# tsinghua-fib-lab/PIML

Hardware: AMD Instinct MI355X
Metric: agent-pair force evals/sec + simulated steps/sec, 4096-agent GC scene (higher is better)
Workload: dtype f32

## Files before the change

include/piml_hip.h:

```cpp
#ifndef PIML_HIP_H
#define PIML_HIP_H

#include <stddef.h>
#include <stdint.h>

#ifdef __cplusplus
extern "C" {
#endif

#define PIML_HIP_ABI_VERSION 35
#define PIML_MAX_TOPK 32

int piml_abi_version(void);

const char* piml_error_string(int err);

int piml_heading_fwd(const float* velocity, int C, int T, int N, float* heading, void* stream);

int piml_relfeat_fwd(const float* position, const float* heading, const float* velocity,
                     const float* acceleration, int state_ld, const float* destination,
                     const float* obstacles, int C, int N, int M, int focal_begin,
                     int focal_count, int topk_ped, int topk_obs, float cos_thr_ped,
                     float cos_thr_obs, float dist_thr_ped, float dist_thr_obs,
                     float* ped_feat, float* obs_feat, float* dest_feat, int dest_feat_ld,
// ... 564 lines not shown
    float* partials;
    float* grads;
    float* packed;
    float* pred;
    const float* g_pred_rows;
    const float* g_d2;
    const float *fold_w3, *fold_b3;
    float fold_scale;
    float* dw1_out;
} piml_decoder_branch;

int piml_decoder_pack_floats(void);
int piml_decoder_partial_floats(void);
int piml_decoder_workgroups(long long agents);
int piml_decoder_fwd(const piml_decoder_branch* branches, int nbranches, const float* self_features, float tau,
                     float* acc, void* stream);
int piml_decoder_bwd(const piml_decoder_branch* branches, int nbranches, const float* g_pred,
                     const float* self_features, float tau, float* g_self, void* stream);

int piml_rowdecoder_slots(long long rows);
int piml_rowdecoder_fwd(const piml_decoder_branch* branches, int nbranches, void* stream);
int piml_rowdecoder_fwd_packed(const piml_decoder_branch* branches, int nbranches, void* stream);
int piml_rowdecoder_bwd(const piml_decoder_branch* branches, int nbranches, void* stream);
int piml_rowdecoder_bwd_acc(const piml_decoder_branch* branches, int nbranches, int accumulate, void* stream);

typedef struct piml_collision_head {
    const float* msgs;
    long long rows;
    const float *w1, *b1, *w2, *b2;
    float* packed;
    float* out;
    const float *fold_w3, *fold_b3;
    float fold_scale;
} piml_collision_head;

int piml_collision_head_pack_floats(void);
int piml_collision_head_fwd(const float* msgs, long long rows, const float* w1, const float* b1, const float* w2,
                            const float* b2, float* packed, float* out, void* stream);

typedef struct piml_head64 {
    const float* x;
    long long rows;
    const float *w1, *b1, *w2, *b2;
    float* hidden;
    float* out;
    const float* g_out;
    float* g_x;
    float* partials;
    float* grads;
} piml_head64;
int piml_head64_partial_floats(void);
int piml_head64_slots(long long rows);
int piml_head64_fwd(const piml_head64* head, void* stream);
int piml_head64_bwd(const piml_head64* head, void* stream);
int piml_head64_bwd_acc(const piml_head64* head, int accumulate, void* stream);

typedef struct piml_corrector {
    long long agents;
    int k;
    float scale;
    const float* enc;
    const unsigned* keep_bits;
    const float *wa, *ba, *wb, *bb, *wc, *bc, *wd, *bd;
    float *hid, *score, *attn, *pooled, *chid, *out;
    const float* g_out;
    float *g_pooled, *g_score, *g_chid, *g_enc;
    float *partials_a, *partials_b, *grads;
} piml_corrector;
int piml_corrector_partial_floats(int which);
int piml_corrector_slots(int which, long long agents, int k);
int piml_corrector_fwd(const piml_corrector* c, void* stream);
int piml_corrector_bwd(const piml_corrector* c, int accumulate, void* stream);

int piml_pinnsf_unfold_defer(int on, void* stream);
#define PIML_PACKED_VALID 1
#define PIML_FORK 2
#define PIML_ACCUMULATE 4
#define PIML_DEFER_SLOT_SUMS 8
#define PIML_DEFER_PACK 16
#define PIML_POOL_H2 32
#define PIML_POOL_TRAIN 64
#define PIML_POOL_MSGS 128
#define PIML_DEFER_UNFOLD 256
int piml_pinnsf_pool_train_ok(const piml_encoder_branch* enc, int nbranches);
int piml_pinnsf_pool_msgs_ok(const piml_encoder_branch* enc, int nbranches);
int piml_pinnsf_pool_h2_ok(const piml_encoder_branch* enc, int nbranches);
int piml_pinnsf_pack_flush(void);
int piml_pinnsf_slot_sums_flush(void);
int piml_pinnsf_pack(const piml_encoder_branch* enc, const piml_decoder_branch* dec, int nbranches,
                     const piml_collision_head* head, int flags, void* stream);
int piml_pinnsf_fwd(const piml_encoder_branch* enc, const piml_decoder_branch* dec, int nbranches,
                    const piml_collision_head* head, const float* self_features, float tau, float* acc, int flags,
                    void* stream);
int piml_pinnsf_bwd(const piml_encoder_branch* enc, const piml_decoder_branch* dec, int nbranches, const float* g_pred,
                    const float* self_features, float tau, float* g_self, int flags, void* stream);

typedef struct piml_comm_id { char internal[128]; } piml_comm_id;
int piml_comm_available(void);
int piml_comm_unique_id(piml_comm_id* id);
int piml_comm_init(void** comm, int world, int rank, const piml_comm_id* id);
int piml_comm_destroy(void* comm);
int piml_allgather_state(void* comm, const float* own, size_t floats_per_rank, float* full, void* stream);
int piml_reducescatter_grad(void* comm, const float* full, float* own, size_t floats_per_rank, void* stream);
int piml_allreduce_sum(void* comm, float* buf, size_t count, void* stream);

typedef struct piml_ipc_handle { char internal[64]; } piml_ipc_handle;
int piml_p2p_alloc(size_t bytes, void** devptr);
int piml_p2p_free(void* devptr);
int piml_p2p_export(void* devptr, piml_ipc_handle* out);
int piml_p2p_open(const piml_ipc_handle* in, void** devptr);
int piml_p2p_close(void* devptr);
int piml_p2p_copy(void* dst, const void* src, size_t bytes, void* stream);
#define PIML_P2P_MAX_PARTS 8
typedef struct piml_p2p_msg {
    const float* scatter_src;
    size_t scatter_floats;
    float* out_scatter;
    int n_bcast;
    const float* bcast_src[PIML_P2P_MAX_PARTS];
    size_t bcast_floats[PIML_P2P_MAX_PARTS];
    float* out_bcast[PIML_P2P_MAX_PARTS];
    int sum;
} piml_p2p_msg;
int piml_p2p_exchange(const piml_p2p_msg* msg, int rank, int world, float* const* peer_recv, unsigned* const* peer_flags,
                      size_t slot_floats, unsigned* ctr, unsigned spin_limit, int* status, void* stream);
int piml_allgather_state_p2p(const float* own, size_t floats_per_rank, int rank, int world, float* const* peer_recv,
                             unsigned* const* peer_flags, unsigned seq, unsigned spin_limit, int* status, void* stream);

#ifdef __cplusplus
}
#endif
#endif
```

include/piml_hip_tuning.h:

```cpp
#ifndef PIML_HIP_TUNING_H
#define PIML_HIP_TUNING_H

#include "piml_hip.h"

#ifdef __cplusplus
extern "C" {
#endif

int piml_timer_create(void** event);
int piml_timer_record(void* event, void* stream);
int piml_timer_elapsed_ms(void* start, void* stop, float* ms);
int piml_timer_destroy(void* event);

int piml_trace_begin(void);
int piml_trace_mark(const char* name, void* stream);
int piml_trace_end(char* names, int names_cap, float* us, int us_cap);

int piml_probe_arith(const float* rx, const float* ry, const float* hx, const float* hy,
                     float* dist, float* cosv, int n, void* stream);

long long piml_encoder_split_tiles(long long tiles);
long long piml_encoder_split_tiles_train(long long tiles);
int piml_encoder_products(int split_bf16);
int piml_rowdecoder_products(int split_bf16);
int piml_encoder_dw2(int layer_split);
int piml_encoder_fused_bwd(int on);
int piml_encoder_sums_bwd(int form);
int piml_encoder_sums_dec_slots(int on);
int piml_encoder_compact_rows(int on);
int piml_relfeat_pack_form(int form);
int piml_relfeat_pack_plan(int form, int waves, int obstacle_workgroups, int nbr, int has_head, int has_fold, int skip_f32,
                           int* pack_blocks, int* share);
int piml_relfeat_pack_tail_blocks(int b, int nb, int total, int* out, int cap);
int piml_pinnsf_streams_init(void);

#ifdef __cplusplus
}
#endif
#endif
```

piml_amd/_lib.py:

```python
import ctypes
import os

import torch

_HERE = os.path.dirname(os.path.abspath(__file__))
LIB_PATH = os.environ.get('PIML_LIB') or os.path.join(_HERE, 'libpiml_hip.so')
ABI_VERSION = 35
COMPACT_MAX_AGENTS = 16384
COMPACT_SLOTS = 256

_lib = None

_i, _f, _p, _z = ctypes.c_int, ctypes.c_float, ctypes.c_void_p, ctypes.c_size_t
_ll = ctypes.c_longlong
_d = ctypes.c_double


class EncoderBranch(ctypes.Structure):
    _fields_ = [('x', _p), ('rows', _ll), ('in_dim', _i), ('k', _i),
                ('w1', _p), ('b1', _p), ('w2', _p), ('b2', _p), ('w3', _p), ('b3', _p),
                ('scale', _f), ('h1', _p), ('h2', _p), ('msgs', _p), ('g_pooled', _p), ('g_msgs', _p),
                ('g2', _p), ('g1', _p), ('g_x', _p), ('partials', _p), ('grads', _p), ('packed', _p), ('relu_mask', _p),
                ('keep_bits', _p), ('drop_state', _p), ('drop_p', _f), ('sum_a', _p), ('sum_b', _p),
                ('nbr_idx', _p), ('plan', _p)]
# ... 10 lines not shown
class CollisionHead(ctypes.Structure):
    _fields_ = [('msgs', _p), ('rows', _ll), ('w1', _p), ('b1', _p), ('w2', _p), ('b2', _p), ('packed', _p), ('out', _p),
                ('fold_w3', _p), ('fold_b3', _p), ('fold_scale', _f)]


class Head64(ctypes.Structure):
    _fields_ = [('x', _p), ('rows', _ll), ('w1', _p), ('b1', _p), ('w2', _p), ('b2', _p), ('hidden', _p), ('out', _p),
                ('g_out', _p), ('g_x', _p), ('partials', _p), ('grads', _p)]


class Corrector(ctypes.Structure):
    _fields_ = [('agents', _ll), ('k', _i), ('scale', _f), ('enc', _p), ('keep_bits', _p),
                ('wa', _p), ('ba', _p), ('wb', _p), ('bb', _p), ('wc', _p), ('bc', _p), ('wd', _p), ('bd', _p),
                ('hid', _p), ('score', _p), ('attn', _p), ('pooled', _p), ('chid', _p), ('out', _p),
                ('g_out', _p), ('g_pooled', _p), ('g_score', _p), ('g_chid', _p), ('g_enc', _p),
                ('partials_a', _p), ('partials_b', _p), ('grads', _p)]


class Scenario(ctypes.Structure):
    _fields_ = [('position', _p), ('velocity', _p), ('acceleration', _p), ('destination', _p), ('hist_velocity', _p),
                ('self_features', _p), ('desired_speed', _p), ('mask', _p), ('flag', _p), ('waypoints', _p), ('exit_idx', _p),
                ('spawn_iters', _p), ('position_out', _p), ('velocity_out', _p), ('acceleration_out', _p),
                ('destination_out', _p), ('mask_out', _p), ('spawn_out', _p), ('frame_counter', _p), ('spawned', _p),
                ('dropped', _p), ('entries', _p), ('route_polyline', _p),
                ('hist_width', _i), ('F', _i), ('D', _i), ('E', _i), ('P', _i), ('R', _i), ('capacity', _i), ('T', _i),
                ('n_initial', _i), ('route_max_iters', _i), ('spawn_cap', _i), ('uniform_speed', _i),
                ('dt', _f), ('spawn_offset', _f), ('route_clearance', _f), ('arrival_radius', _f), ('speed_mean', _f),
                ('speed_std', _f), ('speed_min', _f), ('seed', ctypes.c_uint64), ('poisson_thresholds', ctypes.c_uint32 * 8)]


class ScenarioRules(ctypes.Structure):
    _fields_ = [('spawn_law', _i), ('arrival_rule', _i), ('initial_velocity', _i), ('speed_clamp', _i), ('spawn_cap2', _i),
                ('grid', _i), ('length', _f), ('width', _f), ('side_ratio', _f), ('direction_ratio', _f),
                ('poisson_thresholds2', ctypes.c_uint32 * 8), ('square_grid', _f * 32)]


class MlapmLaw(ctypes.Structure):
    _fields_ = [('variant', _i), ('tau', _f), ('A', _f), ('B', _f), ('C', _f), ('D', _f), ('theta_deg', _f), ('radius', _f)]


class WallGrid(ctypes.Structure):
    _fields_ = [('points', _p), ('cell_start', _p), ('n_points', _i), ('gx', _i), ('gy', _i),
                ('x0', _f), ('y0', _f), ('cell', _f), ('cutoff', _f)]


class WallLaw(ctypes.Structure):
    _fields_ = [('A', _f), ('B', _f)]


class GroupLaw(ctypes.Structure):
    _fields_ = [('A', _f), ('dist', _f)]


class SceneGroups(ctypes.Structure):
    _fields_ = [('row_unit', _p), ('unit_rows', _p), ('n_units', _i), ('group_first', _p), ('group_size', _p)]


class NoiseLaw(ctypes.Structure):
    _fields_ = [('rho', _f), ('amp', _f)]


class NoiseArgs(ctypes.Structure):
    _fields_ = [('state', _p), ('law', NoiseLaw), ('law_table', _p)]


class NavGrid(ctypes.Structure):
    _fields_ = [('u', _p), ('G', _i), ('gx', _i), ('gy', _i), ('x0', _f), ('y0', _f), ('cell', _f), ('near', _f)]


class NavSight(ctypes.Structure):
    _fields_ = [('parent', _p), ('G', _i), ('gx', _i), ('gy', _i)]


class ExitChoice(ctypes.Structure):
    _fields_ = [('margin', _f), ('commit', _f), ('every', _i)]


SPAWN_LAWS = {'gc': 0, 'crosswalk': 1, 'square': 2, 'unit1': 3, 'unit2': 4, 'unit3': 5, 'clip': 6}
SPAWN_CLIP_GROUPS = 7
ARRIVAL_RULES = {'gc': 0, 'radius': 1, 'x_band': 2, 'x_exit': 3}


PACKED_VALID, FORK, ACCUMULATE, DEFER_SLOT_SUMS, DEFER_PACK, POOL_H2, POOL_TRAIN, POOL_MSGS, DEFER_UNFOLD = 1, 2, 4, 8, 16, 32, 64, 128, 256

SIGNATURES = {
    'piml_abi_version': [],
    'piml_heading_fwd': [_p, _i, _i, _i, _p, _p],
    'piml_relfeat_fwd': [_p, _p, _p, _p, _i, _p, _p, _i, _i, _i, _i, _i, _i, _i, _f, _f, _f, _f,
                         _p, _p, _p, _i, _p, _p, _p],
    'piml_mlapm_step_fwd': [_p, _p, _p, _p, _i, _i, _f, _f, _f, _f, _f, _f, _f, _f, _i, _p, _p, _p],
    'piml_mlapm_step_bwd': [_p, _p, _p, _p, _p, _i, _i, _f, _f, _f, _f, _f, _f, _f, _f, _p, _p, _p, _p, _p],
    'piml_mlapm_rollout_step': [_p, _p, _p, _p, _ll, _i, _i, _f, _f, _f, _f, _f, _f, _f, _f, _p, _p, _p],
    'piml_mlapm_bwd_workspace_floats': [_i, _i],
    'piml_mlapm_step_bwd_ws': [_p, _p, _p, _p, _p, _i, _i, _f, _f, _f, _f, _f, _f, _f, _f, _p, _p, _p, _p, _p, _ll, _p],
    'piml_mlapm_fit_workspace_doubles': [_i, _i],
    'piml_mlapm_fit_loss_grad': [_p, _p, _p, _p, _p, _p, _i, _i, _p, _i, _p, _i, _p, _i, _f, _f, _p, _ll, _p, _p, _p],
    'piml_mlapm_rollout_fit_workspace_doubles': [_i, _i, _ll],
    'piml_mlapm_rollout_fit_loss_grad': [_p, _p, _p, _p, _p, _i, _ll, _i, _p, _i, _p, _p, _i, _ll, _p, _i, _f, _f, _d,
                                         _p, _ll, _p, _p, _p, _p],
    'piml_collision_matrix': [_p, _i, _i, _f, _i, _p, _p],
    'piml_collision_friends': [_p, _p, _i, _i, _i, _i, _p],
    'piml_collision_counts': [_p, _i, _i, _p, _i, _p, _p],
    'piml_collision_counts_frames': [_p, _i, _i, _i, _p, _i, _p, _p],
    'piml_collision_counts_scratch': [_p, _i, _i, _p, _i, _p, _p, _p],
    'piml_collision_counts_grid': [_p, _i, _i, _p, _i, _p, _p, _p],
    'piml_collision_label': [_p, _z, _i, _p, _p],
    'piml_sinkhorn_frames': [_p, _p, _p, _p, _i, _i, _i, _f, _i, _f, _p, _p, _p, _p, _p],
    'piml_mmd_frames': [_p, _p, _p, _p, _i, _i, _i, _d, _i, _d, _p, _p],
    'piml_crowd_stats_workspace_bytes': [_i, _i, _i],
    'piml_crowd_stats': [_p, _p, _p, _p, _i, _i, _i, _i, _i, _f, _i, _f, _f, _f, _f, _f, _i, _i, _f, _i,
                         _p, _p, _p, _p, _p, _p, _p, _p, _p, _p, _ll, _p],
    'piml_crowd_stats_voronoi_workspace_bytes': [_i, _i, _i, _i],
    'piml_crowd_stats_voronoi': [_p, _p, _p, _p, _i, _i, _i, _i, _i, _f, _p, _i, _i, _f, _f, _f, _f, _i, _f, _f, _f, _f, _f,
                                 _i, _i, _f, _i, _p, _p, _p, _p, _p, _p, _p, _p, _p, _p, _p, _ll, _p],
    'piml_pair_stats_workspace_bytes': [_i, _i, _i, _i],
    'piml_pair_stats': [_p, _p, _p, _p, _i, _i, _i, _i, _i, _p, _i, _f, _f, _i, _f, _f, _f, _f, _f, _i, _f, _i,
                        _p, _p, _p, _p, _p, _p, _p, _p, _ll, _p],
    'piml_flow_stats_workspace_bytes': [_i, _i, _i, _i],
    'piml_flow_stats': [_p, _p, _p, _p, _i, _i, _i, _i, _i, _f, _f, _i, _f, _f, _f, _f, _f, _i, _f, _f, _f, _f, _f, _i, _i,
                        _p, _p, _p, _p, _p, _p, _p, _p, _p, _p, _p, _p, _ll, _p],
    'piml_view_stats_workspace_bytes': [_i, _i, _i, _i],
    'piml_view_stats': [_p, _p, _p, _p, _i, _i, _i, _i, _i, _p, _i, _f, _f, _i, _f, _f, _f, _f, _i, _i, _f, _f, _f, _f,
                        _p, _p, _p, _p, _p, _p, _p, _ll, _p],
    'piml_track_stats_workspace_bytes': [_i, _i, _i],
    'piml_track_stats': [_p, _p, _p, _i, _i, _i, _i, _i, _f, _f, _i, _f, _f, _i, _p, _p, _p, _p, _p, _p, _p, _p, _p, _p, _p, _p,
                         _p, _p, _ll, _p],
    'piml_obstacle_stats_workspace_bytes': [_i, _i, _i, _i],
    'piml_obstacle_stats': [_p, _p, _p, _p, _i, _i, _i, _i, _i, _p, _i, _f, _f, _f, _i, _f, _f, _f, _f, _f, _i, _f, _i,
                            _p, _p, _p, _p, _p, _p, _p, _p, _p, _p, _p, _p, _p, _p, _ll, _p],
    'piml_line_stats_workspace_bytes': [_i, _i, _i, _i, _i, _i],
    'piml_line_stats': [_p, _p, _p, _i, _i, _i, _i, _i, _p, _i, _f, _f, _i, _i, _p, _p, _p, _p, _p, _p, _p, _p, _p, _p, _p, _ll,
                        _p],
    'piml_group_pairs': [_p, _p, _p, _i, _i, _i, _i, _i, _f, _f, _f, _i, _i, _p, _p, _p, _p, _p, _p, _p],
    'piml_group_members': [_p, _p, _i, _i, _i, _i, _i, _p, _i, _f, _f, _f, _f, _i, _i, _p, _p, _p, _p, _p, _p],
    'piml_group_components': [_p, _p, _p, _p, _i, _i, _i, _i, _i, _i, _p, _p, _p, _p, _p, _p, _p, _p, _p],
    'piml_calc_acceleration': [_p, _z, _i, _i, _f, _f, _f, _f, _f, _f, _p, _p],
    'piml_rollout_step': [_p, _p, _p, _p, _p, _p, _i, _p, _p, _i, _i, _p, _p, _p, _p, _p, _p, _p, _i, _p, _p, _p,
                          _p, _p, _p, _p, _p, _i, _i, _i, _f, _i, _p],
    'piml_rollout_step_ksum': [_p, _i, _p, _i, _f, _p, _p, _p, _p, _p, _p, _i, _p, _p, _i, _i, _p, _p, _p, _p, _p, _p, _p, _i, _p, _p, _p,
                               _p, _p, _p, _p, _p, _i, _i, _i, _f, _i, _p],
    'piml_scenario_step': [_p, _p, _i, _p],
    'piml_scenario_step_rules': [_p, _p, _p, _i, _p],
    'piml_scenario_step_members': [_p, _p, _i, _p, _p, _i, _p],
    'piml_scenario_step_mlapm': [_p, _p, _i, _p, _p, _i, _p],
    'piml_mlapm_law_table_bytes': [_i],
    'piml_mlapm_law_table_fill': [_p, _i, _p],
    'piml_scenario_step_mlapm_laws': [_p, _p, _i, _p, _p, _i, _p],
    'piml_wall_force': [_p, _ll, _p, _f, _f, _p, _p, _p, _p],
    'piml_scenario_step_mlapm_walls': [_p, _p, _i, _p, _p, _p, _p, _p, _p, _i, _p],
    'piml_group_force': [_p, _p, _p, _ll, _f, _f, _p, _p],
    'piml_scenario_step_mlapm_groups': [_p, _p, _i, _p, _p, _p, _p, _p, _p, _p, _p, _p, _i, _i, _p],
    'piml_noise_force': [_p, _p, _p, _p, _p, _i, _i, _ll, _f, _f, _p],
    'piml_scenario_step_mlapm_noise': [_p, _p, _i, _p, _p, _p, _p, _p, _p, _p, _p, _p, _p, _i, _i, _p],
    'piml_nav_relax': [_p, _p, _p, _p, _i, _i, _i, _i, _p, _p],
    'piml_nav_direction': [_p, _p, _p, _ll, _p, _p, _p, _p, _p],
    'piml_scenario_step_mlapm_nav': [_p, _p, _i, _p, _p, _p, _p, _p, _p, _p, _p, _i, _p],
    'piml_nav_density': [_p, _p, _i, _i, _f, _f, _f, _i, _i, _p, _p],
    'piml_nav_cost': [_p, _i, _i, _i, _f, _i, _f, _f, _f, _p, _p],
    'piml_nav_relax_cost': [_p, _p, _p, _p, _p, _i, _i, _i, _i, _i, _p, _p],
    'piml_scenario_step_mlapm_navdyn': [_p, _p, _i, _p, _p, _p, _p, _p, _p, _p, _ll, _p, _i, _p],
    'piml_nav_descent': [_p, _i, _i, _i, _p, _p],
    'piml_nav_flow': [_p, _p, _p, _i, _i, _f, _f, _f, _i, _i, _p, _p, _p],
    'piml_nav_cost_flow': [_p, _p, _p, _i, _i, _i, _i, _f, _i, _f, _f, _f, _f, _f, _p, _p],
    'piml_nav_relax_cost_gates': [_p, _p, _p, _p, _p, _i, _i, _i, _i, _i, _p, _p],
    'piml_nav_relax_active': [_p, _p, _p, _i, _p, _p, _i, _i, _i, _i, _i, _p, _p, _p, _p],
    'piml_nav_choose_exit': [_p, _i, _p, _p, _ll, _p, _p, _p, _i, _p],
    'piml_nav_sight_relax': [_p, _p, _p, _p, _p, _p, _p, _i, _i, _i, _i, _p, _p],
    'piml_nav_direction_sight': [_p, _p, _p, _ll, _p, _p, _p, _p, _p, _p],
    'piml_scenario_step_mlapm_sight': [_p, _p, _i, _p, _p, _p, _p, _p, _p, _p, _p, _p, _i, _p],
    'piml_scenario_step_nav': [_p, _p, _i, _p, _p, _i, _p, _p, _p, _p],
    'piml_scenario_route': [_p, _p, _i, _p, _i, _i, _f, _p, _p, _p],
    'piml_collision_correction_fwd': [_p, _p, _p, _z, _i, _i, _f, _f, _p, _p],
    'piml_collision_correction_bwd': [_p, _p, _p, _p, _z, _i, _i, _f, _f, _p, _p, _p, _p],
    'piml_train_step_fwd': [_p] * 7 + [_i, _i, _p, _p, _p, _p, _p, _p, _p, _i, _i, _i, _i, _f, _p, _p, _p, _p, _p, _p, _p, _p],
    'piml_train_step_fwd_copy': [_p] * 7 + [_i, _i, _p, _p, _p, _p, _p, _p, _p, _i, _i, _i, _i, _f, _p, _p, _p, _p, _p, _p, _p, _p, _ll, _p],
    'piml_train_step_bwd': [_p, _p, _p, _p, _p, _i, _i, _i, _i, _f, _p, _p, _p, _p, _p],
    'piml_train_step_bwd6': [_p, _p, _p, _p, _p, _p, _i, _i, _i, _i, _f, _p, _p, _p, _p, _p],
    'piml_pinnsf_unfold_defer': [_i, _p],
    'piml_train_step_bwd7': [_p, _ll, _p, _p, _p, _p, _ll, _p, _p, _i, _i, _i, _i, _f, _p, _p, _p, _p, _p],
    'piml_train_step_tail_fwd': [_p, _p, _p, _p, _i, _p, _i, _p, _f, _p, _p, _p, _i, _i, _p, _p, _p, _p, _p, _p, _p, _i, _i, _i, _i, _f,
                                 _p, _p, _p, _p, _p, _p, _p, _p, _ll, _p],
    'piml_train_step_tail_bwd': [_p, _ll, _p, _p, _p, _p, _ll, _p, _p, _i, _i, _i, _i, _f, _p, _p, _p, _p, _p, _f, _i, _i, _p, _p, _p, _p],
    'piml_pinnsf_epilogue_fwd': [_p, _p, _p, _z, _f, _p, _p],
    'piml_pinnsf_epilogue_bwd': [_p, _p, _z, _f, _p, _p],
    'piml_pinnsf_epilogue_ksum_fwd': [_p, _i, _p, _i, _p, _z, _f, _p, _p],
    'piml_pinnsf_epilogue_ksum_bwd': [_p, _p, _z, _f, _i, _i, _p, _p, _p, _p],
    'piml_pinnsf_epilogue_agentnorm_fwd': [_p, _p, _p, _i, _i, _f, _p, _p],
    'piml_pinnsf_epilogue_ksum_agentnorm_fwd': [_p, _i, _p, _i, _p, _i, _i, _f, _p, _p],
    'piml_pinnsf_epilogue_agentnorm_bwd': [_p, _p, _i, _i, _f, _p, _p],
    'piml_self_features_fwd': [_p, _i, _p, _p, _z, _p, _p],
    'piml_self_features_bwd': [_p, _z, _p, _p, _p, _p],
    'piml_colsum_blocks': [_z, _i],
    'piml_act_bwd_colsum': [_p, _p, _z, _i, _p, _p, _p, _p],
    'piml_sum_leading': [_p, _i, _z, _p, _p],
    'piml_act_bwd_colsum_stage1': [_p, _p, _z, _i, _p, _p, _p, _p],
    'piml_layer_reduce': [_p, _i, _z, _p, _p, _i, _i, _p, _p],
    'piml_scale_ksum_fwd': [_p, _p, _z, _i, _i, _f, _p, _p, _p, _p],
    'piml_ksum_blocks': [_z, _i],
    'piml_scale_ksum_bwd': [_p, _p, _z, _i, _i, _f, _p, _p, _p, _p],
    'piml_dropout_keep_bits': [_p, _ll, _i, _f, _i, _p, _p],
    'piml_timer_create': [ctypes.POINTER(_p)],
    'piml_timer_record': [_p, _p],
    'piml_timer_elapsed_ms': [_p, _p, ctypes.POINTER(_f)],
    'piml_timer_destroy': [_p],
    'piml_trace_begin': [],
    'piml_trace_mark': [ctypes.c_char_p, _p],
    'piml_trace_end': [ctypes.c_char_p, _i, ctypes.POINTER(_f), _i],
    'piml_probe_arith': [_p, _p, _p, _p, _p, _p, _i, _p],
    'piml_encoder_partial_floats': [],
    'piml_encoder_pack_floats': [],
    'piml_encoder_split_tiles': [_ll],
    'piml_encoder_split_tiles_train': [_ll],
    'piml_multi_copy': [ctypes.POINTER(_p), ctypes.POINTER(_p), ctypes.POINTER(_z), _i, _p],
    'piml_rollout_prologue': [_p] * 8 + [_i] * 4 + [_p] * 11 + [_p],
    'piml_rollout_losses_blocks': [_i, _i],
    'piml_rollout_losses': [_p, _p, _ll, _p, _p, _p, _p, _p, _i, _i, _i, _f, _p, _p, _p, _p, _p, _p, _p],
    'piml_rollout_losses_bwd': [_p, _p, _p, _p, _p, _p, _ll, _p, _p],
    'piml_rollout_losses_frames': [_p, _p, _ll, _p, _p, ctypes.POINTER(_p), _i, _p, _i, _i, _i, _f, _f, _f, _p, _p, _p, _p, _p, _p, _p],
    'piml_rollout_losses_frames_bwd': [_p, _p, _p, _p, _f, _f, _p, _p, _p, _ll, _p, _p],
    'piml_collision_pred_loss_blocks': [_ll, _i],
    'piml_collision_pred_loss': [ctypes.POINTER(_p), ctypes.POINTER(_p), _i, _ll, _i, _i, _p, _i, _i, _f, _p, _p, _p, _p, _p],
    'piml_collision_pred_loss_bwd': [_p, _p, _ll, _p, _p],
    'piml_adam_tickets': [],
    'piml_adam_step': [ctypes.POINTER(_p)] * 5 + [ctypes.POINTER(_ll), _i, ctypes.c_double, ctypes.c_double, ctypes.c_double, ctypes.c_double, ctypes.c_double, _p, _p],
    'piml_pointwise_losses_blocks': [_ll, _ll, _i],
    'piml_pointwise_losses': [_p, _p, _ll, _ll, _p, _ll, _f, _p, _i, _p, _p, _p, _p, _p],
    'piml_p2p_alloc': [_z, ctypes.POINTER(_p)],
    'piml_p2p_free': [_p],
    'piml_p2p_export': [_p, _p],
    'piml_p2p_open': [_p, ctypes.POINTER(_p)],
    'piml_p2p_close': [_p],
    'piml_p2p_copy': [_p, _p, _z, _p],
    'piml_allgather_state_p2p': [_p, _z, _i, _i, ctypes.POINTER(_p), ctypes.POINTER(_p), ctypes.c_uint, ctypes.c_uint, _p, _p],
    'piml_encoder_products': [_i],
    'piml_relfeat_pack_form': [_i],
    'piml_relfeat_pack_plan': [_i, _i, _i, _i, _i, _i, _i, ctypes.POINTER(_i), ctypes.POINTER(_i)],
    'piml_relfeat_pack_tail_blocks': [_i, _i, _i, ctypes.POINTER(_i), _i],
    'piml_rowdecoder_products': [_i],
    'piml_encoder_dw2': [_i],
    'piml_encoder_fused_bwd': [_i],
    'piml_encoder_sums_bwd': [_i],
    'piml_encoder_sums_dec_slots': [_i],
    'piml_encoder_compact_rows': [_i],
    'piml_encoder_pack': [ctypes.POINTER(EncoderBranch), _i, _p],
    'piml_encoder_workgroups': [ctypes.POINTER(EncoderBranch), _i, ctypes.POINTER(_i)],
    'piml_encoder_fwd': [ctypes.POINTER(EncoderBranch), _i, _p],
    'piml_encoder_fwd_packed': [ctypes.POINTER(EncoderBranch), _i, _p],
    'piml_encoder_bwd': [ctypes.POINTER(EncoderBranch), _i, _p],
    'piml_encoder_bwd_acc': [ctypes.POINTER(EncoderBranch), _i, _i, _p],
    'piml_encoder_ksum': [_p, _ll, _i, _p, _p],
    'piml_decoder_pack_floats': [],
    'piml_decoder_partial_floats': [],
    'piml_decoder_workgroups': [_ll],
    'piml_decoder_fwd': [ctypes.POINTER(DecoderBranch), _i, _p, _f, _p, _p],
    'piml_decoder_bwd': [ctypes.POINTER(DecoderBranch), _i, _p, _p, _f, _p, _p],
    'piml_rowdecoder_slots': [_ll],
    'piml_rowdecoder_fwd': [ctypes.POINTER(DecoderBranch), _i, _p],
    'piml_rowdecoder_fwd_packed': [ctypes.POINTER(DecoderBranch), _i, _p],
    'piml_rowdecoder_bwd': [ctypes.POINTER(DecoderBranch), _i, _p],
    'piml_rowdecoder_bwd_acc': [ctypes.POINTER(DecoderBranch), _i, _i, _p],
    'piml_collision_head_pack_floats': [],
    'piml_collision_head_fwd': [_p, _ll, _p, _p, _p, _p, _p, _p, _p],
    'piml_head64_partial_floats': [],
    'piml_head64_slots': [_ll],
    'piml_head64_fwd': [ctypes.POINTER(Head64), _p],
    'piml_head64_bwd': [ctypes.POINTER(Head64), _p],
    'piml_head64_bwd_acc': [ctypes.POINTER(Head64), _i, _p],
    'piml_corrector_partial_floats': [_i],
    'piml_corrector_slots': [_i, _ll, _i],
    'piml_corrector_fwd': [ctypes.POINTER(Corrector), _p],
    'piml_corrector_bwd': [ctypes.POINTER(Corrector), _i, _p],
    'piml_pinnsf_pool_h2_ok': [ctypes.POINTER(EncoderBranch), _i],
    'piml_pinnsf_pool_train_ok': [ctypes.POINTER(EncoderBranch), _i],
    'piml_pinnsf_pool_msgs_ok': [ctypes.POINTER(EncoderBranch), _i],
    'piml_pinnsf_streams_init': [],
    'piml_pinnsf_pack_flush': [],
    'piml_pinnsf_slot_sums_flush': [],
    'piml_pinnsf_pack': [ctypes.POINTER(EncoderBranch), ctypes.POINTER(DecoderBranch), _i, ctypes.POINTER(CollisionHead),
                         _i, _p],
    'piml_pinnsf_fwd': [ctypes.POINTER(EncoderBranch), ctypes.POINTER(DecoderBranch), _i, ctypes.POINTER(CollisionHead),
                        _p, _f, _p, _i, _p],
    'piml_pinnsf_bwd': [ctypes.POINTER(EncoderBranch), ctypes.POINTER(DecoderBranch), _i, _p, _p, _f, _p, _i, _p],
    'piml_comm_available': [],
    'piml_comm_unique_id': [_p],
    'piml_comm_init': [ctypes.POINTER(_p), _i, _i, _p],
    'piml_comm_destroy': [_p],
    'piml_allgather_state': [_p, _p, _z, _p, _p],
    'piml_reducescatter_grad': [_p, _p, _p, _z, _p],
    'piml_allreduce_sum': [_p, _p, _z, _p],
    'piml_relfeat_fwd_self': [_p, _p, _p, _p, _i, _p, _p, _p, _i, _i, _i, _i, _i, _i, _i, _f, _f, _f, _f, _p, _p, _p, _p, _p, _p, _p],
    'piml_relfeat_bwd_self': [_p, _p, _p, _p, _p, _p, _i, _p, _i, _i, _i, _i, _i, _i, _p, _p, _p, _p],
    'piml_relfeat_fwd_tick': [_p, _p, _p, _p, _i, _p, _p, _i, _i, _i, _i, _i, _i, _i, _f, _f, _f, _f,
                              _p, _p, _p, _i, _p, _p, _p, _p],
    'piml_relfeat_self_fwd': [_p, _p, _p, _p, _i, _i, _i, _i, _i, _i, _f, _f, _f, _f, _p, _p, _p, _p, _p, _p, _p],
    'piml_relfeat_self_fwd_part': [_i, _p, _p, _p, _p, _i, _i, _i, _i, _i, _i, _f, _f, _f, _f, _p, _p, _p, _p, _p, _p, _p],
    'piml_relfeat_self_bwd': [_p, _p, _p, _p, _p, _p, _p, _i, _i, _i, _i, _i, _p, _p, _p, _p],
    'piml_relfeat_bwd_det': [_p, _p, _p, _p, _p, _p, _p, _p, _i, _p, _i, _i, _i, _i, _i, _i, _i, _p, _p, _p],
    'piml_relfeat_bwd': [_p, _p, _p, _p, _p, _p, _i, _p, _i, _i, _i, _i, _i, _i, _p, _p, _p],
}


class P2PMsg(ctypes.Structure):
    _fields_ = [('scatter_src', _p), ('scatter_floats', _z), ('out_scatter', _p), ('n_bcast', _i),
                ('bcast_src', _p * 8), ('bcast_floats', _z * 8), ('out_bcast', _p * 8), ('sum', _i)]


SIGNATURES['piml_p2p_exchange'] = [ctypes.POINTER(P2PMsg), _i, _i, ctypes.POINTER(_p), ctypes.POINTER(_p), _z, _p, ctypes.c_uint, _p, _p]


class PimlHipError(RuntimeError):
    pass


def lib():
    global _lib
    if _lib is None:
        if not os.path.exists(LIB_PATH):
            raise PimlHipError(
                f'{LIB_PATH} is missing: build it with `python -m piml_amd.build` '
                '(hipcc --offload-arch=gfx950). piml_amd has no CPU fallback.')
        L = ctypes.CDLL(LIB_PATH)
        for name, args in SIGNATURES.items():
            fn = getattr(L, name)
            fn.argtypes = args
            fn.restype = _i
        L.piml_encoder_split_tiles.restype = _ll
# ... 137 lines not shown
```

piml_amd/csrc/decoder.hip:

```cpp
#include <cstdlib>
#include <type_traits>

#include "common.hpp"
#include "pack.hpp"
#include "reduce.hpp"
#include "stages.hpp"
#include "x3.hpp"
#include "store.hpp"
#include "../../include/piml_hip.h"

namespace piml {

typedef float f32x16 __attribute__((ext_vector_type(16)));

constexpr int DEC_SLAB = 32;

struct DecArgs {
    piml_decoder_branch br[2];
    int nbr;
    const float* self_features;
    float tau;
    float* acc;
    const float* g_pred;
    float* g_self;
    int wg_split;
    int pool_h2;
};

#ifdef PIML_DEC_STAMPS
__device__ unsigned long long g_dec_stamps[1024 * 16];
#define DEC_STAMP(i, wait)                                                                         \
    do {                                                                                           \
        __builtin_amdgcn_sched_barrier(0);                                                         \
        if (wait) asm volatile("s_waitcnt vmcnt(0) lgkmcnt(0)" ::: "memory");                      \
        if (threadIdx.x == 0 && blockIdx.x < 1024) g_dec_stamps[blockIdx.x * 16 + (i)] = __builtin_amdgcn_s_memtime(); \
        __builtin_amdgcn_sched_barrier(0);                                                         \
    } while (0)
#else
#define DEC_STAMP(i, wait)
#endif

__device__ __forceinline__ f32x16 dmfma(float a, float b, f32x16 c) {
    return __builtin_amdgcn_mfma_f32_32x32x2f32(a, b, c, 0, 0, 0);
}
__device__ __forceinline__ int dfeat0(int blk, int q, int h) { return 32 * blk + 8 * q + 4 * h; }

__global__ __launch_bounds__(256) void dec_pack_kernel(DecArgs A) {
    const int b = blockIdx.y;
    const piml_decoder_branch J = b ? A.br[1] : A.br[0];
    const int e = blockIdx.x * 256 + threadIdx.x;
    if (e < DEC_PACK) J.packed[e] = dec_pack_value(J, e);
}

__device__ __forceinline__ void dec_pool_body(const piml_decoder_branch& J, long long bx) {
    const long long t = bx * 256 + threadIdx.x;
    if (t >= J.agents * (DH / 4)) return;
    const long long a = t / (DH / 4);
    const int c = (int)(t % (DH / 4));
    const float4* p = reinterpret_cast<const float4*>(J.msgs) + a * J.k * (DH / 4) + c;
    float4 s = make_float4(0.f, 0.f, 0.f, 0.f);
    for (int i = 0; i < J.k; ++i) {
        const float4 v = p[(size_t)i * (DH / 4)];
        s.x += v.x; s.y += v.y; s.z += v.z; s.w += v.w;
    }
    reinterpret_cast<float4*>(J.pooled)[t] = s;
}

__global__ __launch_bounds__(256) void dec_pool_kernel(DecArgs A) {
    dec_pool_body(blockIdx.y ? A.br[1] : A.br[0], blockIdx.x);
}

constexpr int POOL_ROWS = 10;

template <bool POOL, bool SPLIT = false, bool ROWS = false>
__device__ __forceinline__ void dec_fwd_body(const DecArgs& A, long long tile, int split_branch = 0) {
    constexpr int NB = SPLIT ? 1 : 2;
    __shared__ float part1[NB][2][2][16][64];
    __shared__ float part2[NB][2][2][16][64];
    __shared__ float part3[NB][2][2][32];
    __shared__ float poolx[POOL ? NB : 1][POOL ? 4 : 1][POOL ? 16 : 1][64];
    const int lane = threadIdx.x & 63, wave = uniform((int)(threadIdx.x >> 6));
    const int j = lane & 31, h = lane >> 5;
    const int b = SPLIT ? split_branch : wave >> 2, ob = (wave >> 1) & 1, kh = wave & 1;
    const int bi = SPLIT ? 0 : b;
    const bool active = b < A.nbr;
    const piml_decoder_branch J = b ? A.br[1] : A.br[0];
    const long long agent = tile * 32 + j;
    const bool valid = active && agent < J.agents;
    const float4* PK = reinterpret_cast<const float4*>(J.packed);
    const float* bias = J.packed + DP_B;
    float4 w2f[4], w3f[4], w1f[2][4], b2v[4];
    float b3x = 0.f, b3y = 0.f;
    if (active) {
#pragma unroll
        for (int bl = 0; bl < 2; ++bl)
#pragma unroll
            for (int q = 0; q < 4; ++q) w1f[bl][q] = PK[(A.pool_h2 == 2 ? DP_A1F : DP_A1) / 4 + ((ob * 4 + 2 * kh + bl) * 4 + q) * 64 + lane];
    }
    float4 b1v[4];
    float sfv[5] = {0.f, 0.f, 0.f, 0.f, 0.f};
    auto late_loads = [&]() {
#pragma unroll
        for (int q = 0; q < 4; ++q) {
            b1v[q] = *reinterpret_cast<const float4*>(bias + dfeat0(ob, q, h));
            if (!POOL && !ROWS && A.pool_h2 == 2) {
                const float4 cv = *reinterpret_cast<const float4*>(J.packed + DP_CF + dfeat0(ob, q, h));
                const float kf = (float)J.k;
                b1v[q].x += kf * cv.x; b1v[q].y += kf * cv.y; b1v[q].z += kf * cv.z; b1v[q].w += kf * cv.w;
            }
            w2f[q] = PK[DP_A2 / 4 + ((ob * 2 + kh) * 4 + q) * 64 + lane];
            w3f[q] = PK[DP_A3 / 4 + (kh * 4 + q) * 64 + lane];
            b2v[q] = *reinterpret_cast<const float4*>(bias + 64 + dfeat0(ob, q, h));
        }
        b3x = bias[128];
        b3y = bias[129];
        if (A.self_features && b == 0 && wave == 0) {
            const float* sp = A.self_features + (agent < A.br[0].agents ? agent : 0) * 7;
            sfv[0] = sp[0]; sfv[1] = sp[1]; sfv[2] = sp[2]; sfv[3] = sp[3]; sfv[4] = sp[6];
        }
    };
    if (POOL) {
        if (active) {
            const int blk = wave & 3, k = J.k;
            const float* mp = J.msgs + (valid ? agent : 0) * (long long)k * DH;
            float4 sum[4];
#pragma unroll
            for (int q = 0; q < 4; ++q) sum[q] = make_float4(0.f, 0.f, 0.f, 0.f);
            for (int r0 = 0; r0 < k; r0 += POOL_ROWS) {
                float4 v[POOL_ROWS][4];
#pragma unroll
                for (int u = 0; u < POOL_ROWS; ++u) {
                    const int r = r0 + u < k ? r0 + u : 0;
#pragma unroll
                    for (int q = 0; q < 4; ++q) v[u][q] = *reinterpret_cast<const float4*>(mp + (long long)r * DH + dfeat0(blk, q, h));
                }
#pragma unroll
                for (int u = 0; u < POOL_ROWS; ++u) {
                    const bool ok = r0 + u < k;
#pragma unroll
                    for (int q = 0; q < 4; ++q) {
                        sum[q].x += ok ? v[u][q].x : 0.f; sum[q].y += ok ? v[u][q].y : 0.f;
                        sum[q].z += ok ? v[u][q].z : 0.f; sum[q].w += ok ? v[u][q].w : 0.f;
                    }
                }
            }
            late_loads();
            __builtin_amdgcn_sched_barrier(0);
#pragma unroll
            for (int q = 0; q < 4; ++q) {
                if (valid) *reinterpret_cast<float4*>(J.pooled + agent * DH + dfeat0(blk, q, h)) = sum[q];
                poolx[bi][blk][4 * q + 0][lane] = valid ? sum[q].x : 0.f; poolx[bi][blk][4 * q + 1][lane] = valid ? sum[q].y : 0.f;
                poolx[bi][blk][4 * q + 2][lane] = valid ? sum[q].z : 0.f; poolx[bi][blk][4 * q + 3][lane] = valid ? sum[q].w : 0.f;
            }
        }
        __syncthreads();
    }
    float4 pv[2][4];
    if (SPLIT && !POOL && !ROWS) DEC_STAMP(0, false);
    if (active) {
        if (POOL) {
#pragma unroll
            for (int bl = 0; bl < 2; ++bl)
#pragma unroll
                for (int q = 0; q < 4; ++q)
                    pv[bl][q] = make_float4(poolx[bi][2 * kh + bl][4 * q][lane], poolx[bi][2 * kh + bl][4 * q + 1][lane],
                                            poolx[bi][2 * kh + bl][4 * q + 2][lane], poolx[bi][2 * kh + bl][4 * q + 3][lane]);
        } else {
            const float* base = (ROWS ? J.msgs : J.pooled) + (valid ? agent : 0) * DH;
#pragma unroll
            for (int bl = 0; bl < 2; ++bl)
#pragma unroll
                for (int q = 0; q < 4; ++q) pv[bl][q] = *reinterpret_cast<const float4*>(base + dfeat0(2 * kh + bl, q, h));
            if (!ROWS && A.pool_h2) {
                const long long g0 = (valid ? agent : 0) * J.k;
                if (valid && (g0 >> 5) != ((g0 + J.k - 1) >> 5)) {
                    const float* more = J.msgs + agent * DH;
#pragma unroll
                    for (int bl = 0; bl < 2; ++bl)
#pragma unroll
                        for (int q = 0; q < 4; ++q) {
                            const float4 c = *reinterpret_cast<const float4*>(more + dfeat0(2 * kh + bl, q, h));
                            pv[bl][q].x += c.x; pv[bl][q].y += c.y; pv[bl][q].z += c.z; pv[bl][q].w += c.w;
                        }
                }
            }
        }
        if (!POOL) late_loads();
        f32x16 a1;
#pragma unroll
        for (int q = 0; q < 4; ++q) {
            const float4 bq = b1v[q];
            a1[4 * q] = kh ? 0.f : bq.x; a1[4 * q + 1] = kh ? 0.f : bq.y;
            a1[4 * q + 2] = kh ? 0.f : bq.z; a1[4 * q + 3] = kh ? 0.f : bq.w;
        }
        __builtin_amdgcn_sched_barrier(0);
        if (SPLIT && !POOL && !ROWS) { DEC_STAMP(1, false); DEC_STAMP(2, true); }
#pragma unroll
        for (int bl = 0; bl < 2; ++bl)
#pragma unroll
            for (int q = 0; q < 4; ++q) {
                const float4 w = w1f[bl][q], x = pv[bl][q];
                a1 = dmfma(w.x, valid ? x.x : 0.f, a1);
                a1 = dmfma(w.y, valid ? x.y : 0.f, a1);
                a1 = dmfma(w.z, valid ? x.z : 0.f, a1);
                a1 = dmfma(w.w, valid ? x.w : 0.f, a1);
            }
#pragma unroll
        for (int r = 0; r < 16; ++r) part1[bi][ob][kh][r][lane] = a1[r];
        if (SPLIT && !POOL && !ROWS) DEC_STAMP(3, true);
    }
    __syncthreads();
    if (SPLIT && !POOL && !ROWS) DEC_STAMP(4, false);
    if (active) {
        if (!POOL && !ROWS && A.pool_h2 >= 2 && ob == 0) {
            const long long g0 = (valid ? agent : 0) * J.k;
            if (valid && (g0 >> 5) != ((g0 + J.k - 1) >> 5)) {
#pragma unroll
                for (int bl = 0; bl < 2; ++bl)
#pragma unroll
                    for (int q = 0; q < 4; ++q) *reinterpret_cast<float4*>(J.pooled + agent * DH + dfeat0(2 * kh + bl, q, h)) = pv[bl][q];
            }
        }
        float x[16];
#pragma unroll
        for (int r = 0; r < 16; ++r) x[r] = fmaxf(part1[bi][kh][0][r][lane] + part1[bi][kh][1][r][lane], 0.f);
        x[0] = __builtin_fmaf(part1[bi][kh][0][0][lane] + part1[bi][kh][1][0][lane], 0.f, x[0]);
        if (ob == 0 && J.h1 && valid) {
            float* o = J.h1 + agent * DD;
#pragma unroll
            for (int q = 0; q < 4; ++q)
                *reinterpret_cast<float4*>(o + dfeat0(kh, q, h)) = make_float4(x[4 * q], x[4 * q + 1], x[4 * q + 2], x[4 * q + 3]);
        }
        f32x16 a2;
#pragma unroll
        for (int q = 0; q < 4; ++q) {
            const float4 bq = b2v[q];
            a2[4 * q] = kh ? 0.f : bq.x; a2[4 * q + 1] = kh ? 0.f : bq.y;
            a2[4 * q + 2] = kh ? 0.f : bq.z; a2[4 * q + 3] = kh ? 0.f : bq.w;
        }
#pragma unroll
        for (int q = 0; q < 4; ++q) {
            const float4 w = w2f[q];
            a2 = dmfma(w.x, x[4 * q + 0], a2);
            a2 = dmfma(w.y, x[4 * q + 1], a2);
            a2 = dmfma(w.z, x[4 * q + 2], a2);
            a2 = dmfma(w.w, x[4 * q + 3], a2);
        }
#pragma unroll
        for (int r = 0; r < 16; ++r) part2[bi][ob][kh][r][lane] = a2[r];
        if (SPLIT && !POOL && !ROWS) DEC_STAMP(5, true);
    }
    __syncthreads();
    if (SPLIT && !POOL && !ROWS) DEC_STAMP(6, false);
    if (active && ob == 0) {
        float y[16];
#pragma unroll
        for (int r = 0; r < 16; ++r) y[r] = part2[bi][kh][0][r][lane] + part2[bi][kh][1][r][lane];
        if (J.d2 && valid) {
            float* o = J.d2 + agent * DD;
#pragma unroll
            for (int q = 0; q < 4; ++q)
                *reinterpret_cast<float4*>(o + dfeat0(kh, q, h)) = make_float4(y[4 * q], y[4 * q + 1], y[4 * q + 2], y[4 * q + 3]);
        }
        f32x16 a3;
#pragma unroll
        for (int r = 0; r < 16; ++r) a3[r] = 0.f;
        if (h == 0 && kh == 0) { a3[0] = b3x; a3[1] = b3y; }
#pragma unroll
        for (int q = 0; q < 4; ++q) {
            const float4 w = w3f[q];
            a3 = dmfma(w.x, y[4 * q + 0], a3);
            a3 = dmfma(w.y, y[4 * q + 1], a3);
            a3 = dmfma(w.z, y[4 * q + 2], a3);
            a3 = dmfma(w.w, y[4 * q + 3], a3);
        }
        if (h == 0) { part3[bi][kh][0][j] = a3[0]; part3[bi][kh][1][j] = a3[1]; }
        if (SPLIT && !POOL && !ROWS) DEC_STAMP(7, true);
    }
    __syncthreads();
    if (SPLIT && !POOL && !ROWS) DEC_STAMP(8, false);
    if (ROWS) {
        if ((wave & 3) == 0 && h == 0 && agent < J.agents)
            reinterpret_cast<float2*>(J.pred)[agent] = make_float2(part3[0][0][0][j] + part3[0][1][0][j],
                                                                   part3[0][0][1][j] + part3[0][1][1][j]);
        return;
    }
    if (wave == 0 && h == 0 && agent < A.br[0].agents) {
        float ax = part3[0][0][0][j] + part3[0][1][0][j], ay = part3[0][0][1][j] + part3[0][1][1][j];
        if (A.self_features && b == 0) {
            const float dx = sfv[0], dy = sfv[1], vx = sfv[2], vy = sfv[3], v0 = sfv[4];
            float t = norm2(dx, dy);
            t = (t == 0.f) ? t + 0.1f : t;
            ax += (v0 * (dx / t) - vx) / A.tau;
            ay += (v0 * (dy / t) - vy) / A.tau;
        }
        if (SPLIT) {
            if (A.nbr > 1) {
                atomicAdd(A.acc + 2 * agent, ax);
                atomicAdd(A.acc + 2 * agent + 1, ay);
            } else {
                reinterpret_cast<float2*>(A.acc)[agent] = make_float2(ax, ay);
            }
        } else {
            if (A.nbr > 1) { ax += part3[1][0][0][j] + part3[1][1][0][j]; ay += part3[1][0][1][j] + part3[1][1][1][j]; }
            reinterpret_cast<float2*>(A.acc)[agent] = make_float2(ax, ay);
        }
    }
    if (SPLIT && !POOL && !ROWS) DEC_STAMP(9, true);
}

__global__ __launch_bounds__(512) void dec_fwd_kernel(DecArgs A) { dec_fwd_body<false>(A, blockIdx.x); }

template <bool ROWS = false, bool SPLIT = false>
__device__ __forceinline__ void dec_bwd_dx_body(const DecArgs& A, long long tile, int rows_branch = 0, float* keep_g2 = nullptr,
                                                float* keep_g1 = nullptr) {
    constexpr int NB = (ROWS || SPLIT) ? 1 : 2;
    __shared__ float part[NB][2][2][16][64];
    const int lane = threadIdx.x & 63, wave = uniform((int)(threadIdx.x >> 6));
    const int j = lane & 31, h = lane >> 5;
    const int b = (ROWS || SPLIT) ? rows_branch : wave >> 2, ob = (wave >> 1) & 1, kh = wave & 1, blk = wave & 3;
    const int bi = (ROWS || SPLIT) ? 0 : b;
    const bool active = b < A.nbr;
    const piml_decoder_branch J = b ? A.br[1] : A.br[0];
    const long long agent = tile * 32 + j;
    const bool valid = active && agent < J.agents;
    const float4* PK = reinterpret_cast<const float4*>(J.packed);
    float2 gp = make_float2(0.f, 0.f);
    float4 hv[2][4], t1f[8];
    float sfv[5] = {0.f, 0.f, 0.f, 0.f, 0.f};
    if (active) {
        gp = reinterpret_cast<const float2*>(ROWS ? J.g_pred_rows : A.g_pred)[valid ? agent : 0];
        if (!valid) gp = make_float2(0.f, 0.f);
        float4 gd2[4];
        if (ROWS && J.g_d2) {
#pragma unroll
            for (int q = 0; q < 4; ++q) gd2[q] = *reinterpret_cast<const float4*>(J.g_d2 + (valid ? agent : 0) * DD + dfeat0(kh, q, h));
        }
        if (!ROWS && wave == 0 && b == 0 && A.g_self && A.self_features) {
            const float* sp = A.self_features + (valid ? agent : 0) * 7;
            sfv[0] = sp[0]; sfv[1] = sp[1]; sfv[4] = sp[6];
        }
        const float bg = h ? gp.y : gp.x;
        const float* hp = J.h1 + (valid ? agent : 0) * DD;
#pragma unroll
        for (int o2 = 0; o2 < 2; ++o2)
#pragma unroll
            for (int q = 0; q < 4; ++q) hv[o2][q] = *reinterpret_cast<const float4*>(hp + dfeat0(o2, q, h));
        const float t3f = J.packed[DP_T3 + 64 * kh + lane];
        float4 t2f[4];
#pragma unroll
        for (int q = 0; q < 4; ++q) t2f[q] = PK[DP_T2 / 4 + (ob * 8 + kh * 4 + q) * 64 + lane];
#pragma unroll
        for (int t = 0; t < 8; ++t) t1f[t] = PK[((!ROWS && A.pool_h2 == 2) ? DP_T1F : DP_T1) / 4 + (blk * 8 + t) * 64 + lane];
        __builtin_amdgcn_sched_barrier(0);
        if (SPLIT) { DEC_STAMP(1, false); DEC_STAMP(2, true); }
        f32x16 g2, g1;
#pragma unroll
        for (int r = 0; r < 16; ++r) { g2[r] = 0.f; g1[r] = 0.f; }
        g2 = dmfma(t3f, bg, g2);
        if (ROWS && J.g_d2) {
#pragma unroll
            for (int q = 0; q < 4; ++q) {
                g2[4 * q] += valid ? gd2[q].x : 0.f; g2[4 * q + 1] += valid ? gd2[q].y : 0.f;
                g2[4 * q + 2] += valid ? gd2[q].z : 0.f; g2[4 * q + 3] += valid ? gd2[q].w : 0.f;
            }
        }
        if (SPLIT && keep_g2) {
            if (ob == 0) {
#pragma unroll
                for (int q = 0; q < 4; ++q)
                    *reinterpret_cast<float4*>(keep_g2 + j * DD + dfeat0(kh, q, h)) =
                        valid ? make_float4(g2[4 * q], g2[4 * q + 1], g2[4 * q + 2], g2[4 * q + 3]) : make_float4(0.f, 0.f, 0.f, 0.f);
            }
        } else if (ob == 0 && valid) {
            float* o = J.g_pre2 + agent * DD;
#pragma unroll
            for (int q = 0; q < 4; ++q)
                *reinterpret_cast<float4*>(o + dfeat0(kh, q, h)) = make_float4(g2[4 * q], g2[4 * q + 1], g2[4 * q + 2], g2[4 * q + 3]);
        }
#pragma unroll
        for (int q = 0; q < 4; ++q) {
            const float4 w = t2f[q];
            g1 = dmfma(w.x, g2[4 * q + 0], g1);
            g1 = dmfma(w.y, g2[4 * q + 1], g1);
            g1 = dmfma(w.z, g2[4 * q + 2], g1);
            g1 = dmfma(w.w, g2[4 * q + 3], g1);
        }
#pragma unroll
        for (int r = 0; r < 16; ++r) part[bi][ob][kh][r][lane] = g1[r];
        if (SPLIT) DEC_STAMP(3, true);
    }
    __syncthreads();
    if (SPLIT) DEC_STAMP(4, false);
    if (active) {
    float g1c[2][16];
#pragma unroll
    for (int o2 = 0; o2 < 2; ++o2)
#pragma unroll
        for (int q = 0; q < 4; ++q) {
            const float4 a = hv[o2][q];
            const float m[4] = {a.x, a.y, a.z, a.w};
#pragma unroll
            for (int u = 0; u < 4; ++u) {
                const float v = part[bi][o2][0][4 * q + u][lane] + part[bi][o2][1][4 * q + u][lane];
                g1c[o2][4 * q + u] = (valid && m[u] > 0.f) ? v : 0.f;
            }
        }
    if (SPLIT && keep_g1) {
        if (blk < 2) {
#pragma unroll
            for (int q = 0; q < 4; ++q) {
                const float4 v0 = make_float4(g1c[0][4 * q], g1c[0][4 * q + 1], g1c[0][4 * q + 2], g1c[0][4 * q + 3]);
                const float4 v1 = make_float4(g1c[1][4 * q], g1c[1][4 * q + 1], g1c[1][4 * q + 2], g1c[1][4 * q + 3]);
                if (blk == 0) *reinterpret_cast<float4*>(keep_g1 + j * DD + dfeat0(0, q, h)) = v0;
                else *reinterpret_cast<float4*>(keep_g1 + j * DD + dfeat0(1, q, h)) = v1;
            }
        }
    } else if (blk < 2 && valid) {
        float* o = J.g_pre1 + agent * DD;
#pragma unroll
        for (int q = 0; q < 4; ++q) {
            const float4 v0 = make_float4(g1c[0][4 * q], g1c[0][4 * q + 1], g1c[0][4 * q + 2], g1c[0][4 * q + 3]);
            const float4 v1 = make_float4(g1c[1][4 * q], g1c[1][4 * q + 1], g1c[1][4 * q + 2], g1c[1][4 * q + 3]);
            if (blk == 0) *reinterpret_cast<float4*>(o + dfeat0(0, q, h)) = v0;
            else *reinterpret_cast<float4*>(o + dfeat0(1, q, h)) = v1;
        }
    }
    {
        f32x16 gpool;
#pragma unroll
        for (int r = 0; r < 16; ++r) gpool[r] = 0.f;
#pragma unroll
        for (int bp = 0; bp < 2; ++bp)
#pragma unroll
            for (int q = 0; q < 4; ++q) {
                const float4 w = t1f[bp * 4 + q];
                gpool = dmfma(w.x, g1c[bp][4 * q + 0], gpool);
                gpool = dmfma(w.y, g1c[bp][4 * q + 1], gpool);
                gpool = dmfma(w.z, g1c[bp][4 * q + 2], gpool);
                gpool = dmfma(w.w, g1c[bp][4 * q + 3], gpool);
            }
        if (valid) {
            float* o = J.g_pooled + agent * DH;
#pragma unroll
            for (int q = 0; q < 4; ++q)
                *reinterpret_cast<float4*>(o + dfeat0(blk, q, h)) =
                    make_float4(gpool[4 * q], gpool[4 * q + 1], gpool[4 * q + 2], gpool[4 * q + 3]);
        }
    }
    }
    if (SPLIT) DEC_STAMP(5, true);
    if (!ROWS && wave == 0 && b == 0 && h == 0 && valid && A.g_self && A.self_features) {
        const float dx = sfv[0], dy = sfv[1], v0 = sfv[4], tau = A.tau;
        const float n = norm2(dx, dy);
        const float t = (n == 0.f) ? n + 0.1f : n;
        const float ex = dx / t, ey = dy / t;
        const float gex = gp.x * v0 / tau, gey = gp.y * v0 / tau;
        const float gt = -(gex * dx + gey * dy) / (t * t);
        float gdx = gex / t, gdy = gey / t;
        if (n != 0.f) { gdx += gt * (dx / n); gdy += gt * (dy / n); }
        float* o = A.g_self + agent * 7;
        o[0] = gdx; o[1] = gdy; o[2] = -gp.x / tau; o[3] = -gp.y / tau; o[4] = 0.f; o[5] = 0.f;
        o[6] = (gp.x * ex + gp.y * ey) / tau;
    }
}

__global__ __launch_bounds__(512) void dec_bwd_dx_kernel(DecArgs A) { dec_bwd_dx_body<false>(A, blockIdx.x); }

template <bool ROWS = false>
__device__ __forceinline__ void dec_bwd_dw_body(const DecArgs& A, int b, int p, int w, int lane, long long slab = DEC_SLAB) {
    const piml_decoder_branch J = b ? A.br[1] : A.br[0];
    const long long R = J.agents;
    const long long s0 = (long long)p * slab < R ? (long long)p * slab : R;
    const long long s1e = s0 + slab < R ? s0 + slab : R;
    const float* __restrict__ in1 = ROWS ? J.msgs : J.pooled;
    const float* __restrict__ gpr = ROWS ? J.g_pred_rows : A.g_pred;
    const int i = lane & 31, h = lane >> 5;
    const int mb1 = w >> 2, nb1 = w & 3, mb2 = (w >> 1) & 1, nb2 = w & 1;
    const bool do2 = w < 4, do3 = w == 4 || w == 5;
    f32x16 c1, c2, c3;
#pragma unroll
    for (int r = 0; r < 16; ++r) { c1[r] = 0.f; c2[r] = 0.f; c3[r] = 0.f; }
    float s1 = 0.f, s2 = 0.f, s3 = 0.f;
    constexpr int U = DEC_SLAB / 2;
    for (long long r0 = s0; r0 < s1e || r0 == s0; r0 += DEC_SLAB) {
        const long long r1 = r0 + DEC_SLAB < s1e ? r0 + DEC_SLAB : s1e;
        float a1[U], b1[U], a2[U], b2[U], a3[U], b3[U];
#pragma unroll
        for (int u = 0; u < U; ++u) {
            const long long row = r0 + 2 * u + h;
            const bool ok = row < r1;
            const long long ro = ok ? row : (r0 < R ? r0 : 0);
            a1[u] = J.g_pre1[ro * DD + 32 * mb1 + i];
            b1[u] = in1[ro * DH + 32 * nb1 + i];
            a2[u] = do2 ? J.g_pre2[ro * DD + 32 * mb2 + i] : 0.f;
            b2[u] = do2 ? J.h1[ro * DD + 32 * nb2 + i] : 0.f;
            a3[u] = (do3 && i < 2) ? gpr[ro * 2 + i] : 0.f;
            b3[u] = do3 ? J.d2[ro * DD + 32 * nb2 + i] : 0.f;
        }
#pragma unroll
        for (int u = 0; u < U; ++u) {
            const bool ok = r0 + 2 * u + h < r1;
            const float x1 = ok ? a1[u] : 0.f, x2 = ok ? a2[u] : 0.f, x3 = ok ? a3[u] : 0.f;
            c1 = dmfma(x1, b1[u], c1);
            if (do2) c2 = dmfma(x2, b2[u], c2);
            if (do3) c3 = dmfma(x3, b3[u], c3);
            s1 += x1; s2 += x2; s3 += x3;
        }
    }
    float* P = J.partials + (size_t)p * DEC_PART;
#pragma unroll
    for (int r = 0; r < 16; ++r) {
        const int ri = (r & 3) + 8 * (r >> 2) + 4 * h;
        P[(size_t)(32 * mb1 + ri) * DH + 32 * nb1 + i] = c1[r];
        if (do2) P[DD * DH + (32 * mb2 + ri) * DD + 32 * nb2 + i] = c2[r];
        if (do3 && ri < 2) P[DD * DH + DD * DD + ri * DD + 32 * nb2 + i] = c3[r];
    }
    s1 += __shfl_xor(s1, 32, 64);
    s2 += __shfl_xor(s2, 32, 64);
    s3 += __shfl_xor(s3, 32, 64);
    float* Pb = P + DD * DH + DD * DD + 2 * DD;
    if (h == 0) {
        if (nb1 == 0) Pb[32 * mb1 + i] = s1;
        if (do2 && nb2 == 0) Pb[DD + 32 * mb2 + i] = s2;
        if (w == 4 && i < 8) Pb[2 * DD + i] = i < 2 ? s3 : 0.f;
    }
}

__device__ __forceinline__ void dec_bwd_dw_body4(const DecArgs& A, int b, int p, int w, int lane, const float* keep_g2, const float* keep_g1) {
    const piml_decoder_branch J = b ? A.br[1] : A.br[0];
    const long long R = J.agents;
    const long long s0 = (long long)p * DEC_SLAB < R ? (long long)p * DEC_SLAB : R;
    const int n = (int)(R - s0 < DEC_SLAB ? R - s0 : DEC_SLAB);
    const long long sb = n > 0 ? s0 : 0;
    const int i = lane & 31, h = lane >> 5;
    const int mb2 = w >> 1, nb2 = w & 1;
    const bool do3 = w < 2;
    constexpr int U = DEC_SLAB / 2;
    const float* __restrict__ pooled0 = J.pooled + sb * DH + 32 * w + i;
    const float* __restrict__ h10 = J.h1 + sb * DD + 32 * nb2 + i;
    const float* __restrict__ d20 = J.d2 + sb * DD + 32 * nb2 + i;
    const float* __restrict__ gp0 = A.g_pred + sb * 2 + (i & 1);
    const float* kg1 = keep_g1 + h * DD + i;
    const float* kg2 = keep_g2 + h * DD + 32 * mb2 + i;
    float a1a[U], a1b[U], b1[U], a2[U], b2[U], a3[U], b3[U];
#pragma unroll
    for (int u = 0; u < U; ++u) {
        a1a[u] = kg1[2 * u * DD];
        a1b[u] = kg1[2 * u * DD + 32];
        a2[u] = kg2[2 * u * DD];
        a3[u] = 0.f; b3[u] = 0.f;
    }
    if (n == DEC_SLAB) {
        const float* pb = pooled0 + h * DH;
        const float* hb = h10 + h * DD;
#pragma unroll
        for (int u = 0; u < U; ++u) { b1[u] = pb[2 * u * DH]; b2[u] = hb[2 * u * DD]; }
        if (do3) {
            const float* db = d20 + h * DD;
            const float* gb = gp0 + h * 2;
#pragma unroll
            for (int u = 0; u < U; ++u) { b3[u] = db[2 * u * DD]; a3[u] = gb[4 * u]; }
        }
    } else {
#pragma unroll
        for (int u = 0; u < U; ++u) {
            const int rc = 2 * u + h < n ? 2 * u + h : 0;
            b1[u] = pooled0[rc * DH]; b2[u] = h10[rc * DD];
        }
        if (do3) {
#pragma unroll
            for (int u = 0; u < U; ++u) {
                const int rc = 2 * u + h < n ? 2 * u + h : 0;
                b3[u] = d20[rc * DD]; a3[u] = gp0[rc * 2];
            }
        }
    }
    DEC_STAMP(8, false);
    DEC_STAMP(9, true);
    f32x16 c1a, c1b, c2, c3;
#pragma unroll
    for (int r = 0; r < 16; ++r) { c1a[r] = 0.f; c1b[r] = 0.f; c2[r] = 0.f; c3[r] = 0.f; }
    float s1a = 0.f, s1b = 0.f, s2 = 0.f, s3 = 0.f;
#pragma unroll
    for (int u = 0; u < U; ++u) {
        c1a = dmfma(a1a[u], b1[u], c1a);
        c1b = dmfma(a1b[u], b1[u], c1b);
        c2 = dmfma(a2[u], b2[u], c2);
        s1a += a1a[u]; s1b += a1b[u]; s2 += a2[u];
    }
    if (do3) {
#pragma unroll
        for (int u = 0; u < U; ++u) {
            const float x3 = (i < 2 && 2 * u + h < n) ? a3[u] : 0.f;
            c3 = dmfma(x3, b3[u], c3);
            s3 += x3;
        }
    }
    float* P = J.partials + (size_t)p * DEC_PART;
    DEC_STAMP(10, false);
    {
#ifdef PIML_DEC_STAMPS
        asm volatile("v_mov_b32 %0, %0" : "+v"(c1a[0]));
        DEC_STAMP(11, false);
#endif
    }
    {
        store_acc32<PIML_WT_DEC_BWD_SLOTS>(P + 32 * w, DH, lane, [&](int r) { return c1a[r]; });
        store_acc32<PIML_WT_DEC_BWD_SLOTS>(P + 32 * DH + 32 * w, DH, lane, [&](int r) { return c1b[r]; });
        store_acc32<PIML_WT_DEC_BWD_SLOTS>(P + DD * DH + 32 * mb2 * DD + 32 * nb2, DD, lane, [&](int r) { return c2[r]; });
        if (do3 && h == 0) {
            float* P3 = P + DD * DH + DD * DD + 32 * nb2 + i;
            P3[0] = c3[0]; P3[DD] = c3[1];
        }
    }
    s1a += __shfl_xor(s1a, 32, 64);
    s1b += __shfl_xor(s1b, 32, 64);
    s2 += __shfl_xor(s2, 32, 64);
    s3 += __shfl_xor(s3, 32, 64);
    float* Pb = P + DD * DH + DD * DD + 2 * DD;
    if (h == 0) {
        if (w == 0) { Pb[i] = s1a; Pb[32 + i] = s1b; }
        if (nb2 == 0) Pb[DD + 32 * mb2 + i] = s2;
        if (w == 0 && i < 8) Pb[2 * DD + i] = i < 2 ? s3 : 0.f;
    }
    DEC_STAMP(12, false);
    DEC_STAMP(13, true);
}

__global__ __launch_bounds__(256) void dec_bwd_split_kernel(DecArgs A) {
    const int bx = blockIdx.x;
    const int b = A.nbr > 1 ? (bx & 1) : 0;
    const long long tile = A.nbr > 1 ? (bx >> 1) : bx;
    __shared__ __align__(16) float keep[2][32 * DD];
    DEC_STAMP(0, false);
    dec_bwd_dx_body<false, true>(A, tile, b, keep[0], keep[1]);
    DEC_STAMP(6, false);
    __syncthreads();
    DEC_STAMP(7, false);
    dec_bwd_dw_body4(A, b, (int)tile, uniform((int)(threadIdx.x >> 6)), threadIdx.x & 63, keep[0], keep[1]);
}

__global__ __launch_bounds__(512) void dec_bwd_dw_kernel(DecArgs A) {
    const int lane = threadIdx.x & 63, w = uniform((int)(threadIdx.x >> 6));
    const int b = (A.nbr > 1 && (int)blockIdx.x >= A.wg_split) ? 1 : 0;
    dec_bwd_dw_body<false>(A, b, (int)blockIdx.x - (b ? A.wg_split : 0), w, lane);
}

__global__ __launch_bounds__(256) void rowdec_fwd_kernel(DecArgs A, int tiles0) {
    const int bx = blockIdx.x;
    if (bx < tiles0) dec_fwd_body<false, true, true>(A, bx, 0);
    else dec_fwd_body<false, true, true>(A, bx - tiles0, 1);
}

__global__ __launch_bounds__(256) void rowdec_bwd_dx_kernel(DecArgs A, int tiles0) {
    const int bx = blockIdx.x;
    if (bx < tiles0) dec_bwd_dx_body<true>(A, bx, 0);
    else dec_bwd_dx_body<true>(A, bx - tiles0, 1);
}

template <int NFLOATS>
__device__ __forceinline__ void rowdec_stage(float* lds, const float* __restrict__ src, int tid) {
    constexpr int N4 = NFLOATS / 4, ROUNDS = (N4 + 511) / 512;
    static_assert(NFLOATS % 4 == 0, "float4 granularity");
    const float4* s4 = reinterpret_cast<const float4*>(src);
    float4* d4 = reinterpret_cast<float4*>(lds);
    float4 v[ROUNDS];
#pragma unroll
    for (int r = 0; r < ROUNDS; ++r) {
        const int e = r * 512 + tid;
        v[r] = s4[e < N4 ? e : 0];
    }
#pragma unroll
    for (int r = 0; r < ROUNDS; ++r) {
        const int e = r * 512 + tid;
        if (e < N4) d4[e] = v[r];
    }
}

__global__ __launch_bounds__(512) void rowdec_fwd_big_kernel(DecArgs A, int wg_split) {
    __shared__ __align__(16) float lds[DP_T3];
    const int tid = threadIdx.x, lane = tid & 63, wave = uniform((int)(tid >> 6));
    const int b = (A.nbr > 1 && (int)blockIdx.x >= wg_split) ? 1 : 0;
    const piml_decoder_branch J = b ? A.br[1] : A.br[0];
    const int wg0 = b ? wg_split : 0;
    const int nwg = b ? (int)gridDim.x - wg_split : (A.nbr > 1 ? wg_split : (int)gridDim.x);
    const long long R = J.agents, ntiles = (R + 31) >> 5;
    if ((long long)((int)blockIdx.x - wg0) * 8 >= ntiles) return;
    rowdec_stage<DP_T3>(lds, J.packed, tid);
    __syncthreads();
    const float4* F = reinterpret_cast<const float4*>(lds);
    const float* bias = lds + DP_B;
    const int j = lane & 31, h = lane >> 5;
    for (long long tile = (long long)((int)blockIdx.x - wg0) * 8 + wave; tile < ntiles; tile += (long long)nwg * 8) {
        const long long row = tile * 32 + j;
        const bool valid = row < R;
        f32x16 X[4];
        {
            const float* base = J.msgs + (valid ? row : 0) * DH;
#pragma unroll
            for (int blk = 0; blk < 4; ++blk)
#pragma unroll
                for (int q = 0; q < 4; ++q) {
                    const float4 v = *reinterpret_cast<const float4*>(base + dfeat0(blk, q, h));
                    X[blk][4 * q] = valid ? v.x : 0.f; X[blk][4 * q + 1] = valid ? v.y : 0.f;
                    X[blk][4 * q + 2] = valid ? v.z : 0.f; X[blk][4 * q + 3] = valid ? v.w : 0.f;
                }
        }
        f32x16 a1[2], a2[2];
#pragma unroll
        for (int ob = 0; ob < 2; ++ob) {
#pragma unroll
            for (int q = 0; q < 4; ++q) {
                const float4 bq = *reinterpret_cast<const float4*>(bias + dfeat0(ob, q, h));
                a1[ob][4 * q] = bq.x; a1[ob][4 * q + 1] = bq.y; a1[ob][4 * q + 2] = bq.z; a1[ob][4 * q + 3] = bq.w;
            }
#pragma unroll
            for (int bp = 0; bp < 4; ++bp) {
                __builtin_amdgcn_sched_barrier(0);
#pragma unroll
                for (int q = 0; q < 4; ++q) {
                    const float4 w = F[DP_A1 / 4 + ((ob * 4 + bp) * 4 + q) * 64 + lane];
                    a1[ob] = dmfma(w.x, X[bp][4 * q + 0], a1[ob]);
// ... 944 lines not shown
#ifdef PIML_DEC_STAMPS
extern "C" __attribute__((visibility("default"))) int piml_dec_stamps(unsigned long long* out) {
    return (int)hipMemcpyFromSymbol(out, HIP_SYMBOL(piml::g_dec_stamps), sizeof(unsigned long long) * 1024 * 16);
}
#endif

using namespace piml;

PIML_API int piml_decoder_pack_floats(void) { return DEC_PACK; }
PIML_API int piml_decoder_partial_floats(void) { return DEC_PART; }
PIML_API int piml_decoder_workgroups(long long agents) { return dec_dw_workgroups(agents); }

static int head_check(const piml_collision_head* h);

static int dec_fill(DecArgs& A, const piml_decoder_branch* br, int nbr) {
    if (!br || nbr < 1 || nbr > 2) return hipErrorInvalidValue;
    A = DecArgs{};
    A.nbr = nbr;
    for (int i = 0; i < nbr; ++i) {
        if (!dec_branch_ok(br[i]) || br[i].agents != br[0].agents || !br[i].pooled) return hipErrorInvalidValue;
        A.br[i] = br[i];
    }
    if (nbr == 1) A.br[1] = br[0];
    return hipSuccess;
}

static int dec_fill_bwd(DecArgs& A, const piml_decoder_branch* br, int nbr, const float* g_pred) {
    if (!g_pred) return hipErrorInvalidValue;
    if (int e = dec_fill(A, br, nbr)) return e;
    for (int i = 0; i < nbr; ++i) {
        const piml_decoder_branch& b = br[i];
        if (!b.h1 || !b.d2 || !b.g_pre2 || !b.g_pre1 || !b.g_pooled || !b.partials || !b.grads) return hipErrorInvalidValue;
    }
    A.g_pred = g_pred;
    return hipSuccess;
}

int piml::dec_stage_pack(const piml_decoder_branch* br, int nbr, hipStream_t s) {
    if (!br || nbr < 1 || nbr > 2) return hipErrorInvalidValue;
    DecArgs A = {};
    A.nbr = nbr;
    for (int i = 0; i < nbr; ++i) {
        const piml_decoder_branch& b = br[i];
        if (!b.w1 || !b.b1 || !b.w2 || !b.b2 || !b.w3 || !b.b3 || !b.packed) return hipErrorInvalidValue;
        A.br[i] = b;
    }
    if (nbr == 1) A.br[1] = br[0];
    hipLaunchKernelGGL(dec_pack_kernel, dim3((DEC_PACK + 255) / 256, nbr), dim3(256), 0, s, A);
    return hipGetLastError();
}

int piml::dec_stage_pool(const piml_decoder_branch* br, int nbr, hipStream_t s) {
    DecArgs A;
    if (int e = dec_fill(A, br, nbr)) return e;
    hipLaunchKernelGGL(dec_pool_kernel, dim3((unsigned)((br[0].agents * (DH / 4) + 255) / 256), nbr), dim3(256), 0, s, A);
    return hipGetLastError();
}

template <bool X3>
__global__ __launch_bounds__(256) __attribute__((amdgpu_waves_per_eu(2))) void dec_fwd_head_kernel(DecArgs A, piml_collision_head Hd, int dec_blocks) {
    const int bx = blockIdx.x;
    if (bx < dec_blocks) {
        if (A.nbr > 1) dec_fwd_body<true, true>(A, bx >> 1, bx & 1);
        else dec_fwd_body<true, true>(A, bx, 0);
    } else {
        extern __shared__ __align__(16) float head_lds[];
        if (X3) head_fwd_body_x3<4, false, HEAD_LDS_GROUPS_POOL>(Hd.msgs, Hd.rows, Hd.packed, Hd.out, (long long)bx - dec_blocks, reinterpret_cast<u32x4*>(head_lds));
        else head_fwd_body<4>(Hd.msgs, Hd.rows, Hd.packed, Hd.out, (long long)bx - dec_blocks);
    }
}

template <bool FOLD>
__global__ __launch_bounds__(256) __attribute__((amdgpu_waves_per_eu(2))) void dec_fwd_head_sum_kernel(DecArgs A, piml_collision_head Hd, int dec_blocks) {
    const int bx = blockIdx.x;
    if (bx < dec_blocks) {
        if (A.nbr > 1) dec_fwd_body<false, true>(A, bx >> 1, bx & 1);
        else dec_fwd_body<false, true>(A, bx, 0);
    } else {
        extern __shared__ __align__(16) float head_lds[];
        head_fwd_body_x3<4, FOLD, HEAD_LDS_GROUPS>(Hd.msgs, Hd.rows, Hd.packed, Hd.out, (long long)bx - dec_blocks, reinterpret_cast<u32x4*>(head_lds));
    }
}

int piml::dec_stage_fwd_sum(const piml_decoder_branch* br, int nbr, const piml_collision_head* h, const float* self_features,
                            float tau, float* acc, hipStream_t s, bool fold) {
    DecArgs A;
    if (!acc) return hipErrorInvalidValue;
    if (int e = dec_fill(A, br, nbr)) return e;
    for (int i = 0; i < nbr; ++i)
        if (!br[i].msgs || (fold && (!br[i].fold_w3 || !br[i].fold_b3))) return hipErrorInvalidValue;
    piml_collision_head Hd = {};
    int head_blocks = 0;
    if (h && h->rows > 0) {
        if (int e = head_check(h)) return e;
        if (fold && (!h->fold_w3 || !h->fold_b3)) return hipErrorInvalidValue;
        if (!g_head_x3) return hipErrorInvalidValue;
        Hd = *h;
        head_blocks = (int)(((h->rows + 31) / 32 + 3) / 4);
    }
    A.self_features = self_features;
    A.tau = tau;
    A.acc = acc;
    A.pool_h2 = fold ? 2 : 3;
    const int tiles = (int)((br[0].agents + 31) / 32) * nbr;
    const dim3 g((unsigned)(tiles + head_blocks));
    const int lds = head_blocks ? head_lds_bytes(HEAD_LDS_GROUPS) : 0;
    if (fold) hipLaunchKernelGGL(dec_fwd_head_sum_kernel<true>, g, dim3(256), lds, s, A, Hd, tiles);
    else hipLaunchKernelGGL(dec_fwd_head_sum_kernel<false>, g, dim3(256), lds, s, A, Hd, tiles);
    return hipGetLastError();
}

int piml::dec_stage_fwd_fused(const piml_decoder_branch* br, int nbr, const piml_collision_head* h, const float* self_features,
                              float tau, float* acc, hipStream_t s) {
    DecArgs A;
    if (!acc) return hipErrorInvalidValue;
    if (int e = dec_fill(A, br, nbr)) return e;
    piml_collision_head Hd = {};
    int head_blocks = 0;
    if (h && h->rows > 0) {
        if (int e = head_check(h)) return e;
        Hd = *h;
        head_blocks = (int)(((h->rows + 31) / 32 + 3) / 4);
    }
    A.self_features = self_features;
    A.tau = tau;
    A.acc = acc;
    const int tiles = (int)((br[0].agents + 31) / 32) * nbr;
    if (g_head_x3) hipLaunchKernelGGL(dec_fwd_head_kernel<true>, dim3((unsigned)(tiles + head_blocks)), dim3(256), head_blocks ? head_lds_bytes(HEAD_LDS_GROUPS_POOL) : 0, s, A, Hd, tiles);
    else hipLaunchKernelGGL(dec_fwd_head_kernel<false>, dim3((unsigned)(tiles + head_blocks)), dim3(256), 0, s, A, Hd, tiles);
    return hipGetLastError();
}

__global__ __launch_bounds__(256) __attribute__((amdgpu_waves_per_eu(2))) void dec_fwd_ph2_kernel(DecArgs A) {
    const int bx = blockIdx.x;
    if (A.nbr > 1) dec_fwd_body<false, true>(A, bx >> 1, bx & 1);
    else dec_fwd_body<false, true>(A, bx, 0);
}

int piml::dec_stage_fwd_ph2(const piml_decoder_branch* br, int nbr, const float* self_features, float tau, float* acc,
                            hipStream_t s) {
    DecArgs A;
    if (!acc) return hipErrorInvalidValue;
    if (int e = dec_fill(A, br, nbr)) return e;
    for (int i = 0; i < nbr; ++i)
        if (!br[i].msgs) return hipErrorInvalidValue;
    A.self_features = self_features;
    A.tau = tau;
    A.acc = acc;
    A.pool_h2 = 1;
    const int tiles = (int)((br[0].agents + 31) / 32) * nbr;
    hipLaunchKernelGGL(dec_fwd_ph2_kernel, dim3((unsigned)tiles), dim3(256), 0, s, A);
    return hipGetLastError();
}

int piml::dec_stage_fwd(const piml_decoder_branch* br, int nbr, const float* self_features, float tau, float* acc,
                        hipStream_t s) {
    DecArgs A;
    if (!acc) return hipErrorInvalidValue;
    if (int e = dec_fill(A, br, nbr)) return e;
    A.self_features = self_features;
    A.tau = tau;
    A.acc = acc;
    const unsigned tiles = (unsigned)((br[0].agents + 31) / 32);
    hipLaunchKernelGGL(dec_fwd_kernel, dim3(tiles), dim3(512), 0, s, A);
    return hipGetLastError();
}

int piml::dec_stage_bwd_dx(const piml_decoder_branch* br, int nbr, const float* g_pred, const float* self_features,
                           float tau, float* g_self, hipStream_t s) {
    DecArgs A;
    if (int e = dec_fill_bwd(A, br, nbr, g_pred)) return e;
    A.self_features = self_features;
    A.tau = tau;
    A.g_self = g_self;
    const unsigned tiles = (unsigned)((br[0].agents + 31) / 32);
    hipLaunchKernelGGL(dec_bwd_dx_kernel, dim3(tiles), dim3(512), 0, s, A);
    return hipGetLastError();
}

int piml::dec_stage_bwd_fused(const piml_decoder_branch* br, int nbr, const float* g_pred, const float* self_features,
                              float tau, float* g_self, hipStream_t s, bool sums) {
    DecArgs A;
    if (int e = dec_fill_bwd(A, br, nbr, g_pred)) return e;
    A.self_features = self_features;
    A.tau = tau;
    A.g_self = g_self;
    if (sums) {
        for (int i = 0; i < nbr; ++i)
            if (!br[i].fold_w3) return hipErrorInvalidValue;
        A.pool_h2 = 2;
    }
    static_assert(DEC_SLAB == 32, "the dW slab of a workgroup is its dX tile");
    const unsigned tiles = (unsigned)((br[0].agents + 31) / 32);
    hipLaunchKernelGGL(dec_bwd_split_kernel, dim3(tiles * (unsigned)nbr), dim3(256), 0, s, A);
    return hipGetLastError();
}

int piml::dec_stage_bwd_dw(const piml_decoder_branch* br, int nbr, const float* g_pred, bool reduce, hipStream_t s) {
    DecArgs A;
    if (int e = dec_fill_bwd(A, br, nbr, g_pred)) return e;
    const int per = dec_dw_workgroups(br[0].agents);
    A.wg_split = per;
    hipLaunchKernelGGL(dec_bwd_dw_kernel, dim3(per * nbr), dim3(512), 0, s, A);
    if (reduce)
        hipLaunchKernelGGL(dec_reduce_kernel, dim3((DEC_PART / 4 + 15) / 16, nbr), dim3(256), 0, s, A, per, DEC_PART / 4);
    return hipGetLastError();
}

static int head_check(const piml_collision_head* h) {
    if (!h || h->rows < 0) return hipErrorInvalidValue;
    if (h->rows > 0 && (!h->msgs || !h->w1 || !h->b1 || !h->w2 || !h->b2 || !h->packed || !h->out)) return hipErrorInvalidValue;
    return hipSuccess;
}

int piml::head_stage_pack(const piml_collision_head* h, hipStream_t s) {
    if (!h || !h->w1 || !h->b1 || !h->w2 || !h->b2 || !h->packed) return hipErrorInvalidValue;
    hipLaunchKernelGGL(head_pack_kernel, dim3((HEAD_PACK + 255) / 256), dim3(256), 0, s, *h);
    return hipGetLastError();
}

int piml::head_stage_fwd(const piml_collision_head* h, hipStream_t s) {
    if (int e = head_check(h)) return e;
    if (h->rows == 0) return hipSuccess;
    const long long tiles = (h->rows + 31) / 32;
    if (g_head_x3) hipLaunchKernelGGL(head_fwd_kernel<true>, dim3((unsigned)((tiles + 3) / 4)), dim3(256), 0, s, h->msgs, h->rows, h->packed, h->out);
    else hipLaunchKernelGGL(head_fwd_kernel<false>, dim3((unsigned)((tiles + 3) / 4)), dim3(256), 0, s, h->msgs, h->rows, h->packed, h->out);
    return hipGetLastError();
}

PIML_API int piml_decoder_fwd(const piml_decoder_branch* br, int nbr, const float* self_features, float tau,
                              float* acc, void* stream) {
    hipStream_t s = as_stream(stream);
    if (int e = dec_stage_pack(br, nbr, s)) return e;
    if (int e = dec_stage_pool(br, nbr, s)) return e;
    return dec_stage_fwd(br, nbr, self_features, tau, acc, s);
}

PIML_API int piml_decoder_bwd(const piml_decoder_branch* br, int nbr, const float* g_pred, const float* self_features,
                              float tau, float* g_self, void* stream) {
    hipStream_t s = as_stream(stream);
    if (int e = dec_stage_bwd_dx(br, nbr, g_pred, self_features, tau, g_self, s)) return e;
    return dec_stage_bwd_dw(br, nbr, g_pred, true, s);
}

static long long rowdec_slab(long long rows) {
    long long slab = (rows + 255) / 256;
    slab = (slab + DEC_SLAB - 1) / DEC_SLAB * DEC_SLAB;
    const long long least = rows < 16384 ? 64 : 256;
    return slab < least ? least : slab;
}

constexpr int kRowdecBigTiles = 1024;

static int rowdec_wg_split(const piml_decoder_branch* br, int nbr, int total) {
    if (nbr < 2) return total;
    int w = (int)(total * (double)br[0].agents / ((double)br[0].agents + (double)br[1].agents) + 0.5);
    return w < 1 ? 1 : (w > total - 1 ? total - 1 : w);
}

PIML_API int piml_rowdecoder_slots(long long rows) {
    if (rows <= 0) return 0;
    const long long slab = rowdec_slab(rows);
    return (int)((rows + slab - 1) / slab);
}

static int rowdec_fill(DecArgs& A, const piml_decoder_branch* br, int nbr, bool bwd) {
    if (!br || nbr < 1 || nbr > 2) return hipErrorInvalidValue;
    A = DecArgs{};
    A.nbr = nbr;
    for (int i = 0; i < nbr; ++i) {
        const piml_decoder_branch& b = br[i];
        if (!dec_branch_ok(b) || !b.h1 || !b.d2) return hipErrorInvalidValue;
        if (!bwd && !b.pred) return hipErrorInvalidValue;
        if (bwd && (!b.g_pred_rows || !b.g_pre2 || !b.g_pre1 || !b.g_pooled || !b.partials || !b.grads)) return hipErrorInvalidValue;
        A.br[i] = b;
    }
// ... 110 lines not shown
```

piml_amd/csrc/encoder_bwd5.hip:

```cpp
#include "common.hpp"
#include "encoder.hpp"
#include "x3.hpp"
#include "store.hpp"

namespace piml {

typedef short f5_s16x4 __attribute__((ext_vector_type(4)));
typedef __attribute__((address_space(3))) f5_s16x4 f5_lds_s16x4;

constexpr int F5_THREADS = 512;
constexpr int F5_IMG = 3 * 128 * 64;
constexpr int F5_M = 0;
constexpr int F5_H = F5_M + 2 * F5_IMG;
constexpr int F5_TROW = 36;
constexpr int F5_TBYTES = 128 * F5_TROW * 4;
constexpr int F5_T = F5_H + 2 * F5_IMG;
constexpr int F5_XS = F5_T + 2 * F5_TBYTES;
constexpr int F5_MK = F5_XS + 3 * 1024;
constexpr int F5_W1 = F5_MK + 2 * 512;
constexpr int F5_GXP = F5_W1 + 4096;
constexpr int F5_GXP_BYTES = 4 * 32 * 16 * 4;
constexpr int F5_TAB = F5_GXP + 2 * F5_GXP_BYTES;
constexpr int F5_KMAX = 16;
constexpr int F5_LDS_BYTES = F5_TAB + F5_KMAX * 2 * 16 * 4;
constexpr int F5_LDS_LAUNCH = F5_LDS_BYTES;
static_assert(F5_LDS_LAUNCH <= 160 * 1024, "fits the CU");
constexpr int F5_PART1 = EH * EH + 1024 + 2 * EH;

struct F5Args {
    EncArgs A;
    int nA[2];
    DecSlotSums D;
};

template <int C>
__device__ __forceinline__ float f5_row_shl(float v) {
    return __int_as_float(__builtin_amdgcn_mov_dpp(__float_as_int(v), 0x100 + C, 0xf, 0xf, false));
}
template <int C>
__device__ __forceinline__ void f5_chains_add(float4& s, const float4 v) {
    if constexpr (C < 16) {
        slot_chains_add(s, make_float4(f5_row_shl<C>(v.x), f5_row_shl<C>(v.y), f5_row_shl<C>(v.z), f5_row_shl<C>(v.w)));
        f5_chains_add<C + 1>(s, v);
    }
}
__device__ __forceinline__ void f5_dec_sums(const DecSlotSums& D, int wg, int nwg, int t, int nthr) {
    const int total = D.nsets * D.lanes, per = (total + nwg - 1) / nwg;
    const int e1 = min(wg * per + per, total), half = nthr >> 4;
    for (int e = wg * per + (t >> 4); e < e1; e += 2 * half) {
        const bool two = e + half < e1;
        const int ea = e, eb = two ? e + half : e;
        const int sa = ea >= D.lanes ? 1 : 0, sb = eb >= D.lanes ? 1 : 0;
        const float4* const p[2] = {reinterpret_cast<const float4*>(sa ? D.parts[1] : D.parts[0]),
                                    reinterpret_cast<const float4*>(sb ? D.parts[1] : D.parts[0])};
        const int j[2] = {ea - sa * D.lanes, eb - sb * D.lanes};
        float4 s[2];
        slot_chains<2>(p, D.slots, D.lanes, j, t & 15, s);
        const float4 va = s[0], vb = s[1];
        f5_chains_add<1>(s[0], va);
        f5_chains_add<1>(s[1], vb);
        if ((t & 15) == 0) {
            slot_sum_store(reinterpret_cast<float4*>(sa ? D.grads[1] : D.grads[0]) + j[0], s[0], D.accumulate != 0);
            if (two) slot_sum_store(reinterpret_cast<float4*>(sb ? D.grads[1] : D.grads[0]) + j[1], s[1], D.accumulate != 0);
        }
    }
}

#ifdef PIML_F5_STAMPS
__device__ unsigned long long g_f5_stamps[256 * 8 * 16];
#define F5_STAMP(i)                                                        \
    do {                                                                   \
        __builtin_amdgcn_sched_barrier(0);                                 \
        {                                                                  \
            const unsigned long long t_ = __builtin_amdgcn_s_memtime();    \
            st[i] += t_ - tprev;                                           \
            tprev = t_;                                                    \
        }                                                                  \
        __builtin_amdgcn_sched_barrier(0);                                 \
    } while (0)
#else
#define F5_STAMP(i)
#endif

#define F5_BARRIER() asm volatile("s_waitcnt lgkmcnt(0)\n\ts_barrier" ::: "memory")

__device__ __forceinline__ float f5_relu(float x) { return __int_as_float(max(__float_as_int(x), 0)); }
__device__ __forceinline__ constexpr int f5_rho(int r) { return (r & 3) + 8 * (r >> 2); }

#define F5_SLOT(MF, FILL)                        \
    do {                                         \
        MF;                                      \
        __builtin_amdgcn_sched_barrier(0);       \
        FILL;                                    \
        __builtin_amdgcn_sched_barrier(0);       \
    } while (0)

template <bool GX, int INC, int CPM>
__device__ __forceinline__ void enc_bwd_sums2_body(const F5Args& F) {
    constexpr bool CP = CPM != 0;
    extern __shared__ __align__(16) unsigned char smem[];
    const int tid = threadIdx.x, lane = tid & 63;
    const int wv = __builtin_amdgcn_readfirstlane(tid >> 6);
    const int crew = wv >> 2, w = wv & 3;
    const int ctid = tid & 255;
    const int n = lane & 31, h = lane >> 5;
    int bx = (int)blockIdx.x, b = 0;
    const int* __restrict__ plan = CP ? F.A.br[1].plan : nullptr;
    int nA0 = F.nA[0], nA1 = F.nA[1], nne = 0, nemp = 0, ctiles = 0;
    if (CP) {
        nne = __builtin_amdgcn_readfirstlane(plan[0]); nemp = __builtin_amdgcn_readfirstlane(plan[1]);
        ctiles = __builtin_amdgcn_readfirstlane(plan[2]);
        nA0 = __builtin_amdgcn_readfirstlane(plan[3]); nA1 = __builtin_amdgcn_readfirstlane(plan[4]);
    }
    if (CPM == 2 || (CPM == 0 && bx >= nA0)) { b = 1; bx -= nA0; }
    const piml_encoder_branch J = b ? F.A.br[1] : F.A.br[0];
    const int nwg = b ? nA1 : nA0;
    constexpr bool cp = CPM == 2;
    const bool cpe = cp && nemp > 0;
    const unsigned R = (unsigned)J.rows;
    const unsigned IN = __builtin_amdgcn_readfirstlane((unsigned)J.in_dim), K = __builtin_amdgcn_readfirstlane((unsigned)J.k);
    const unsigned kmagic = __builtin_amdgcn_readfirstlane((unsigned)((0x100000000ull + K - 1) / K));
    const int ntiles = cp ? ctiles : (int)((R + 31) >> 5);
    const int nit = bx < ntiles ? (ntiles - bx + nwg - 1) / nwg : 0;
    float* P = J.partials + (size_t)bx * F5_PART1;
    constexpr int NS = INC == 6 ? 3 : 4;

    auto rsrc = [&](const void* base, unsigned bytes) {
        return __builtin_amdgcn_make_buffer_rsrc(const_cast<void*>(base), 0, (int)bytes, 0x00020000);
    };
    constexpr unsigned kOut = 0x80000000u;
    const __amdgpu_buffer_rsrc_t rs_gp = rsrc(J.g_pooled, (R / K) * EH * 4);
    const __amdgpu_buffer_rsrc_t rs_x = rsrc(J.x, R * IN * 4);
    const __amdgpu_buffer_rsrc_t rs_mk = rsrc(J.relu_mask, (unsigned)ntiles * 1024);
    const __amdgpu_buffer_rsrc_t rs_gx = rsrc(J.g_x, GX ? R * IN * 4 : 0u);
    const unsigned cS = CP ? 32u / K : 1u;
    const __amdgpu_buffer_rsrc_t rs_pl = rsrc(CP ? plan + CP_LISTS : nullptr, CP ? (unsigned)nne * 4u : 0u);
    auto ld1 = [&](const __amdgpu_buffer_rsrc_t& rs, unsigned voff, unsigned soff) {
        return (unsigned)__builtin_amdgcn_raw_buffer_load_b32(rs, (int)voff, (int)soff, 0);
    };

// ... 546 lines not shown
```

piml_amd/csrc/encoder_x3.hip:

```cpp
#include <cstdlib>

#include "common.hpp"
#include "encoder.hpp"
#include "philox.hpp"
#include "x3.hpp"

namespace piml {

struct Pieces {
    u32x4 hi[8], mid[8], lo[8];
};

__device__ __forceinline__ void split_tile(const f32x16 (&in)[4], Pieces& P) {
#pragma unroll
    for (int kb = 0; kb < 8; ++kb) {
        const f32x16& a = in[kb >> 1];
        const int r = 8 * (kb & 1);
        unsigned hi[4], mid[4], lo[4];
#pragma unroll
        for (int d = 0; d < 4; ++d) split3(a[r + 2 * d], a[r + 2 * d + 1], hi[d], mid[d], lo[d]);
        P.hi[kb] = (u32x4){hi[0], hi[1], hi[2], hi[3]};
        P.mid[kb] = (u32x4){mid[0], mid[1], mid[2], mid[3]};
        P.lo[kb] = (u32x4){lo[0], lo[1], lo[2], lo[3]};
    }
// ... 588 lines not shown
    if (!cp && (long long)((int)blockIdx.x - wg0) >= ntiles) return;
    const float* x3 = J.packed + PACK_F32;
    float xb[4];
    ENC_STAMP(0, false);
    const int k = J.k;
    const int agents = CP ? (int)(R / k) : 0;
    int iv[CP_ROUNDS0];
    if (cp) {
#pragma unroll
        for (int i = 0; i < CP_ROUNDS0; ++i) {
            const int a = i * ENC_THREADS + tid;
            iv[i] = a < agents ? J.nbr_idx[(size_t)a * k] : -1;
        }
    } else {
        load_x(xb, J.x, first, ntiles, R, IN, lane);
    }
    stage_linear<X3_IMG>(lds, x3, tid);
    stage_linear<1024 + 384>(lds + X3_FWD_F32, J.packed + 32768, tid);
    ENC_STAMP(1, true);
    int nne = 0, nemp = 0, S = 1, slot_n = 0, kn = 0;
    bool rowlive = false;
    const unsigned short* list = reinterpret_cast<const unsigned short*>(lds + CP_LDS_LIST);
    if (cp) {
        int* cnt = reinterpret_cast<int*>(lds + CP_LDS_CNT);
        unsigned short* lw = reinterpret_cast<unsigned short*>(lds + CP_LDS_LIST);
        const int rounds = (agents + ENC_THREADS - 1) / ENC_THREADS;
        unsigned flags = 0;
#pragma unroll
        for (int i = 0; i < CP_ROUNDS0; ++i) flags |= (iv[i] >= 0 ? 1u : 0u) << i;
        for (int i = CP_ROUNDS0; i < rounds; ++i) {
            const int a = i * ENC_THREADS + tid;
            const int v = a < agents ? J.nbr_idx[(size_t)a * k] : -1;
            flags |= (v >= 0 ? 1u : 0u) << i;
        }
        for (int i = 0; i < rounds; ++i) {
            const unsigned long long bal = __ballot((flags >> i) & 1u);
            if (lane == 0) cnt[i * ENC_WAVES + wave] = __popcll(bal);
        }
        __syncthreads();
        if (wave == 0) {
            int v[4], tot = 0;
#pragma unroll
            for (int u = 0; u < 4; ++u) { v[u] = 4 * lane + u < rounds * ENC_WAVES ? cnt[4 * lane + u] : 0; tot += v[u]; }
            int inc = tot;
#pragma unroll
            for (int d = 1; d < 64; d <<= 1) {
                const int o = __shfl_up(inc, d, 64);
                if (lane >= d) inc += o;
            }
            int ex = inc - tot;
#pragma unroll
            for (int u = 0; u < 4; ++u) { cnt[4 * lane + u] = ex; ex += v[u]; }
            if (lane == 63) cnt[256] = inc;
        }
        __syncthreads();
        nne = uniform(cnt[256]);
        nemp = agents - nne;
        for (int i = 0; i < rounds; ++i) {
            const int a = i * ENC_THREADS + tid;
            const unsigned bit = (flags >> i) & 1u;
            const unsigned long long bal = __ballot(bit);
            const int pos = cnt[i * ENC_WAVES + wave] + __popcll(bal & ((1ull << lane) - 1ull));
            if (a < agents) lw[bit ? pos : agents - 1 - (a - pos)] = (unsigned short)a;
        }
        S = 32 / k;
        ntiles = (nne + S - 1) / S;
        const int n = lane & 31;
        slot_n = n / k; kn = n - slot_n * k; rowlive = slot_n < S;
        if ((int)blockIdx.x == wg0) {
            if (tid == 0) cnt[257] = 0x7fffffff;
        }
        __syncthreads();
        if ((int)blockIdx.x == wg0) {
            const int tiles0 = (int)((A.br[0].rows + 31) >> 5);
            if (tid >= 2 && tid <= PIML_COMPACT_SLOTS - 2)
                atomicMin(reinterpret_cast<unsigned*>(cnt + 257), cp_split_cost(tid, tiles0, (int)ntiles, nemp) * 256u + (unsigned)tid);
            const int apad = (agents + 3) & ~3;
            for (int c = tid; c < nne; c += ENC_THREADS) J.plan[CP_LISTS + c] = list[c];
            for (int e = tid; e < nemp; e += ENC_THREADS) J.plan[CP_LISTS + apad + e] = list[agents - 1 - e];
            __syncthreads();
            if (tid == 0) {
                const int w0 = cnt[257] & 255;
                J.plan[0] = nne; J.plan[1] = nemp; J.plan[2] = (int)ntiles; J.plan[3] = w0; J.plan[4] = PIML_COMPACT_SLOTS - w0;
            }
        }
    } else {
        __syncthreads();
    }
    ENC_STAMP(2, false);
    auto load_xc = [&](long long tile) {
        const int idx = S * (int)tile + slot_n;
        const bool ok = tile < ntiles && rowlive && idx < nne;
        const long long row = ok ? (long long)list[idx] * k + kn : 0;
#pragma unroll
        for (int s = 0; s < 4; ++s) {
            const int c = 2 * s + (lane >> 5);
            xb[s] = (ok && c < IN) ? J.x[row * IN + c] : 0.f;
        }
    };
    if (cp) load_xc(first);
    const long long agents_d = R / k;
    for (long long tile = first; tile < ntiles; tile += stride) {
        int lane_t = lane;
        asm volatile("" : "+v"(lane_t));
        const u32x4* W2hm = reinterpret_cast<const u32x4*>(lds) + lane_t;
        const u32x4* W2lo = W2hm + X3_HM / 4;
        const float* W1f = lds + X3_FWD_F32;
        const float* bias = W1f + 1024;
        const int h = lane_t >> 5;
        f32x16 a[4];
        Pieces P;
#pragma unroll
        for (int blk = 0; blk < 4; ++blk) {
#pragma unroll
            for (int q = 0; q < 4; ++q) {
                const float4 bq = *reinterpret_cast<const float4*>(bias + feat0(blk, q, h));
                a[blk][4 * q + 0] = bq.x; a[blk][4 * q + 1] = bq.y; a[blk][4 * q + 2] = bq.z; a[blk][4 * q + 3] = bq.w;
            }
#pragma unroll
            for (int s = 0; s < 4; ++s) a[blk] = mfma32(W1f[(blk * 4 + s) * 64 + lane_t], xb[s], a[blk]);
#pragma unroll
            for (int r = 0; r < 16; ++r) a[blk][r] = relu1(a[blk][r]);
        }
        uint2* mrow = reinterpret_cast<uint2*>(J.relu_mask) + (tile * 2) * 64 + lane_t;
        mrow[0] = make_uint2(sign_bits(a[0], a[1]), sign_bits(a[2], a[3]));
        ENC_STAMP(3, false);
        split_tile(a, P);
        ENC_STAMP(4, false);
        if (cp) load_xc(tile + stride);
        else load_x(xb, J.x, tile + stride, ntiles, R, IN, lane);
#pragma unroll
        for (int blk = 0; blk < 4; ++blk) {
            f32x16 acc, sm;
            const float bv = bias[128 + 32 * blk + (lane_t & 31)];
#pragma unroll
            for (int r = 0; r < 16; ++r) { sm[r] = 0.f; acc[r] = bv; }
#pragma unroll
            for (int kb = 0; kb < 8; ++kb) {
                const int fb = blk * 8 + kb;
                kblock_x3_t(acc, sm, W2hm[(fb * 2) * 64], W2hm[(fb * 2 + 1) * 64], W2lo[fb * 64], P.hi[kb], P.mid[kb], P.lo[kb]);
            }
#pragma unroll
            for (int r = 0; r < 16; ++r) a[blk][r] = relu1(acc[r] + sm[r]);
        }
        ENC_STAMP(5, false);
        mrow[64] = make_uint2(sign_bits(a[0], a[1]), sign_bits(a[2], a[3]));
        if (J.h2) store_h2_rows<true>(a, J.h2, tile, R, lane_t);
        ENC_STAMP(6, false);
        if (cp) {
            if (k == 10) pool_rows_c<10>(a, (int)tile, nne, list, lane_t, J.sum_a, J.sum_b);
            else if (k == 6) pool_rows_c<6>(a, (int)tile, nne, list, lane_t, J.sum_a, J.sum_b);
            else pool_rows_c<2>(a, (int)tile, nne, list, lane_t, J.sum_a, J.sum_b);
        } else {
            pool_rows_k(a, k, tile, agents_d, lane_t, J.sum_a, J.sum_b);
        }
        ENC_STAMP(7, false);
    }
    if (cp && nemp > 0) {
        const int nwav = nwg * ENC_WAVES, idle = nwav - (int)ntiles;
        const int q = idle > 0 ? (int)first - (int)ntiles : (int)first, share = idle > 0 ? idle : nwav;
        if (q >= 0) {
            const float2 hc = reinterpret_cast<const float2*>(J.packed + PACK_ZROW + EH)[lane];
            const float2 v = make_float2((float)k * hc.x, (float)k * hc.y);
            for (int e = q; e < nemp; e += share) {
                const int ag = list[agents - 1 - e];
                reinterpret_cast<float2*>(J.sum_a + (size_t)ag * EH)[lane] = v;
// ... 595 lines not shown
```

piml_amd/csrc/network.hip:

```cpp
#include <cstdio>
#include <cstdlib>
#include <mutex>

#include "common.hpp"
#include "pack.hpp"
#include "reduce.hpp"
#include "stages.hpp"
#include "trace.hpp"

namespace piml {

namespace {

struct Side {
    hipStream_t s[2] = {nullptr, nullptr};
    hipEvent_t ev[6] = {};
    bool ok = false;
};

constexpr int kMaxDevices = 64;
Side g_side[kMaxDevices];
std::mutex g_mu;

int side_streams(Side** out) {
// ... 199 lines not shown
    for (int i = 0; P->valid && i < P->R.nsets; ++i)
        if (P->R.set[i].grads == grads) return true;
    return false;
}

int pending_slot_sums_leave(const ReduceAll& R, hipStream_t s) {
    PendingSums* P = pending_entry();
    if (!P) return hipErrorInvalidDevice;
    {
        std::lock_guard<std::mutex> lock(g_mu);
        ReduceAll& Q = P->R;
        bool merge = P->valid && P->stream == s && Q.accumulate == R.accumulate && Q.nunf == 0 && R.nunf == 0 &&
                     Q.nsets + R.nsets <= (int)(sizeof(Q.set) / sizeof(Q.set[0]));
        for (int i = 0; merge && i < Q.nsets; ++i)
            for (int j = 0; j < R.nsets; ++j)
                if (Q.set[i].grads == R.set[j].grads) { merge = false; break; }
        if (merge) {
            for (int j = 0; j < R.nsets; ++j) Q.set[Q.nsets++] = R.set[j];
            if (R.gx > Q.gx) Q.gx = R.gx;
            return hipSuccess;
        }
    }
    if (int e = pending_slot_sums_flush()) return e;
    std::lock_guard<std::mutex> lock(g_mu);
    P->R = R; P->stream = s; P->valid = true;
    return hipSuccess;
}

bool pending_slot_sums_take(hipStream_t s, ReduceAll* out) {
    PendingSums* P = pending_entry();
    if (!P) return false;
    std::lock_guard<std::mutex> lock(g_mu);
    if (!P->valid || P->stream != s) return false;
    *out = P->R;
    P->valid = false;
    return true;
}

}

using namespace piml;

PIML_API int piml_pinnsf_streams_init(void) {
    Side* S;
    return side_streams(&S);
}

PIML_API int piml_pinnsf_pack(const piml_encoder_branch* enc, const piml_decoder_branch* dec, int nbr,
                              const piml_collision_head* head, int flags, void* stream) {
    if (!enc || !dec || nbr < 1 || nbr > 2) return hipErrorInvalidValue;
    PackAll A = {};
    A.nbr = nbr;
    A.has_head = head != nullptr;
    A.skip_f32 = enc_f32_images_needed() ? 0 : 1;
    for (int i = 0; i < nbr; ++i) {
        const piml_encoder_branch& e = enc[i];
        const piml_decoder_branch& d = dec[i];
        if (e.in_dim < 1 || e.in_dim > 8 || !e.w1 || !e.b1 || !e.w2 || !e.b2 || !e.w3 || !e.b3 || !e.packed || !d.w1 || !d.b1 ||
            !d.w2 || !d.b2 || !d.w3 || !d.b3 || !d.packed)
            return hipErrorInvalidValue;
        A.enc[i] = e;
        A.dec[i] = d;
    }
    if (head) {
        if (!head->w1 || !head->b1 || !head->w2 || !head->b2 || !head->packed) return hipErrorInvalidValue;
        A.head = *head;
        if (head->fold_w3) {
            if (!head->fold_b3) return hipErrorInvalidValue;
            A.has_fold = 1;
        }
    }
    for (int i = 0; i < nbr; ++i)
        if (dec[i].fold_w3) {
            if (!dec[i].fold_b3) return hipErrorInvalidValue;
            A.has_fold = 1;
        }
    if (flags & PIML_DEFER_PACK) return pending_pack_leave(A, as_stream(stream));
    return launch_pack(A, as_stream(stream));
}

PIML_API int piml_pinnsf_pack_flush(void) { return pending_pack_flush(nullptr); }

static int reduce_all(const piml_encoder_branch* enc, const piml_decoder_branch* dec, int nbr, hipStream_t s, bool accumulate, bool defer = false,
                      bool sums = false, bool defer_unfold = false, bool dec_summed = false) {
    ReduceAll R = {};
    R.accumulate = accumulate ? 1 : 0;
    R.defer_unfold = defer_unfold ? 1 : 0;
    R.dec_upstream = dec_summed ? 1 : 0;
    int w0 = 0, n = 0, maxl = 0;
    const int total = piml_encoder_workgroups(enc, nbr, &w0);
    const int dslots = piml_decoder_workgroups(dec[0].agents);
    int n0[2] = {0, 0}, n1[2] = {0, 0};
    const bool dw2 = !sums && enc_dw2_used(enc, nbr, n0, n1);
    auto add = [&](const float* parts, float* grads, int slots, int lanes, int split, int off0, int off1) {
        R.set[n++] = ReduceSet{parts, grads, slots, lanes, split, off0, off1};
        if (lanes > maxl) maxl = lanes;
    };
    for (int i = 0; i < nbr; ++i) {
        if (sums) {
            add(enc[i].partials, enc[i].grads, nbr == 1 ? total : (i == 0 ? w0 : total - w0), DW2_L1_LANES, DW2_L1_SPLIT, DW2_L1_OFF0, DW2_L1_OFF1);
            if (nbr == 2 && enc[1].plan) R.set[n - 1].dev_slots = enc[1].plan + 3 + i;
            R.unf[i] = UnfoldSet{dec[i].grads, dec[i].w1, enc[i].w3, enc[i].b3, dec[i].fold_scale, enc[i].k, dec[i].dw1_out, enc[i].grads};
            R.nunf = nbr;
        } else if (dw2) {
            add(enc[i].partials, enc[i].grads, n0[i], DW2_L0_LANES, DW2_L0_SPLIT, 0, DW2_L0_OFF1);
            add(enc[i].partials + (size_t)n0[i] * (DW2_L0_LANES * 4), enc[i].grads, n1[i], DW2_L1_LANES, DW2_L1_SPLIT, DW2_L1_OFF0, DW2_L1_OFF1);
        } else {
            add(enc[i].partials, enc[i].grads, nbr == 1 ? total : (i == 0 ? w0 : total - w0), ENC_PART / 4, 0x7fffffff, 0, 0);
        }
    }
    if (!dec_summed)
        for (int i = 0; i < nbr; ++i) add(dec[i].partials, dec[i].grads, dslots, DEC_PART / 4, 0x7fffffff, 0, 0);
    R.nsets = n;
    R.gx = (maxl + 15) / 16;
    if (defer) return pending_slot_sums_leave(R, s);
    UnfoldTail t;
    if (int e = launch_slot_sums(unfold_begin(R, s, &t), s)) return e;
    trace_mark("pinnsf_reduce", s);
    return unfold_end(t);
}

static int g_dec_slots_enc = !(getenv("PIML_ENC_DEC_SLOTS") && atoi(getenv("PIML_ENC_DEC_SLOTS")) == 0);

PIML_API int piml_encoder_sums_dec_slots(int on) {
    const int old = g_dec_slots_enc;
    if (on >= 0) g_dec_slots_enc = on ? 1 : 0;
    return old;
}

static int g_compact_rows = !(getenv("PIML_ENC_COMPACT") && atoi(getenv("PIML_ENC_COMPACT")) == 0);

PIML_API int piml_encoder_compact_rows(int on) {
    const int old = g_compact_rows;
    if (on >= 0) g_compact_rows = on ? 1 : 0;
    return old;
}

PIML_API int piml_pinnsf_slot_sums_flush(void) { return pending_slot_sums_flush(); }

PIML_API int piml_pinnsf_pool_h2_ok(const piml_encoder_branch* enc, int nbr) { return enc_pool_h2_ok(enc, nbr) ? 1 : 0; }
PIML_API int piml_pinnsf_pool_train_ok(const piml_encoder_branch* enc, int nbr) { return enc_pool_train_ok(enc, nbr) ? 1 : 0; }
PIML_API int piml_pinnsf_pool_msgs_ok(const piml_encoder_branch* enc, int nbr) { return enc_pool_msgs_ok(enc, nbr) ? 1 : 0; }

PIML_API int piml_pinnsf_fwd(const piml_encoder_branch* enc, const piml_decoder_branch* dec, int nbr,
                             const piml_collision_head* head, const float* self_features, float tau, float* acc,
                             int flags, void* stream) {
    hipStream_t m = as_stream(stream);
    const bool pack = !(flags & PIML_PACKED_VALID);
    PIML_TRY(pending_pack_flush(m));
    if (flags & PIML_POOL_TRAIN) {
        if ((flags & (PIML_FORK | PIML_POOL_H2)) || !enc_pool_train_ok(enc, nbr)) return hipErrorInvalidValue;
        for (int i = 0; i < nbr; ++i)
            if (dec[i].pooled != enc[i].sum_a || dec[i].msgs != enc[i].sum_b) return hipErrorInvalidValue;
        if (pack) PIML_TRY(piml_pinnsf_pack(enc, dec, nbr, head, 0, stream));
        PIML_TRY(enc_stage_fwd_sum(enc, nbr, m, nbr > 1 ? acc : nullptr, nbr > 1 ? dec[0].agents * 2 : 0));
        trace_mark("enc_fwd_sum", m);
        PIML_TRY(dec_stage_fwd_sum(dec, nbr, head, self_features, tau, acc, m));
        trace_mark("dec_fwd_head_sum", m);
        return hipSuccess;
    }
    if (flags & PIML_POOL_MSGS) {
        if ((flags & (PIML_FORK | PIML_POOL_H2)) || !enc_pool_msgs_ok(enc, nbr)) return hipErrorInvalidValue;
        for (int i = 0; i < nbr; ++i)
            if (dec[i].pooled != enc[i].sum_a || dec[i].msgs != enc[i].sum_b) return hipErrorInvalidValue;
        if (head && head->rows > 0 && head->msgs != enc[0].msgs) return hipErrorInvalidValue;
        if (pack) PIML_TRY(piml_pinnsf_pack(enc, dec, nbr, head, 0, stream));
        PIML_TRY(enc_stage_fwd(enc, nbr, m, nbr > 1 ? acc : nullptr, nbr > 1 ? dec[0].agents * 2 : 0, true));
        trace_mark("enc_fwd", m);
        PIML_TRY(dec_stage_fwd_sum(dec, nbr, head, self_features, tau, acc, m, false));
        trace_mark("dec_fwd_head_sum", m);
        return hipSuccess;
    }
    if (flags & PIML_POOL_H2) {
        if ((flags & PIML_FORK) || head || !enc_pool_h2_ok(enc, nbr)) return hipErrorInvalidValue;
        if (pack) PIML_TRY(piml_pinnsf_pack(enc, dec, nbr, nullptr, 0, stream));
        PIML_TRY(enc_stage_fwd_pool(enc, nbr, m, nbr > 1 ? acc : nullptr, nbr > 1 ? dec[0].agents * 2 : 0));
        trace_mark("enc_fwd", m);
        PIML_TRY(dec_stage_fwd_ph2(dec, nbr, self_features, tau, acc, m));
        trace_mark("dec_fwd_head", m);
        return hipSuccess;
    }
    if (!(flags & PIML_FORK)) {
        if (pack) PIML_TRY(piml_pinnsf_pack(enc, dec, nbr, head, 0, stream));
        PIML_TRY(enc_stage_fwd(enc, nbr, m, nbr > 1 ? acc : nullptr, nbr > 1 ? dec[0].agents * 2 : 0));
        trace_mark("enc_fwd", m);
        PIML_TRY(dec_stage_fwd_fused(dec, nbr, head, self_features, tau, acc, m));
        trace_mark("dec_fwd_head", m);
        return hipSuccess;
    }
    Side* S;
    PIML_TRY(side_streams(&S));
    hipStream_t s0 = S->s[0], s1 = S->s[1];
    if (pack) {
        PIML_TRY(edge(m, s0, S->ev[0]));
        PIML_TRY(dec_stage_pack(dec, nbr, s0));
        if (head) PIML_TRY(head_stage_pack(head, s0));
        PIML_TRY(hipEventRecord(S->ev[1], s0));
        PIML_TRY(enc_stage_pack(enc, nbr, m));
    }
    PIML_TRY(enc_stage_fwd(enc, nbr, m));
    if (head) {
        PIML_TRY(edge(m, s1, S->ev[2]));
        if (pack) PIML_TRY(hipStreamWaitEvent(s1, S->ev[1], 0));
        PIML_TRY(head_stage_fwd(head, s1));
        PIML_TRY(hipEventRecord(S->ev[3], s1));
    }
    PIML_TRY(dec_stage_pool(dec, nbr, m));
    if (pack) PIML_TRY(hipStreamWaitEvent(m, S->ev[1], 0));
    PIML_TRY(dec_stage_fwd(dec, nbr, self_features, tau, acc, m));
    if (head) PIML_TRY(hipStreamWaitEvent(m, S->ev[3], 0));
    return hipSuccess;
}

PIML_API int piml_pinnsf_bwd(const piml_encoder_branch* enc, const piml_decoder_branch* dec, int nbr, const float* g_pred,
                             const float* self_features, float tau, float* g_self, int flags, void* stream) {
    hipStream_t m = as_stream(stream);
    if (flags & PIML_POOL_TRAIN) {
        if (flags & PIML_FORK) return hipErrorInvalidValue;
        for (int i = 0; i < nbr; ++i)
            if (!dec[i].dw1_out || !dec[i].fold_w3 || dec[i].g_pooled != enc[i].g_pooled) return hipErrorInvalidValue;
        PIML_TRY(dec_stage_bwd_fused(dec, nbr, g_pred, self_features, tau, g_self, m, true));
        trace_mark("dec_bwd", m);
        DecSlotSums D = {};
        if (g_dec_slots_enc) {
            D.nsets = nbr;
            D.slots = piml_decoder_workgroups(dec[0].agents);
            D.lanes = DEC_PART / 4;
            D.accumulate = (flags & PIML_ACCUMULATE) != 0;
            for (int i = 0; i < nbr; ++i) {
                D.parts[i] = dec[i].partials;
                D.grads[i] = dec[i].grads;
                if (pending_slot_sums_write(dec[i].grads)) D.nsets = 0;
            }
        }
        bool dec_summed = false;
        PIML_TRY(enc_stage_bwd_sum(enc, nbr, m, D.nsets > 0 ? &D : nullptr, &dec_summed));
        trace_mark("enc_bwd_dx", m);
        return reduce_all(enc, dec, nbr, m, (flags & PIML_ACCUMULATE) != 0, (flags & PIML_DEFER_SLOT_SUMS) != 0, true,
                          (flags & PIML_DEFER_UNFOLD) != 0, dec_summed);
    }
    if (!(flags & PIML_FORK)) {
        PIML_TRY(dec_stage_bwd_fused(dec, nbr, g_pred, self_features, tau, g_self, m));
        trace_mark("dec_bwd", m);
        PIML_TRY(enc_stage_bwd_dx(enc, nbr, m));
        trace_mark("enc_bwd_dx", m);
        PIML_TRY(enc_stage_bwd_dw(enc, nbr, m));
        trace_mark("enc_bwd_dw", m);
        PIML_TRY(reduce_all(enc, dec, nbr, m, (flags & PIML_ACCUMULATE) != 0, (flags & PIML_DEFER_SLOT_SUMS) != 0));
        return hipSuccess;
    }
    if (flags & (PIML_ACCUMULATE | PIML_DEFER_SLOT_SUMS)) return hipErrorInvalidValue;
    PIML_TRY(dec_stage_bwd_dx(dec, nbr, g_pred, self_features, tau, g_self, m));
    Side* S;
    PIML_TRY(side_streams(&S));
    hipStream_t s0 = S->s[0];
    PIML_TRY(edge(m, s0, S->ev[4]));
    PIML_TRY(dec_stage_bwd_dw(dec, nbr, g_pred, true, s0));
    PIML_TRY(hipEventRecord(S->ev[5], s0));
    PIML_TRY(enc_stage_bwd_dx(enc, nbr, m));
    PIML_TRY(enc_stage_bwd_dw(enc, nbr, m));
    PIML_TRY(hipStreamWaitEvent(m, S->ev[5], 0));
    return enc_stage_reduce(enc, nbr, m);
}
```

piml_amd/csrc/pack.hpp:

```cpp
#pragma once
#include <hip/hip_runtime.h>

#include "../../include/piml_hip.h"

namespace piml {

constexpr int EH = 128;
constexpr int DH = 128;
constexpr int DD = 64;
constexpr int ENC_PART = 2 * EH * EH + EH * 8 + 3 * EH;
constexpr int DEC_PART = DD * DH + DD * DD + 2 * DD + DD + DD + 8;

constexpr int PACK_FWD = 16384 * 2 + 1024 + 384;
constexpr int PACK_DX = 16384 * 2 + 1024;
constexpr int PACK_F32 = PACK_FWD + PACK_DX;

constexpr int X3_HM = 32 * 2 * 64 * 4;
constexpr int X3_LO = 32 * 64 * 4;
constexpr int X3_IMG = X3_HM + X3_LO;
constexpr int PACK_X3 = 4 * X3_IMG;
constexpr int PACK_FLOATS = PACK_F32 + PACK_X3;
constexpr int PACK_ZROW = PACK_FLOATS;
constexpr int PACK_TOTAL = PACK_FLOATS + 2 * EH;

// ... 92 lines not shown
    {
        const bool t1 = e >= DP_T1;
        const int f = t1 ? e - DP_T1 : e - DP_T2;
        const float* W = t1 ? J.w1 : J.w2;
        const int cols = t1 ? DH : DD;
        const int u = f & 3, lane = (f >> 2) & 63, q = (f >> 8) & 3, rest = f >> 10;
        const int bp = rest & 1, blk = rest >> 1;
        const int r = 32 * bp + 8 * q + 4 * (lane >> 5) + u;
        return W[(size_t)r * cols + 32 * blk + (lane & 31)];
    }
}

constexpr int HP_B = 2 * 4 * 4 * 256;
constexpr int HP_W2 = HP_B + 68;
constexpr int HP_X3 = HP_W2 + 64;
constexpr int HP_X3F = HP_X3 + 2 * 8 * 3 * 256;
constexpr int HP_BF = HP_X3F + 2 * 8 * 3 * 256;
constexpr int HEAD_PACK = HP_BF + 64;
constexpr int HEAD_PACK_PLAIN = HP_X3F;
static_assert(HP_X3 % 4 == 0 && HP_X3F % 4 == 0, "16-byte aligned fragments");

__device__ __forceinline__ float head_pack_value(const piml_collision_head& H, int e) {
    const float* __restrict__ w1 = H.w1;
    if (e >= HEAD_PACK_PLAIN) return 0.f;
    if (e < HP_B) {
        const int u = e & 3, lane = (e >> 2) & 63, q = (e >> 8) & 3, rest = e >> 10;
        const int bp = rest & 3, ob = rest >> 2;
        const int i = 32 * ob + (lane & 31), c = 32 * bp + 8 * q + 4 * (lane >> 5) + u;
        return w1[(size_t)i * DH + c];
    }
    if (e >= HP_X3) {
        const int x = e - HP_X3, d = x & 3, lane = (x >> 2) & 63, rest = x >> 8;
        const int piece = rest % 3, kb = (rest / 3) & 7, ob = rest / 24;
        const int i = 32 * ob + (lane & 31), c = 16 * kb + 8 * (lane >> 5) + 2 * d;
        unsigned hi, mid, lo;
        split3(w1[(size_t)i * DH + c], w1[(size_t)i * DH + c + 1], hi, mid, lo);
        return __uint_as_float(piece == 0 ? hi : (piece == 1 ? mid : lo));
    }
    if (e >= HP_W2) return H.w2[e - HP_W2];
    const int g = e - HP_B;
    return g < 64 ? H.b1[g] : (g == 64 ? H.b2[0] : 0.f);
}

constexpr int FOLD_GROUPS = DD * 3;

template <int CH>
__device__ __forceinline__ double fold_partial(const float* __restrict__ row, const float* __restrict__ col, int stride, int chunk) {
    constexpr int N = DH / CH;
    float wv[N], xv[N];
#pragma unroll
    for (int t = 0; t < N; ++t) { wv[t] = row[chunk * N + t]; xv[t] = col[(size_t)(chunk * N + t) * stride]; }
    double a = 0.0;
#pragma unroll
    for (int t = 0; t < N; ++t) a += (double)wv[t] * (double)xv[t];
    return a;
}

__device__ __forceinline__ void dec_fold_store(const piml_decoder_branch& J, int i, int hc, int lane, double sum) {
    const float v = (float)((double)J.fold_scale * sum);
    if (hc == 2) {
        if (lane == 0) J.packed[DP_CF + i] = v;
        return;
    }
    const int c = 64 * hc + lane;
    J.packed[DP_A1F + ((((i >> 5) * 4 + (c >> 5)) * 4 + ((c >> 3) & 3)) * 64 + (i & 31) + 32 * ((c >> 2) & 1)) * 4 + (c & 3)] = v;
    J.packed[DP_T1F + ((((c >> 5) * 2 + (i >> 5)) * 4 + ((i >> 3) & 3)) * 64 + (c & 31) + 32 * ((i >> 2) & 1)) * 4 + (i & 3)] = v;
}
__device__ __forceinline__ void head_fold_store(const piml_collision_head& H, int i, int hc, int lane, double sum) {
    if (hc == 2) {
        if (lane == 0) H.packed[HP_BF + i] = (float)((double)H.b1[i] + (double)H.fold_scale * sum);
        return;
    }
    const float a = (float)((double)H.fold_scale * sum);
    const float b = __shfl_down(a, 1, 64);
    if (lane & 1) return;
    const int c = 64 * hc + lane;
    unsigned hi, mid, lo;
    split3(a, b, hi, mid, lo);
    unsigned* dst = reinterpret_cast<unsigned*>(H.packed + HP_X3F) + ((((i >> 5) * 8 + (c >> 4)) * 3) * 64 + (i & 31) + 32 * ((c >> 3) & 1)) * 4 + ((c & 7) >> 1);
    dst[0] = hi; dst[256] = mid; dst[512] = lo;
}

template <int N>
__device__ __forceinline__ void slot_chains(const float4* const (&parts)[N], int B, int lanes, const int (&j)[N], int c, float4 (&s)[N]) {
#pragma unroll
    for (int n = 0; n < N; ++n) s[n] = make_float4(0.f, 0.f, 0.f, 0.f);
    for (int q0 = c; q0 < B; q0 += 16 * 8) {
        float4 v[N][8];
#pragma unroll
        for (int n = 0; n < N; ++n)
#pragma unroll
            for (int u = 0; u < 8; ++u) {
                const int q = q0 + 16 * u;
                v[n][u] = parts[n][(size_t)(q < B ? q : c) * lanes + j[n]];
            }
#pragma unroll
        for (int n = 0; n < N; ++n)
#pragma unroll
            for (int u = 0; u < 8; ++u) {
                const bool ok = q0 + 16 * u < B;
                s[n].x += ok ? v[n][u].x : 0.f; s[n].y += ok ? v[n][u].y : 0.f; s[n].z += ok ? v[n][u].z : 0.f; s[n].w += ok ? v[n][u].w : 0.f;
            }
    }
}
__device__ __forceinline__ void slot_chains_add(float4& s, const float4 v) { s.x += v.x; s.y += v.y; s.z += v.z; s.w += v.w; }
__device__ __forceinline__ void slot_sum_store(float4* dst, float4 s, bool accumulate) {
    if (accumulate) slot_chains_add(s, *dst);
    *dst = s;
}

__device__ __forceinline__ void sum_slots_16x16_at(int bx, const float* __restrict__ partials, float* __restrict__ grads, int B, int lanes,
                                                   int split = 0x7fffffff, int off0 = 0, int off1 = 0, bool accumulate = false) {
    __shared__ float4 sh[256];
    const int col = threadIdx.x & 15, grp = threadIdx.x >> 4;
    const int j = bx * 16 + col;
    float4 s = make_float4(0.f, 0.f, 0.f, 0.f);
    if (j < lanes) {
        const float4* const p[1] = {reinterpret_cast<const float4*>(partials)};
        const int jj[1] = {j};
        float4 r[1];
        slot_chains<1>(p, B, lanes, jj, grp, r);
        s = r[0];
    }
    sh[threadIdx.x] = s;
    __syncthreads();
    if (grp == 0 && j < lanes) {
#pragma unroll
        for (int q = 1; q < 16; ++q) slot_chains_add(s, sh[q * 16 + col]);
        slot_sum_store(reinterpret_cast<float4*>(grads) + (j < split ? off0 + j : off1 + (j - split)), s, accumulate);
    }
}

struct DecSlotSums {
    const float* parts[2];
    float* grads[2];
    int nsets, slots, lanes, accumulate;
};

__device__ __forceinline__ void sum_slots_16x16(const float* __restrict__ partials, float* __restrict__ grads, int B, int lanes,
                                                int split = 0x7fffffff, int off0 = 0, int off1 = 0, bool accumulate = false) {
    sum_slots_16x16_at((int)blockIdx.x, partials, grads, B, lanes, split, off0, off1, accumulate);
}

constexpr int DW2_L0_LANES = (EH * EH + EH) / 4, DW2_L0_SPLIT = EH * EH / 4, DW2_L0_OFF1 = (2 * EH * EH + 1024) / 4;
constexpr int DW2_L1_LANES = (EH * EH + 1024 + 2 * EH) / 4, DW2_L1_SPLIT = (EH * EH + 1024) / 4, DW2_L1_OFF0 = EH * EH / 4,
              DW2_L1_OFF1 = (2 * EH * EH + 1024 + EH) / 4;

}
```

piml_amd/csrc/stages.hpp:

```cpp
#pragma once
#include <hip/hip_runtime.h>

#include "../../include/piml_hip.h"
#include "pack.hpp"

namespace piml {

int enc_stage_pack(const piml_encoder_branch* br, int nbr, hipStream_t s);
bool enc_f32_images_needed();
int enc_stage_fwd(const piml_encoder_branch* br, int nbr, hipStream_t s, float* zero = nullptr, long long zero_n = 0, bool msum = false);
bool enc_pool_msgs_ok(const piml_encoder_branch* br, int nbr);
bool enc_pool_h2_ok(const piml_encoder_branch* br, int nbr);
int enc_stage_fwd_pool(const piml_encoder_branch* br, int nbr, hipStream_t s, float* zero = nullptr, long long zero_n = 0);
bool enc_pool_train_ok(const piml_encoder_branch* br, int nbr);
int enc_stage_fwd_sum(const piml_encoder_branch* br, int nbr, hipStream_t s, float* zero = nullptr, long long zero_n = 0);
int enc_stage_bwd_sum(const piml_encoder_branch* br, int nbr, hipStream_t s, const DecSlotSums* dec = nullptr, bool* dec_summed = nullptr);
int enc_stage_bwd_dx(const piml_encoder_branch* br, int nbr, hipStream_t s);
int enc_stage_bwd_dw(const piml_encoder_branch* br, int nbr, hipStream_t s);
int enc_stage_reduce(const piml_encoder_branch* br, int nbr, hipStream_t s, bool accumulate = false, bool defer = false);
bool enc_dw2_used(const piml_encoder_branch* br, int nbr, int* n0, int* n1);

int dec_stage_pack(const piml_decoder_branch* br, int nbr, hipStream_t s);
int dec_stage_pool(const piml_decoder_branch* br, int nbr, hipStream_t s);
int dec_stage_fwd_fused(const piml_decoder_branch* br, int nbr, const piml_collision_head* h, const float* self_features,
                        float tau, float* acc, hipStream_t s);
int dec_stage_fwd_ph2(const piml_decoder_branch* br, int nbr, const float* self_features, float tau, float* acc,
                      hipStream_t s);
int dec_stage_fwd(const piml_decoder_branch* br, int nbr, const float* self_features, float tau, float* acc,
                  hipStream_t s);
int dec_stage_bwd_dx(const piml_decoder_branch* br, int nbr, const float* g_pred, const float* self_features, float tau,
                     float* g_self, hipStream_t s);
int dec_stage_bwd_fused(const piml_decoder_branch* br, int nbr, const float* g_pred, const float* self_features, float tau,
                        float* g_self, hipStream_t s, bool sums = false);
int dec_stage_fwd_sum(const piml_decoder_branch* br, int nbr, const piml_collision_head* h, const float* self_features, float tau,
                      float* acc, hipStream_t s, bool fold = true);
int dec_stage_bwd_dw(const piml_decoder_branch* br, int nbr, const float* g_pred, bool reduce, hipStream_t s);

int dropout_stage(unsigned long long* state, const long long* rows, unsigned* const* bits, const unsigned* streams, int njobs,
                  int cols, float p, hipStream_t s);

int head_stage_pack(const piml_collision_head* h, hipStream_t s);
int head_stage_fwd(const piml_collision_head* h, hipStream_t s);

}
```

piml_amd/csrc/store.hpp:

```cpp
#pragma once
#include <hip/hip_runtime.h>

#ifndef PIML_WT_ENC_BWD_SLOTS
#define PIML_WT_ENC_BWD_SLOTS 3
#endif
#ifndef PIML_WT_DEC_BWD_SLOTS
#define PIML_WT_DEC_BWD_SLOTS 3
#endif

namespace piml {

typedef unsigned st_u32x4 __attribute__((ext_vector_type(4)));
typedef float st_f32x4 __attribute__((ext_vector_type(4)));

template <bool WT>
__device__ __forceinline__ void store16(float4* p, const float4 v) {
    if constexpr (WT) {
        const st_f32x4 r = {v.x, v.y, v.z, v.w};
        asm volatile("global_store_dwordx4 %0, %1, off sc1\n\ts_nop 1" ::"v"(p), "v"(r) : "memory");
    } else *p = v;
}

template <bool WT>
__device__ __forceinline__ void store16(const __amdgpu_buffer_rsrc_t rs, unsigned voff, unsigned soff, const st_u32x4 v) {
    if constexpr (WT) __builtin_amdgcn_raw_buffer_store_b128(v, rs, (int)voff, (int)soff, 16);
    else __builtin_amdgcn_raw_buffer_store_b128(v, rs, (int)voff, (int)soff, 0);
}

__device__ __forceinline__ float st_quad_xor1(float v) {
    return __int_as_float(__builtin_amdgcn_mov_dpp(__float_as_int(v), 0xB1, 0xf, 0xf, false));
}
__device__ __forceinline__ float st_quad_xor2(float v) {
    return __int_as_float(__builtin_amdgcn_mov_dpp(__float_as_int(v), 0x4E, 0xf, 0xf, false));
}
__device__ __forceinline__ float4 quad_transpose(float m0, float m1, float m2, float m3, int lane) {
    const bool odd = lane & 1, hi = lane & 2;
    const float r01 = st_quad_xor1(odd ? m0 : m1), r23 = st_quad_xor1(odd ? m2 : m3);
    const float a0 = odd ? r01 : m0, a1 = odd ? m1 : r01;
    const float a2 = odd ? r23 : m2, a3 = odd ? m3 : r23;
    const float s0 = st_quad_xor2(hi ? a0 : a2), s1 = st_quad_xor2(hi ? a1 : a3);
    return hi ? make_float4(s0, s1, a2, a3) : make_float4(a0, a1, s0, s1);
}

template <bool WT>
__device__ __forceinline__ void store4(float* p, float v) {
    if constexpr (WT) __hip_atomic_store(p, v, __ATOMIC_RELAXED, __HIP_MEMORY_SCOPE_AGENT);
    else *p = v;
}

template <int FORM, class F>
__device__ __forceinline__ void store_acc32(float* block, int ld, int lane, F&& value) {
    const int i = lane & 31, h = lane >> 5;
    if constexpr (FORM == 0 || FORM == 3) {
#pragma unroll
        for (int r = 0; r < 16; ++r) store4<FORM == 3>(block + (size_t)((r & 3) + 8 * (r >> 2) + 4 * h) * ld + i, value(r));
    } else {
        float* p = block + (size_t)(4 * h + (i & 3)) * ld + 4 * (i >> 2);
#pragma unroll
        for (int g = 0; g < 4; ++g)
            store16<FORM == 2>(reinterpret_cast<float4*>(p + (size_t)(8 * g) * ld),
                               quad_transpose(value(4 * g), value(4 * g + 1), value(4 * g + 2), value(4 * g + 3), lane));
    }
}

}
```

piml_amd/ops.py:

```python
import collections
import weakref
import ctypes
import math

import torch

from . import _lib

MAX_TOPK = 32
import contextlib
import functools
import os as _os
DETERMINISTIC_BWD = _os.environ.get('PIML_DETERMINISTIC_BWD', '0') == '1'


@functools.lru_cache(maxsize=None)
def cos_threshold(angle_deg):
    return float(torch.tensor(math.cos(3.14 * angle_deg / 180), dtype=torch.float32))


def _gpu_f32(name, t):
    if not isinstance(t, torch.Tensor) or not t.is_cuda:
        raise _lib.PimlHipError(f'{name}: expected a GPU tensor (piml_amd has no CPU path), got '
                                f'{getattr(t, "device", type(t))}')
# ... 2227 lines not shown
        return self

    def __exit__(self, *exc):
        global _DEFER_DEPTH
        _DEFER_DEPTH -= 1
        if _DEFER_DEPTH == 0:
            _flush_deferred_sums()
            _DEFER_SEEN.clear()
        return False


def _flush_deferred_sums():
    for dev in list(_DEFER_DEVS) or [None]:
        with (torch.cuda.device(dev) if dev is not None else contextlib.nullcontext()):
            _lib.check(_lib.lib().piml_pinnsf_slot_sums_flush(), 'piml_pinnsf_slot_sums_flush')
    _DEFER_DEVS.clear()
    _DEFER_KEEP.clear()


def _defer_slot_sums(params, sink, dev=None):
    if _DEFER_DEPTH <= 0 or FORK_NETWORK or _os.environ.get('PIML_DEFER_SLOT_SUMS', '1') == '0':
        return False
    ok = sink is not None
    if not ok:
        ok = all(getattr(p, 'grad', None) is None and id(p) not in _DEFER_SEEN and not getattr(p, '_backward_hooks', None)
                 and not getattr(p, '_post_accumulate_grad_hooks', None) for p in params)
        if ok:
            _DEFER_SEEN.update(id(p) for p in params)
    if ok:
        _DEFER_DEVS.add(dev)
    else:
        _flush_deferred_sums()
    return ok


class _FusedPinnsf(torch.autograd.Function):
    PER = 13
    FIRST = 10
    SELF = 9

    @staticmethod
    def forward(ctx, need_grad, nbr, scales, tau, fold_epilogue, packs, nhead, keeps, sums, self_features, *tensors):
        L = _lib.lib()
        PER = _FusedPinnsf.PER
        xs = [tensors[PER * b] for b in range(nbr)]
        ewb = [[_gpu_f32('encoder weight', t.detach()) for t in tensors[PER * b + 1:PER * b + 7]] for b in range(nbr)]
        dwb = [[_gpu_f32('decoder weight', t.detach()) for t in tensors[PER * b + 7:PER * b + 13]] for b in range(nbr)]
        hwb = [_gpu_f32('head weight', t.detach()) for t in tensors[PER * nbr:PER * nbr + 4]] if nhead else None
        dev = xs[0].device
        opt = dict(device=dev, dtype=torch.float32)
        H = ENCODER_HIDDEN
        lead = tuple(xs[0].shape[:-2])
        agents = 1
        for d in lead:
            agents *= d
        sf = _gpu_f32('self_features', self_features).reshape(agents, 7) if fold_epilogue else None
        x2s, ks, msgs, h1s, h2s = [], [], [], [], []
        msum = False
        for b in range(nbr):
            x = _gpu_f32('encoder input', xs[b])
            if tuple(x.shape[:-2]) != lead:
                raise ValueError('fused_pinnsf: both branches must share the leading (..., N) shape')
            x2s.append(x.reshape(-1, x.shape[-1]))
            ks.append(x.shape[-2])
        if sums:
            probe = (_lib.EncoderBranch * nbr)()
            for b in range(nbr):
                probe[b].rows, probe[b].in_dim, probe[b].k = x2s[b].shape[0], x2s[b].shape[1], ks[b]
            wanted = sums
            sums = bool(L.piml_pinnsf_pool_train_ok(probe, nbr)) and not FORK_NETWORK and \
                (packs is None or packs.fold == tuple(float(sc) for sc in scales)) and all(k is None for k in keeps)
            if wanted and not sums and need_grad and not FORK_NETWORK and RELU_MASK and POOL_MSGS:
                for b in range(nbr):
                    probe[b].relu_mask = 1
                msum = bool(L.piml_pinnsf_pool_msgs_ok(probe, nbr))
        ctx.sums = sums
        nidx, plan = None, None
        if sums and nbr == 2 and ks[1] in (2, 6, 10) and x2s[0].shape[1] == 6 and x2s[1].shape[1] == 6 and \
                agents <= _lib.COMPACT_MAX_AGENTS and L.piml_encoder_compact_rows(-1) and L.piml_encoder_sums_bwd(-1) == 2:
            nidx = _nbr_idx_of(xs[1]) if xs[1].data_ptr() == x2s[1].data_ptr() else None
            if nidx is not None:
                plan = torch.empty(16 + 2 * ((agents + 3) // 4 * 4), device=dev, dtype=torch.int32)
        ctx.plan = plan
        sum_a, sum_b, masks = [None] * nbr, [None] * nbr, [None] * nbr
        for b in range(nbr):
            R = x2s[b].shape[0]
            h1s.append(None)
            if msum:
                msgs.append(torch.empty(R, H, **opt) if (nhead and b == 0) else None)
                sum_a[b], sum_b[b] = torch.empty(agents, H, **opt), torch.empty(agents, H, **opt)
                h2s.append(_h2_buffer(R, opt))
            elif sums:
                msgs.append(None)
                sum_a[b], sum_b[b] = torch.empty(agents, H, **opt), torch.empty(agents, H, **opt)
                tiles = (R + 31) // 32
                if plan is not None and b == 1:
                    tiles = max(tiles, -(-agents // (32 // ks[b])))
                masks[b] = torch.empty(2 * tiles, H, **opt)
                h2s.append(torch.empty(R, H, **opt) if (nhead and b == 0) else None)
            else:
                msgs.append(torch.empty(R, H, **opt))
                h2s.append(_h2_buffer(R, opt) if need_grad else None)
        if not sums and need_grad and _h1_needed([x2.shape[0] for x2 in x2s], alone=False):
            h1s = [torch.empty(x2.shape[0], H, **opt) for x2 in x2s]
        flags = (_lib.FORK if FORK_NETWORK else 0) | (_lib.POOL_TRAIN if sums else 0) | (_lib.POOL_MSGS if msum else 0)
        if packs is not None:
            if packs.sig != _weights_sig(ewb, dwb, hwb):
                raise ValueError('fused_pinnsf: `packs` were filled from other weight tensors, or the weights were modified in '
                                 'place since (optimizer step / load_state_dict inside a packed_weights() block): pinnsf_prepack first')
            epack, dpack, hpack = packs.epack, packs.dpack, packs.hpack
            flags |= _lib.PACKED_VALID
        else:
            epack = torch.empty(nbr, L.piml_encoder_pack_floats(), **opt)
            dpack = torch.empty(nbr, L.piml_decoder_pack_floats(), **opt)
            hpack = torch.empty(L.piml_collision_head_pack_floats(), **opt) if nhead else None
        keeps, draws = zip(*[_resolve_keep(keeps[b], x2s[b].shape[0], H, dev) for b in range(nbr)])
        earr = (_lib.EncoderBranch * nbr)(*[_enc_branch_struct(x2s[b], ks[b], scales[b], ewb[b], msgs[b], h1s[b], h2s[b],
                                                               packed=epack[b], keep_bits=keeps[b], draw_p=draws[b],
                                                               relu_mask=masks[b], sum_a=sum_a[b], sum_b=sum_b[b],
                                                               nbr_idx=nidx if b == 1 else None, plan=plan if b == 1 else None)
                                            for b in range(nbr)])
        pooled = sum_a if (sums or msum) else [torch.empty(agents, H, **opt) for _ in range(nbr)]
        dh1 = [torch.empty(agents, 64, **opt) if need_grad else None for _ in range(nbr)]
        dd2 = [torch.empty(agents, 64, **opt) if need_grad else None for _ in range(nbr)]
        folds = [(ewb[b][4], ewb[b][5], scales[b]) if sums else None for b in range(nbr)]
        darr = (_lib.DecoderBranch * nbr)(*[_dec_branch_struct(sum_b[b] if (sums or msum) else msgs[b], agents, ks[b], dwb[b], dpack[b], pooled[b],
                                                               dh1[b], dd2[b], fold=folds[b]) for b in range(nbr)])
        acc = torch.empty(agents, 2, **opt)
        head, coll = None, None
        if nhead:
            coll = torch.empty(x2s[0].shape[0], **opt)
            head = _lib.CollisionHead()
            head.msgs, head.rows = (h2s[0] if sums else msgs[0]).data_ptr(), x2s[0].shape[0]
            head.w1, head.b1, head.w2, head.b2 = [t.data_ptr() for t in hwb]
            head.packed, head.out = hpack.data_ptr(), coll.data_ptr()
            if sums:
                head.fold_w3, head.fold_b3, head.fold_scale = ewb[0][4].data_ptr(), ewb[0][5].data_ptr(), float(scales[0])
        with torch.cuda.device(dev):
            _lib.check(L.piml_pinnsf_fwd(earr, darr, nbr, ctypes.byref(head) if head is not None else None, _ptr(sf),
                                         float(tau), _ptr(acc), flags, _stream()), 'piml_pinnsf_fwd')
        if need_grad:
            saved_msgs = sum_b if sums else ([msgs[b] if msgs[b] is not None else sum_b[b] for b in range(nbr)] if msum else msgs)
            ctx.save_for_backward(*x2s, *h1s, *(masks if sums else h2s), *saved_msgs, *pooled, *dh1, *dd2,
                                  *[w for wb in ewb for w in wb],
                                  *[w for wb in dwb for w in wb], epack, dpack, *([sf] if sf is not None else []),
                                  *(hwb if nhead else []))
        ctx.meta = (nbr, tuple(scales), float(tau), bool(fold_epilogue), tuple(ks), [tuple(x.shape) for x in xs],
                    tuple(self_features.shape), agents, need_grad, int(nhead))
        ctx.keeps = keeps
        ctx.sink = ParamGradSink._active if need_grad else None
        ctx.params = tensors if need_grad else None
        ctx.set_materialize_grads(False)
        out = (acc.view(*lead, 2), *[None if (sums or msum) else msgs[b].view(*lead, ks[b], H) for b in range(nbr)])
        if nhead:
            out = out + (coll.view(*lead, ks[0]),)
        return out

    @staticmethod
    @torch.autograd.function.once_differentiable
    def backward(ctx, g_acc, *g_rest):
        nbr, scales, tau, fold, ks, xshapes, sf_shape, agents, need_grad, nhead = ctx.meta
        PER, FIRST = _FusedPinnsf.PER, _FusedPinnsf.FIRST
        nin = FIRST + PER * nbr + 4 * nhead
        grads = [None] * nin
        g_msgs = list(g_rest[:nbr])
        g_coll = g_rest[nbr] if nhead else None
        if not need_grad or (g_acc is None and g_coll is None and all(g is None for g in g_msgs)):
            return tuple(grads)
        L = _lib.lib()
        sv = list(ctx.saved_tensors)
        take = lambda n: [sv.pop(0) for _ in range(n)]
        x2s, h1s, h2s, msgs, pooled, dh1, dd2 = [take(nbr) for _ in range(7)]
        ewb = [take(6) for _ in range(nbr)]
        dwb = [take(6) for _ in range(nbr)]
        epack, dpack = take(2)
        sf = sv.pop(0) if fold else None
        hwb = take(4) if nhead else None
        dev = x2s[0].device
        opt = dict(device=dev, dtype=torch.float32)
        H = ENCODER_HIDDEN
        flags = _lib.FORK if FORK_NETWORK else 0
        if ctx.sums:
            return _FusedPinnsf._backward_sums(ctx, g_acc, g_coll, grads, x2s, h2s, pooled, dh1, dd2, ewb, dwb, epack, dpack, sf)
        if g_coll is not None:
            with torch.enable_grad():
                ins = [t.detach().requires_grad_(True) for t in (msgs[0], *hwb)]
                y = torch.sigmoid(torch.relu(ins[0] @ ins[1].t() + ins[2]) @ ins[3].t() + ins[4]).squeeze(-1)
                hg = torch.autograd.grad(y, ins, g_coll.reshape(-1), allow_unused=True)
            o = FIRST + PER * nbr
            for jx in range(4):
                if ctx.needs_input_grad[o + jx]:
                    grads[o + jx] = hg[1 + jx]
            g_msgs[0] = hg[0] if g_msgs[0] is None else g_msgs[0].reshape(-1, H) + hg[0]
        live = [b for b in range(nbr) if g_acc is not None or g_msgs[b] is not None]
        keep = []
        with torch.cuda.device(dev):
            part = L.piml_encoder_partial_floats()
            estructs, g_pooled = [], [None] * nbr
            for b in live:
                R, in_dim = x2s[b].shape
                gm = _gpu_f32('g_msgs', g_msgs[b]).reshape(R, H) if g_msgs[b] is not None else None
                g2, g1 = torch.empty(R, H, **opt), torch.empty(R, H, **opt)
                gx = torch.empty(R, in_dim, **opt) if ctx.needs_input_grad[FIRST + PER * b] else None
                if g_acc is not None:
                    g_pooled[b] = torch.empty(agents, H, **opt)
                keep.append((gm, g2, g1, gx))
                estructs.append(_enc_branch_struct(x2s[b], ks[b], scales[b], ewb[b], None, h1s[b], h2s[b], g_pooled[b], gm,
                                                   g2, g1, gx, packed=epack[b], keep_bits=ctx.keeps[b]))
            earr = (_lib.EncoderBranch * len(live))(*estructs)
            w0 = ctypes.c_int(0)
            total = L.piml_encoder_workgroups(earr, len(live), ctypes.byref(w0))
            slots = [w0.value, total - w0.value] if len(live) == 2 else [total]
            parts = [torch.empty(n, part, **opt) for n in slots]
            sink = ParamGradSink.current(ctx.sink) if (g_acc is not None and not FORK_NETWORK) else None
            dflats = None
            if sink is not None:
                ids = lambda lo, hi: tuple(id(t) for t in ctx.params[lo:hi])
                flats, acc_e = sink.take([ids(PER * b + 1, PER * b + 7) for b in live], part, opt)
                dflats, acc_d = sink.take([ids(PER * b + 7, PER * b + 13) for b in range(nbr)], L.piml_decoder_partial_floats(), opt)
                if flats is None or dflats is None or acc_e != acc_d:
                    sink, dflats = None, None
                elif acc_e:
                    flags |= _lib.ACCUMULATE
            if sink is None:
                flats = [torch.empty(part, **opt) for _ in slots]
            for i in range(len(live)):
                earr[i].partials, earr[i].grads = parts[i].data_ptr(), flats[i].data_ptr()
            if g_acc is not None:
                ga = _gpu_f32('g_acc', g_acc).reshape(agents, 2)
                want_self = fold and ctx.needs_input_grad[_FusedPinnsf.SELF]
                g_self = torch.empty(agents, 7, **opt) if want_self else None
                nwg = L.piml_decoder_workgroups(agents)
                dparts = [torch.empty(nwg, L.piml_decoder_partial_floats(), **opt) for _ in range(nbr)]
                if dflats is None:
                    dflats = [torch.empty(L.piml_decoder_partial_floats(), **opt) for _ in range(nbr)]
                dstructs = []
                for b in range(nbr):
                    gp2, gp1 = torch.empty(agents, 64, **opt), torch.empty(agents, 64, **opt)
                    keep += [gp2, gp1]
                    dstructs.append(_dec_branch_struct(msgs[b], agents, ks[b], dwb[b], dpack[b], pooled[b], dh1[b], dd2[b],
                                                       gp2, gp1, g_pooled[b], dparts[b], dflats[b]))
                darr = (_lib.DecoderBranch * nbr)(*dstructs)
                if len(live) == nbr and _defer_slot_sums([ctx.params[PER * b + jx] for b in range(nbr) for jx in range(1, 13)], sink, dev):
                    flags |= _lib.DEFER_SLOT_SUMS
                    _defer_keep(parts, dparts)
                _lib.check(L.piml_pinnsf_bwd(earr, darr, nbr, _ptr(ga), _ptr(sf), float(tau), _ptr(g_self), flags,
                                             _stream()), 'piml_pinnsf_bwd')
                if want_self:
                    grads[_FusedPinnsf.SELF] = g_self.view(sf_shape)
                for b in range(nbr):
                    flat = dflats[b]
                    o = FIRST + PER * b + 7
                    need = ctx.needs_input_grad[o:o + 6]
                    dW1, dW2 = flat[:64 * H].view(64, H), flat[64 * H:64 * H + 4096].view(64, 64)
                    dW3 = flat[64 * H + 4096:64 * H + 4096 + 128].view(2, 64)
                    rest = flat[64 * H + 4096 + 128:]
                    for jx, t in enumerate((dW1, rest[:64], dW2, rest[64:128], dW3, rest[128:130])):
                        if need[jx]:
                            if sink is not None:
                                sink.give(ctx.params[o + jx - FIRST], t)
                            else:
                                grads[o + jx] = t
            else:
                if h1s[live[0]] is None and _h1_needed([x2s[b].shape[0] for b in live], alone=False):
                    raise _lib.PimlHipError(
                        'fused_pinnsf: a backward pass through the messages of a subset of the branches only needs the '
                        'layer-1 activations, which the forward did not store; run it with PIML_H1_RECOMPUTE=0')
                _lib.check(L.piml_encoder_bwd(earr, len(live), _stream()), 'piml_encoder_bwd')
            for i, b in enumerate(live):
                flat = flats[i]
                in_dim = x2s[b].shape[1]
                o = FIRST + PER * b
                need = ctx.needs_input_grad[o:o + 7]
                if need[0]:
                    grads[o] = keep[i][3].view(xshapes[b])
                dW3, dW2 = flat[:H * H].view(H, H), flat[H * H:2 * H * H].view(H, H)
                dW1 = flat[2 * H * H:2 * H * H + H * in_dim].view(H, in_dim)
                db3, db2, db1 = flat[2 * H * H + 8 * H:].view(3, H)
                for jx, t in zip(range(1, 7), (dW1, db1, dW2, db2, dW3, db3)):
                    if need[jx]:
                        if sink is not None:
                            sink.give(ctx.params[o + jx - FIRST], t)
                        else:
                            grads[o + jx] = t
        return tuple(grads)


def _backward_sums(ctx, g_acc, g_coll, grads, x2s, masks, pooled, dh1, dd2, ewb, dwb, epack, dpack, sf):
    nbr, scales, tau, fold, ks, xshapes, sf_shape, agents, need_grad, nhead = ctx.meta
    PER, FIRST = _FusedPinnsf.PER, _FusedPinnsf.FIRST
    if g_coll is not None:
        raise _lib.PimlHipError('fused_pinnsf(sums=True): the collision head\'s output received a gradient; this form serves callers '
                                'that train on predictions[0] only (model.messages_wanted = True selects the message path)')
    if g_acc is None:
        return tuple(grads)
    L = _lib.lib()
    dev = x2s[0].device
    opt = dict(device=dev, dtype=torch.float32)
    H = ENCODER_HIDDEN
    with torch.cuda.device(dev):
        part1 = H * H + 1024 + 2 * H
        g_pooled = [torch.empty(agents, H, **opt) for _ in range(nbr)]
        gxs = [torch.empty(x2s[b].shape, **opt) if ctx.needs_input_grad[FIRST + PER * b] else None for b in range(nbr)]
        if len({g is None for g in gxs}) > 1:
            gxs = [g if g is not None else torch.empty(x2s[b].shape, **opt) for b, g in enumerate(gxs)]
        earr = (_lib.EncoderBranch * nbr)(*[_enc_branch_struct(x2s[b], ks[b], scales[b], ewb[b], None, None, None, g_pooled[b], None,
                                                               None, None, gxs[b], packed=epack[b], relu_mask=masks[b],
                                                               plan=ctx.plan if b == 1 else None)
                                            for b in range(nbr)])
        w0 = ctypes.c_int(0)
        total = L.piml_encoder_workgroups(earr, nbr, ctypes.byref(w0))
        slots = [w0.value, total - w0.value] if nbr == 2 else [total]
        if ctx.plan is not None:
            slots = [_lib.COMPACT_SLOTS] * nbr
        parts = [torch.empty(n, part1, **opt) for n in slots]
        sink = ParamGradSink.current(ctx.sink)
        flags = _lib.POOL_TRAIN
        flats = dflats = dw1 = None
        if sink is not None:
            ids = lambda lo, hi: tuple(id(t) for t in ctx.params[lo:hi])
            flats, acc_e = sink.take([ids(PER * b + 1, PER * b + 7) for b in range(nbr)], L.piml_encoder_partial_floats(), opt)
            dflats, acc_d = sink.take([ids(PER * b + 7, PER * b + 13) for b in range(nbr)], L.piml_decoder_partial_floats(), opt, mode='fold')
            dw1, _ = sink.take([ids(PER * b + 7, PER * b + 13) for b in range(nbr)], 64 * H, opt, mode='fold')
            if acc_e != acc_d:
                raise _lib.PimlHipError('fused_pinnsf(sums=True): the encoders and decoders of one network went through different numbers '
                                        'of backward passes inside ParamGradSink.step()')
            if acc_e:
                flags |= _lib.ACCUMULATE
            flags |= _lib.DEFER_UNFOLD
        else:
            flats = [torch.empty(L.piml_encoder_partial_floats(), **opt) for _ in range(nbr)]
        for b in range(nbr):
            earr[b].partials, earr[b].grads = parts[b].data_ptr(), flats[b].data_ptr()
        ga = _gpu_f32('g_acc', g_acc).reshape(agents, 2)
        want_self = fold and ctx.needs_input_grad[_FusedPinnsf.SELF]
        g_self = torch.empty(agents, 7, **opt) if want_self else None
        nwg = L.piml_decoder_workgroups(agents)
        dparts = [torch.empty(nwg, L.piml_decoder_partial_floats(), **opt) for _ in range(nbr)]
        if sink is None:
            dflats = [torch.empty(L.piml_decoder_partial_floats(), **opt) for _ in range(nbr)]
            dw1 = [torch.empty(64 * H, **opt) for _ in range(nbr)]
        keep, dstructs = [], []
        for b in range(nbr):
            gp2, gp1 = torch.empty(agents, 64, **opt), torch.empty(agents, 64, **opt)
            keep += [gp2, gp1]
            dstructs.append(_dec_branch_struct(pooled[b], agents, ks[b], dwb[b], dpack[b], pooled[b], dh1[b], dd2[b], gp2, gp1,
                                               g_pooled[b], dparts[b], dflats[b], fold=(ewb[b][4], ewb[b][5], scales[b]), dw1_out=dw1[b]))
        darr = (_lib.DecoderBranch * nbr)(*dstructs)
        if _defer_slot_sums([ctx.params[PER * b + jx] for b in range(nbr) for jx in range(1, 13)], sink, dev):
            flags |= _lib.DEFER_SLOT_SUMS
            _defer_keep(parts, dparts, dflats, flats, dw1, ctx.plan)
        _lib.check(L.piml_pinnsf_bwd(earr, darr, nbr, _ptr(ga), _ptr(sf), float(tau), _ptr(g_self), flags, _stream()), 'piml_pinnsf_bwd')
        if want_self:
            grads[_FusedPinnsf.SELF] = g_self.view(sf_shape)
        for b in range(nbr):
            flat = dflats[b]
            o = FIRST + PER * b + 7
            need = ctx.needs_input_grad[o:o + 6]
            dW2 = flat[64 * H:64 * H + 4096].view(64, 64)
            dW3 = flat[64 * H + 4096:64 * H + 4096 + 128].view(2, 64)
            rest = flat[64 * H + 4096 + 128:]
            for jx, t in enumerate((dw1[b].view(64, H), rest[:64], dW2, rest[64:128], dW3, rest[128:130])):
                if need[jx]:
                    if sink is not None:
                        sink.give(ctx.params[o + jx - FIRST], t)
                    else:
                        grads[o + jx] = t
            flat = flats[b]
            in_dim = x2s[b].shape[1]
            o = FIRST + PER * b
            need = ctx.needs_input_grad[o:o + 7]
            if need[0]:
                grads[o] = gxs[b].view(xshapes[b])
            dW3, dW2 = flat[:H * H].view(H, H), flat[H * H:2 * H * H].view(H, H)
            dW1 = flat[2 * H * H:2 * H * H + H * in_dim].view(H, in_dim)
            db3, db2, db1 = flat[2 * H * H + 8 * H:].view(3, H)
            for jx, t in zip(range(1, 7), (dW1, db1, dW2, db2, dW3, db3)):
                if need[jx]:
                    if sink is not None:
                        sink.give(ctx.params[o + jx - FIRST], t)
                    else:
                        grads[o + jx] = t
    return tuple(grads)


_FusedPinnsf._backward_sums = staticmethod(_backward_sums)


def fused_pinnsf(branches, self_features, tau, fold_epilogue=True, head=None, packs=None, sums=False):
    if not 1 <= len(branches) <= 2:
        raise ValueError('fused_pinnsf: one or two branches')
    flat = []
    for br in branches:
        x, e, d, p = br['x'], br['encoder'], br['decoder'], br['predictor']
        if not x.is_cuda:
            raise _lib.PimlHipError('fused_pinnsf: expected GPU tensors (piml_amd has no CPU path)')
        H = ENCODER_HIDDEN
        ok = (x.dim() >= 3 and 1 <= x.shape[-1] <= ENCODER_MAX_IN and x.numel() > 0 and
              [tuple(t.shape) for t in e] == [(H, x.shape[-1]), (H,), (H, H), (H,), (H, H), (H,)] and
              [tuple(t.shape) for t in d] == [(64, H), (64,), (64, 64), (64,)] and
              [tuple(t.shape) for t in p] == [(2, 64), (2,)])
        if not ok:
            raise ValueError('fused_pinnsf: unsupported geometry (encoder in<=8 -> 128 x3, decoder 128 -> 64 -> 64, '
                             'predictor 64 -> 2)')
        flat += [x, *e, *d, *p]
    if head is not None:
        if [tuple(t.shape) for t in head] != [(64, ENCODER_HIDDEN), (64,), (1, 64), (1,)]:
            raise ValueError('fused_pinnsf: head must be (w1 (64,128), b1 (64), w2 (1,64), b2 (1))')
        flat += list(head)
    if tuple(self_features.shape[:-1]) != tuple(branches[0]['x'].shape[:-2]) or self_features.shape[-1] != 7:
        raise ValueError('fused_pinnsf: self_features (..., N, 7) must match the features\' leading shape')
    need_grad = torch.is_grad_enabled() and (any(t.requires_grad for t in flat) or self_features.requires_grad)
    keeps = tuple(b.get('keep_bits') for b in branches)
    if len({(k is None, isinstance(k, tuple)) for k in keeps}) > 1:
        raise ValueError('fused_pinnsf: the same kind of keep_bits (none / given bits / drawn) for every branch')
    out = _FusedPinnsf.apply(need_grad, len(branches), tuple(float(b['scale']) for b in branches), float(tau),
                             bool(fold_epilogue), packs, int(head is not None), keeps, bool(sums), self_features, *flat)
    nbr = len(branches)
    if head is not None:
        return out[0], list(out[1:1 + nbr]), out[1 + nbr]
    return out[0], list(out[1:])


def pooled_h2_decoder_weights(enc_w, dec_w, scale, k):
    w3, b3, wd1, bd1 = enc_w[4].detach().double(), enc_w[5].detach().double(), dec_w[0].detach().double(), dec_w[1].detach().double()
    w1c = (float(scale) * (wd1 @ w3)).float().contiguous()
    b1c = (bd1 + float(scale) * int(k) * (wd1 @ b3)).float().contiguous()
    return [w1c, b1c, *dec_w[2:]]


# ... 369 lines not shown
```

Before: 249.2 billion.

## Add compact decoder path that folds empty-neighbour agents into one virtual row

Adds a DEC_COMPACT mode for the second (obstacle) decoder branch. It runs the decoder forward and backward only on agents that have neighbours, taken from the compact plan. All agents with no neighbours share one virtual row, whose output is scattered to them with atomics. In backward, their pooled gradient comes from a precomputed Jacobian row times each agent's g_pred. This is meant to skip decoder MLP work on the many identical empty rows, at the cost of extra atomics, a double-precision Jacobian computation, more kernel complexity, and per-slot reduction changes in slot_chains.

New measurement: 246.2 billion. 1.2% lower.

```diff
diff --git a/include/piml_hip.h b/include/piml_hip.h
--- a/include/piml_hip.h
+++ b/include/piml_hip.h
@@ -670,6 +670,7 @@
 #define PIML_POOL_TRAIN 64
 #define PIML_POOL_MSGS 128
 #define PIML_DEFER_UNFOLD 256
+#define PIML_DEC_COMPACT 512
 int piml_pinnsf_pool_train_ok(const piml_encoder_branch* enc, int nbranches);
 int piml_pinnsf_pool_msgs_ok(const piml_encoder_branch* enc, int nbranches);
 int piml_pinnsf_pool_h2_ok(const piml_encoder_branch* enc, int nbranches);
diff --git a/include/piml_hip_tuning.h b/include/piml_hip_tuning.h
--- a/include/piml_hip_tuning.h
+++ b/include/piml_hip_tuning.h
@@ -28,6 +28,7 @@
 int piml_encoder_sums_bwd(int form);
 int piml_encoder_sums_dec_slots(int on);
 int piml_encoder_compact_rows(int on);
+int piml_decoder_compact_rows(int on);
 int piml_relfeat_pack_form(int form);
 int piml_relfeat_pack_plan(int form, int waves, int obstacle_workgroups, int nbr, int has_head, int has_fold, int skip_f32,
                            int* pack_blocks, int* share);
diff --git a/piml_amd/_lib.py b/piml_amd/_lib.py
--- a/piml_amd/_lib.py
+++ b/piml_amd/_lib.py
@@ -116,6 +116,7 @@
 
 
 PACKED_VALID, FORK, ACCUMULATE, DEFER_SLOT_SUMS, DEFER_PACK, POOL_H2, POOL_TRAIN, POOL_MSGS, DEFER_UNFOLD = 1, 2, 4, 8, 16, 32, 64, 128, 256
+DEC_COMPACT = 512
 
 SIGNATURES = {
     'piml_abi_version': [],
@@ -276,6 +277,7 @@
     'piml_encoder_sums_bwd': [_i],
     'piml_encoder_sums_dec_slots': [_i],
     'piml_encoder_compact_rows': [_i],
+    'piml_decoder_compact_rows': [_i],
     'piml_encoder_pack': [ctypes.POINTER(EncoderBranch), _i, _p],
     'piml_encoder_workgroups': [ctypes.POINTER(EncoderBranch), _i, ctypes.POINTER(_i)],
     'piml_encoder_fwd': [ctypes.POINTER(EncoderBranch), _i, _p],
diff --git a/piml_amd/csrc/decoder.hip b/piml_amd/csrc/decoder.hip
--- a/piml_amd/csrc/decoder.hip
+++ b/piml_amd/csrc/decoder.hip
@@ -2,6 +2,7 @@
 #include <type_traits>
 
 #include "common.hpp"
+#include "encoder.hpp"
 #include "pack.hpp"
 #include "reduce.hpp"
 #include "stages.hpp"
@@ -25,7 +26,29 @@
     float* g_self;
     int wg_split;
     int pool_h2;
+    const int* cplan;
 };
+
+struct DecCpTile {
+    bool on, virt;
+    int nne, nemp, ntc;
+    const int* agent_of;
+    const int* empty_of;
+};
+template <bool CP>
+__device__ __forceinline__ DecCpTile dec_cp_tile(const DecArgs& A, int b, long long tile) {
+    DecCpTile T = {};
+    if (CP && b == 1) {
+        T.on = true;
+        T.nne = __builtin_amdgcn_readfirstlane(A.cplan[0]);
+        T.nemp = __builtin_amdgcn_readfirstlane(A.cplan[1]);
+        T.ntc = (T.nne + 31) >> 5;
+        T.virt = tile == T.ntc && T.nemp > 0;
+        T.agent_of = A.cplan + CP_LISTS;
+        T.empty_of = A.cplan + CP_LISTS + (((int)A.br[1].agents + 3) & ~3);
+    }
+    return T;
+}
 
 #ifdef PIML_DEC_STAMPS
 __device__ unsigned long long g_dec_stamps[1024 * 16];
@@ -72,8 +95,9 @@
 
 constexpr int POOL_ROWS = 10;
 
-template <bool POOL, bool SPLIT = false, bool ROWS = false>
+template <bool POOL, bool SPLIT = false, bool ROWS = false, bool CP = false>
 __device__ __forceinline__ void dec_fwd_body(const DecArgs& A, long long tile, int split_branch = 0) {
+    static_assert(!CP || (SPLIT && !POOL && !ROWS), "the compact decoder is a form of the split kernel on the sums");
     constexpr int NB = SPLIT ? 1 : 2;
     __shared__ float part1[NB][2][2][16][64];
     __shared__ float part2[NB][2][2][16][64];
@@ -85,8 +109,16 @@
     const int bi = SPLIT ? 0 : b;
     const bool active = b < A.nbr;
     const piml_decoder_branch J = b ? A.br[1] : A.br[0];
-    const long long agent = tile * 32 + j;
-    const bool valid = active && agent < J.agents;
+    const DecCpTile T = dec_cp_tile<CP>(A, b, tile);
+    if (CP && T.on && !(tile < T.ntc || T.virt)) return;
+    long long agent = tile * 32 + j, srow = agent;
+    bool valid = active && agent < J.agents;
+    if (CP && T.on) {
+        valid = T.virt ? j == 0 : agent < T.nne;
+        srow = T.virt ? T.nne : agent;
+        agent = T.virt ? T.empty_of[0] : T.agent_of[valid ? srow : 0];
+    }
+    __shared__ float vh1[CP ? DD : 1];
     const float4* PK = reinterpret_cast<const float4*>(J.packed);
     const float* bias = J.packed + DP_B;
     float4 w2f[4], w3f[4], w1f[2][4], b2v[4];
@@ -171,7 +203,7 @@
             for (int bl = 0; bl < 2; ++bl)
 #pragma unroll
                 for (int q = 0; q < 4; ++q) pv[bl][q] = *reinterpret_cast<const float4*>(base + dfeat0(2 * kh + bl, q, h));
-            if (!ROWS && A.pool_h2) {
+            if (!ROWS && A.pool_h2 && !(CP && T.on)) {
                 const long long g0 = (valid ? agent : 0) * J.k;
                 if (valid && (g0 >> 5) != ((g0 + J.k - 1) >> 5)) {
                     const float* more = J.msgs + agent * DH;
@@ -212,7 +244,15 @@
     __syncthreads();
     if (SPLIT && !POOL && !ROWS) DEC_STAMP(4, false);
     if (active) {
-        if (!POOL && !ROWS && A.pool_h2 >= 2 && ob == 0) {
+        if (CP && T.on) {
+            if (ob == 0 && valid) {
+#pragma unroll
+                for (int bl = 0; bl < 2; ++bl)
+#pragma unroll
+                    for (int q = 0; q < 4; ++q)
+                        *reinterpret_cast<float4*>(const_cast<float*>(J.msgs) + srow * DH + dfeat0(2 * kh + bl, q, h)) = pv[bl][q];
+            }
+        } else if (!POOL && !ROWS && A.pool_h2 >= 2 && ob == 0) {
             const long long g0 = (valid ? agent : 0) * J.k;
             if (valid && (g0 >> 5) != ((g0 + J.k - 1) >> 5)) {
 #pragma unroll
@@ -226,10 +266,14 @@
         for (int r = 0; r < 16; ++r) x[r] = fmaxf(part1[bi][kh][0][r][lane] + part1[bi][kh][1][r][lane], 0.f);
         x[0] = __builtin_fmaf(part1[bi][kh][0][0][lane] + part1[bi][kh][1][0][lane], 0.f, x[0]);
         if (ob == 0 && J.h1 && valid) {
-            float* o = J.h1 + agent * DD;
+            float* o = J.h1 + srow * DD;
 #pragma unroll
             for (int q = 0; q < 4; ++q)
                 *reinterpret_cast<float4*>(o + dfeat0(kh, q, h)) = make_float4(x[4 * q], x[4 * q + 1], x[4 * q + 2], x[4 * q + 3]);
+            if (CP && T.virt) {
+#pragma unroll
+                for (int r = 0; r < 16; ++r) vh1[dfeat0(kh, r >> 2, h) + (r & 3)] = x[r];
+            }
         }
         f32x16 a2;
 #pragma unroll
@@ -257,7 +301,7 @@
 #pragma unroll
         for (int r = 0; r < 16; ++r) y[r] = part2[bi][kh][0][r][lane] + part2[bi][kh][1][r][lane];
         if (J.d2 && valid) {
-            float* o = J.d2 + agent * DD;
+            float* o = J.d2 + srow * DD;
 #pragma unroll
             for (int q = 0; q < 4; ++q)
                 *reinterpret_cast<float4*>(o + dfeat0(kh, q, h)) = make_float4(y[4 * q], y[4 * q + 1], y[4 * q + 2], y[4 * q + 3]);
@@ -283,6 +327,41 @@
         if ((wave & 3) == 0 && h == 0 && agent < J.agents)
             reinterpret_cast<float2*>(J.pred)[agent] = make_float2(part3[0][0][0][j] + part3[0][1][0][j],
                                                                    part3[0][0][1][j] + part3[0][1][1][j]);
+        return;
+    }
+    if (CP && T.on) {
+        if (!T.virt) {
+            if (wave == 0 && h == 0 && valid) {
+                atomicAdd(A.acc + 2 * agent, part3[0][0][0][j] + part3[0][1][0][j]);
+                atomicAdd(A.acc + 2 * agent + 1, part3[0][0][1][j] + part3[0][1][1][j]);
+            }
+            return;
+        }
+        const int tid = threadIdx.x;
+        const float ox = part3[0][0][0][0] + part3[0][1][0][0], oy = part3[0][0][1][0] + part3[0][1][1][0];
+        for (int e = tid; e < T.nemp; e += 256) {
+            const int a = T.empty_of[e];
+            atomicAdd(A.acc + 2 * a, ox);
+            atomicAdd(A.acc + 2 * a + 1, oy);
+        }
+        __shared__ float wv[2][DD];
+        if (tid < 2 * DD) {
+            const int i = tid & 63, c = tid >> 6;
+            double sum = 0.0;
+#pragma unroll 8
+            for (int m = 0; m < DD; ++m) sum += (double)J.w2[m * DD + i] * (double)J.w3[c * DD + m];
+            wv[c][i] = vh1[i] > 0.f ? (float)sum : 0.f;
+        }
+        __syncthreads();
+        {
+            const int n = tid & 127, c = tid >> 7;
+            double sum = 0.0;
+#pragma unroll 8
+            for (int i = 0; i < DD; ++i)
+                sum += (double)J.packed[DP_T1F + ((((n >> 5) * 2 + (i >> 5)) * 4 + ((i >> 3) & 3)) * 64 + (n & 31) + 32 * ((i >> 2) & 1)) * 4 + (i & 3)] *
+                       (double)wv[c][i];
+            const_cast<float*>(J.msgs)[(J.agents + c) * DH + n] = (float)sum;
+        }
         return;
     }
     if (wave == 0 && h == 0 && agent < A.br[0].agents) {
@@ -311,9 +390,9 @@
 
 __global__ __launch_bounds__(512) void dec_fwd_kernel(DecArgs A) { dec_fwd_body<false>(A, blockIdx.x); }
 
-template <bool ROWS = false, bool SPLIT = false>
+template <bool ROWS = false, bool SPLIT = false, bool CP = false>
 __device__ __forceinline__ void dec_bwd_dx_body(const DecArgs& A, long long tile, int rows_branch = 0, float* keep_g2 = nullptr,
-                                                float* keep_g1 = nullptr) {
+                                                float* keep_g1 = nullptr, float* keep_gp = nullptr, float2 vgp = make_float2(0.f, 0.f)) {
     constexpr int NB = (ROWS || SPLIT) ? 1 : 2;
     __shared__ float part[NB][2][2][16][64];
     const int lane = threadIdx.x & 63, wave = uniform((int)(threadIdx.x >> 6));
@@ -322,8 +401,14 @@
     const int bi = (ROWS || SPLIT) ? 0 : b;
     const bool active = b < A.nbr;
     const piml_decoder_branch J = b ? A.br[1] : A.br[0];
-    const long long agent = tile * 32 + j;
-    const bool valid = active && agent < J.agents;
+    const DecCpTile T = dec_cp_tile<CP>(A, b, tile);
+    long long agent = tile * 32 + j, srow = agent;
+    bool valid = active && agent < J.agents;
+    if (CP && T.on) {
+        valid = T.virt ? j == 0 : agent < T.nne;
+        srow = T.virt ? T.nne : agent;
+        agent = T.virt ? 0 : T.agent_of[valid ? srow : 0];
+    }
     const float4* PK = reinterpret_cast<const float4*>(J.packed);
     float2 gp = make_float2(0.f, 0.f);
     float4 hv[2][4], t1f[8];
@@ -331,6 +416,8 @@
     if (active) {
         gp = reinterpret_cast<const float2*>(ROWS ? J.g_pred_rows : A.g_pred)[valid ? agent : 0];
         if (!valid) gp = make_float2(0.f, 0.f);
+        if (CP && T.virt && valid) gp = vgp;
+        if (CP && wave == 0 && h == 0) { keep_gp[2 * j] = gp.x; keep_gp[2 * j + 1] = gp.y; }
         float4 gd2[4];
         if (ROWS && J.g_d2) {
 #pragma unroll
@@ -341,7 +428,7 @@
             sfv[0] = sp[0]; sfv[1] = sp[1]; sfv[4] = sp[6];
         }
         const float bg = h ? gp.y : gp.x;
-        const float* hp = J.h1 + (valid ? agent : 0) * DD;
+        const float* hp = J.h1 + (valid ? srow : 0) * DD;
 #pragma unroll
         for (int o2 = 0; o2 < 2; ++o2)
 #pragma unroll
@@ -440,12 +527,12 @@
                 gpool = dmfma(w.z, g1c[bp][4 * q + 2], gpool);
                 gpool = dmfma(w.w, g1c[bp][4 * q + 3], gpool);
             }
-        if (valid) {
+        if (valid && !(CP && T.virt)) {
             float* o = J.g_pooled + agent * DH;
 #pragma unroll
             for (int q = 0; q < 4; ++q)
-                *reinterpret_cast<float4*>(o + dfeat0(blk, q, h)) =
-                    make_float4(gpool[4 * q], gpool[4 * q + 1], gpool[4 * q + 2], gpool[4 * q + 3]);
+                store16<PIML_WT_DEC_BWD_GPOOLED != 0>(reinterpret_cast<float4*>(o + dfeat0(blk, q, h)),
+                                                      make_float4(gpool[4 * q], gpool[4 * q + 1], gpool[4 * q + 2], gpool[4 * q + 3]));
         }
     }
     }
@@ -527,17 +614,19 @@
     }
 }
 
-__device__ __forceinline__ void dec_bwd_dw_body4(const DecArgs& A, int b, int p, int w, int lane, const float* keep_g2, const float* keep_g1) {
+template <bool CP = false>
+__device__ __forceinline__ void dec_bwd_dw_body4(const DecArgs& A, int b, int p, int w, int lane, const float* keep_g2, const float* keep_g1,
+                                                 const float* keep_gp = nullptr, long long cp_sb = 0, int cp_n = 0, const float* cp_in1 = nullptr) {
     const piml_decoder_branch J = b ? A.br[1] : A.br[0];
     const long long R = J.agents;
     const long long s0 = (long long)p * DEC_SLAB < R ? (long long)p * DEC_SLAB : R;
-    const int n = (int)(R - s0 < DEC_SLAB ? R - s0 : DEC_SLAB);
-    const long long sb = n > 0 ? s0 : 0;
+    const int n = CP ? cp_n : (int)(R - s0 < DEC_SLAB ? R - s0 : DEC_SLAB);
+    const long long sb = CP ? cp_sb : (n > 0 ? s0 : 0);
     const int i = lane & 31, h = lane >> 5;
     const int mb2 = w >> 1, nb2 = w & 1;
     const bool do3 = w < 2;
     constexpr int U = DEC_SLAB / 2;
-    const float* __restrict__ pooled0 = J.pooled + sb * DH + 32 * w + i;
+    const float* __restrict__ pooled0 = (CP ? cp_in1 : J.pooled) + sb * DH + 32 * w + i;
     const float* __restrict__ h10 = J.h1 + sb * DD + 32 * nb2 + i;
     const float* __restrict__ d20 = J.d2 + sb * DD + 32 * nb2 + i;
     const float* __restrict__ gp0 = A.g_pred + sb * 2 + (i & 1);
@@ -560,7 +649,7 @@
             const float* db = d20 + h * DD;
             const float* gb = gp0 + h * 2;
 #pragma unroll
-            for (int u = 0; u < U; ++u) { b3[u] = db[2 * u * DD]; a3[u] = gb[4 * u]; }
+            for (int u = 0; u < U; ++u) { b3[u] = db[2 * u * DD]; a3[u] = CP ? keep_gp[2 * (2 * u + h) + (i & 1)] : gb[4 * u]; }
         }
     } else {
 #pragma unroll
@@ -572,7 +661,7 @@
 #pragma unroll
             for (int u = 0; u < U; ++u) {
                 const int rc = 2 * u + h < n ? 2 * u + h : 0;
-                b3[u] = d20[rc * DD]; a3[u] = gp0[rc * 2];
+                b3[u] = d20[rc * DD]; a3[u] = CP ? keep_gp[2 * rc + (i & 1)] : gp0[rc * 2];
             }
         }
     }
@@ -639,6 +728,72 @@
     __syncthreads();
     DEC_STAMP(7, false);
     dec_bwd_dw_body4(A, b, (int)tile, uniform((int)(threadIdx.x >> 6)), threadIdx.x & 63, keep[0], keep[1]);
+}
+
+__global__ __launch_bounds__(256) void dec_bwd_split_cp_kernel(DecArgs A) {
+    const int bx = blockIdx.x, tid = threadIdx.x, lane = tid & 63, wave = uniform(tid >> 6);
+    const int tiles = (int)((A.br[0].agents + 31) >> 5);
+    const int b = bx == 2 * tiles ? 1 : (bx & 1);
+    const int tile = bx >> 1;
+    __shared__ __align__(16) float keep[2][32 * DD];
+    __shared__ float keep_gp[64];
+    const DecCpTile T = dec_cp_tile<true>(A, b, tile);
+    const piml_decoder_branch J = A.br[1];
+    float2 vgp = make_float2(0.f, 0.f);
+    if (T.virt) {
+        double sx = 0.0, sy = 0.0;
+        for (int e0 = tid; e0 < T.nemp; e0 += 256 * 16) {
+            int a[16];
+            float2 g[16];
+#pragma unroll
+            for (int u = 0; u < 16; ++u) a[u] = T.empty_of[e0 + 256 * u < T.nemp ? e0 + 256 * u : e0];
+#pragma unroll
+            for (int u = 0; u < 16; ++u) g[u] = reinterpret_cast<const float2*>(A.g_pred)[a[u]];
+#pragma unroll
+            for (int u = 0; u < 16; ++u) {
+                const bool ok = e0 + 256 * u < T.nemp;
+                sx += ok ? (double)g[u].x : 0.0; sy += ok ? (double)g[u].y : 0.0;
+            }
+        }
+        double* red = reinterpret_cast<double*>(keep[0]);
+        static_assert(sizeof(keep[0]) >= 2 * 256 * sizeof(double), "the partial sums fit");
+        red[tid] = sx;
+        red[256 + tid] = sy;
+        __syncthreads();
+        sx = 0.0; sy = 0.0;
+        for (int t = 0; t < 256; ++t) { sx += red[t]; sy += red[256 + t]; }
+        vgp = make_float2((float)sx, (float)sy);
+        __syncthreads();
+    }
+    if (!T.on || tile < T.ntc || T.virt) {
+        dec_bwd_dx_body<false, true, true>(A, tile, b, keep[0], keep[1], keep_gp, vgp);
+        __syncthreads();
+        const int n = !T.on ? 0 : (T.virt ? 1 : (T.nne - 32 * tile < DEC_SLAB ? T.nne - 32 * tile : DEC_SLAB));
+        if (T.on) dec_bwd_dw_body4<true>(A, 1, tile, wave, lane, keep[0], keep[1], keep_gp, T.virt ? T.nne : 32 * tile, n, J.msgs);
+        else {
+            const long long R = A.br[0].agents, s0 = (long long)tile * DEC_SLAB < R ? (long long)tile * DEC_SLAB : R;
+            const int n0 = (int)(R - s0 < DEC_SLAB ? R - s0 : DEC_SLAB);
+            dec_bwd_dw_body4<true>(A, 0, tile, wave, lane, keep[0], keep[1], keep_gp, n0 > 0 ? s0 : 0, n0, A.br[0].pooled);
+        }
+    }
+    if (!T.on || T.nemp == 0 || tile < T.ntc) return;
+    const int nsh = tiles - T.ntc;
+    if (nsh > 0 && T.virt) return;
+    const int nwav = 4 * (nsh > 0 ? nsh : 1), w0 = 4 * (nsh > 0 ? tile - T.ntc - 1 : 0) + wave;
+    const float* jc = J.msgs + J.agents * DH;
+    const float j0a = jc[lane], j0b = jc[lane + 64], j1a = jc[DH + lane], j1b = jc[DH + lane + 64];
+    for (int e0 = 64 * w0; e0 < T.nemp; e0 += 64 * nwav) {
+        const int cnt = T.nemp - e0 < 64 ? T.nemp - e0 : 64;
+        const int al = T.empty_of[e0 + (lane < cnt ? lane : 0)];
+        const float2 gl = reinterpret_cast<const float2*>(A.g_pred)[al];
+        for (int u = 0; u < cnt; ++u) {
+            const int a = __shfl(al, u, 64);
+            const float gx = __shfl(gl.x, u, 64), gy = __shfl(gl.y, u, 64);
+            float* o = J.g_pooled + (size_t)a * DH + lane;
+            store4<PIML_WT_DEC_BWD_GPOOLED != 0>(o, __builtin_fmaf(gy, j1a, gx * j0a));
+            store4<PIML_WT_DEC_BWD_GPOOLED != 0>(o + 64, __builtin_fmaf(gy, j1b, gx * j0b));
+        }
+    }
 }
 
 __global__ __launch_bounds__(512) void dec_bwd_dw_kernel(DecArgs A) {
@@ -1749,11 +1904,23 @@
     }
 }
 
+__global__ __launch_bounds__(256) __attribute__((amdgpu_waves_per_eu(2))) void dec_fwd_head_sum_cp_kernel(DecArgs A, piml_collision_head Hd, int dec_blocks) {
+    const int bx = blockIdx.x;
+    if (bx < dec_blocks) {
+        dec_fwd_body<false, true, false, true>(A, bx >> 1, bx == dec_blocks - 1 ? 1 : (bx & 1));
+    } else {
+        extern __shared__ __align__(16) float head_lds[];
+        head_fwd_body_x3<4, true, HEAD_LDS_GROUPS>(Hd.msgs, Hd.rows, Hd.packed, Hd.out, (long long)bx - dec_blocks, reinterpret_cast<u32x4*>(head_lds));
+    }
+}
+
 int piml::dec_stage_fwd_sum(const piml_decoder_branch* br, int nbr, const piml_collision_head* h, const float* self_features,
-                            float tau, float* acc, hipStream_t s, bool fold) {
+                            float tau, float* acc, hipStream_t s, bool fold, const int* cplan) {
     DecArgs A;
     if (!acc) return hipErrorInvalidValue;
     if (int e = dec_fill(A, br, nbr)) return e;
+    if (cplan && (!fold || nbr != 2 || !br[1].h1 || !br[1].d2 || br[1].agents > PIML_COMPACT_MAX_AGENTS)) return hipErrorInvalidValue;
+    A.cplan = cplan;
     for (int i = 0; i < nbr; ++i)
         if (!br[i].msgs || (fold && (!br[i].fold_w3 || !br[i].fold_b3))) return hipErrorInvalidValue;
     piml_collision_head Hd = {};
@@ -1772,7 +1939,8 @@
     const int tiles = (int)((br[0].agents + 31) / 32) * nbr;
     const dim3 g((unsigned)(tiles + head_blocks));
     const int lds = head_blocks ? head_lds_bytes(HEAD_LDS_GROUPS) : 0;
-    if (fold) hipLaunchKernelGGL(dec_fwd_head_sum_kernel<true>, g, dim3(256), lds, s, A, Hd, tiles);
+    if (cplan) hipLaunchKernelGGL(dec_fwd_head_sum_cp_kernel, dim3((unsigned)(tiles + 1 + head_blocks)), dim3(256), lds, s, A, Hd, tiles + 1);
+    else if (fold) hipLaunchKernelGGL(dec_fwd_head_sum_kernel<true>, g, dim3(256), lds, s, A, Hd, tiles);
     else hipLaunchKernelGGL(dec_fwd_head_sum_kernel<false>, g, dim3(256), lds, s, A, Hd, tiles);
     return hipGetLastError();
 }
@@ -1846,7 +2014,7 @@
 }
 
 int piml::dec_stage_bwd_fused(const piml_decoder_branch* br, int nbr, const float* g_pred, const float* self_features,
-                              float tau, float* g_self, hipStream_t s, bool sums) {
+                              float tau, float* g_self, hipStream_t s, bool sums, const int* cplan) {
     DecArgs A;
     if (int e = dec_fill_bwd(A, br, nbr, g_pred)) return e;
     A.self_features = self_features;
@@ -1859,6 +2027,12 @@
     }
     static_assert(DEC_SLAB == 32, "the dW slab of a workgroup is its dX tile");
     const unsigned tiles = (unsigned)((br[0].agents + 31) / 32);
+    if (cplan) {
+        if (!sums || nbr != 2 || br[1].agents > PIML_COMPACT_MAX_AGENTS) return hipErrorInvalidValue;
+        A.cplan = cplan;
+        hipLaunchKernelGGL(dec_bwd_split_cp_kernel, dim3(2 * tiles + 1), dim3(256), 0, s, A);
+        return hipGetLastError();
+    }
     hipLaunchKernelGGL(dec_bwd_split_kernel, dim3(tiles * (unsigned)nbr), dim3(256), 0, s, A);
     return hipGetLastError();
 }
diff --git a/piml_amd/csrc/encoder_bwd5.hip b/piml_amd/csrc/encoder_bwd5.hip
--- a/piml_amd/csrc/encoder_bwd5.hip
+++ b/piml_amd/csrc/encoder_bwd5.hip
@@ -47,6 +47,8 @@
 __device__ __forceinline__ void f5_dec_sums(const DecSlotSums& D, int wg, int nwg, int t, int nthr) {
     const int total = D.nsets * D.lanes, per = (total + nwg - 1) / nwg;
     const int e1 = min(wg * per + per, total), half = nthr >> 4;
+    const int B0 = D.dev_slots[0] ? __builtin_amdgcn_readfirstlane(*D.dev_slots[0]) : D.slots;
+    const int B1 = D.dev_slots[1] ? __builtin_amdgcn_readfirstlane(*D.dev_slots[1]) : D.slots;
     for (int e = wg * per + (t >> 4); e < e1; e += 2 * half) {
         const bool two = e + half < e1;
         const int ea = e, eb = two ? e + half : e;
@@ -54,8 +56,9 @@
         const float4* const p[2] = {reinterpret_cast<const float4*>(sa ? D.parts[1] : D.parts[0]),
                                     reinterpret_cast<const float4*>(sb ? D.parts[1] : D.parts[0])};
         const int j[2] = {ea - sa * D.lanes, eb - sb * D.lanes};
+        const int B[2] = {sa ? B1 : B0, sb ? B1 : B0};
         float4 s[2];
-        slot_chains<2>(p, D.slots, D.lanes, j, t & 15, s);
+        slot_chains<2>(p, B, D.lanes, j, t & 15, s);
         const float4 va = s[0], vb = s[1];
         f5_chains_add<1>(s[0], va);
         f5_chains_add<1>(s[1], vb);
diff --git a/piml_amd/csrc/encoder_x3.hip b/piml_amd/csrc/encoder_x3.hip
--- a/piml_amd/csrc/encoder_x3.hip
+++ b/piml_amd/csrc/encoder_x3.hip
@@ -694,6 +694,7 @@
             if (tid == 0) {
                 const int w0 = cnt[257] & 255;
                 J.plan[0] = nne; J.plan[1] = nemp; J.plan[2] = (int)ntiles; J.plan[3] = w0; J.plan[4] = PIML_COMPACT_SLOTS - w0;
+                J.plan[5] = (nne + 31) / 32 + (nemp > 0 ? 1 : 0);
             }
         }
     } else {
diff --git a/piml_amd/csrc/network.hip b/piml_amd/csrc/network.hip
--- a/piml_amd/csrc/network.hip
+++ b/piml_amd/csrc/network.hip
@@ -305,7 +305,7 @@
 PIML_API int piml_pinnsf_pack_flush(void) { return pending_pack_flush(nullptr); }
 
 static int reduce_all(const piml_encoder_branch* enc, const piml_decoder_branch* dec, int nbr, hipStream_t s, bool accumulate, bool defer = false,
-                      bool sums = false, bool defer_unfold = false, bool dec_summed = false) {
+                      bool sums = false, bool defer_unfold = false, bool dec_summed = false, bool dec_compact = false) {
     ReduceAll R = {};
     R.accumulate = accumulate ? 1 : 0;
     R.defer_unfold = defer_unfold ? 1 : 0;
@@ -333,7 +333,10 @@
         }
     }
     if (!dec_summed)
-        for (int i = 0; i < nbr; ++i) add(dec[i].partials, dec[i].grads, dslots, DEC_PART / 4, 0x7fffffff, 0, 0);
+        for (int i = 0; i < nbr; ++i) {
+            add(dec[i].partials, dec[i].grads, dslots, DEC_PART / 4, 0x7fffffff, 0, 0);
+            if (dec_compact && i == 1) R.set[n - 1].dev_slots = enc[1].plan + 5;
+        }
     R.nsets = n;
     R.gx = (maxl + 15) / 16;
     if (defer) return pending_slot_sums_leave(R, s);
@@ -357,6 +360,18 @@
     const int old = g_compact_rows;
     if (on >= 0) g_compact_rows = on ? 1 : 0;
     return old;
+}
+
+static int g_dec_compact = getenv("PIML_DEC_COMPACT") && atoi(getenv("PIML_DEC_COMPACT")) != 0;
+
+PIML_API int piml_decoder_compact_rows(int on) {
+    const int old = g_dec_compact;
+    if (on >= 0) g_dec_compact = on ? 1 : 0;
+    return old;
+}
+
+static bool dec_compact_ok(const piml_encoder_branch* enc, int nbr, int flags, bool fwd) {
+    return (flags & PIML_POOL_TRAIN) && nbr == 2 && enc[1].plan && (!fwd || enc[1].nbr_idx);
 }
 
 PIML_API int piml_pinnsf_slot_sums_flush(void) { return pending_slot_sums_flush(); }
@@ -375,13 +390,15 @@
         if ((flags & (PIML_FORK | PIML_POOL_H2)) || !enc_pool_train_ok(enc, nbr)) return hipErrorInvalidValue;
         for (int i = 0; i < nbr; ++i)
             if (dec[i].pooled != enc[i].sum_a || dec[i].msgs != enc[i].sum_b) return hipErrorInvalidValue;
+        if ((flags & PIML_DEC_COMPACT) && !dec_compact_ok(enc, nbr, flags, true)) return hipErrorInvalidValue;
         if (pack) PIML_TRY(piml_pinnsf_pack(enc, dec, nbr, head, 0, stream));
         PIML_TRY(enc_stage_fwd_sum(enc, nbr, m, nbr > 1 ? acc : nullptr, nbr > 1 ? dec[0].agents * 2 : 0));
         trace_mark("enc_fwd_sum", m);
-        PIML_TRY(dec_stage_fwd_sum(dec, nbr, head, self_features, tau, acc, m));
+        PIML_TRY(dec_stage_fwd_sum(dec, nbr, head, self_features, tau, acc, m, true, (flags & PIML_DEC_COMPACT) ? enc[1].plan : nullptr));
         trace_mark("dec_fwd_head_sum", m);
         return hipSuccess;
     }
+    if (flags & PIML_DEC_COMPACT) return hipErrorInvalidValue;
     if (flags & PIML_POOL_MSGS) {
         if ((flags & (PIML_FORK | PIML_POOL_H2)) || !enc_pool_msgs_ok(enc, nbr)) return hipErrorInvalidValue;
         for (int i = 0; i < nbr; ++i)
@@ -442,7 +459,9 @@
         if (flags & PIML_FORK) return hipErrorInvalidValue;
         for (int i = 0; i < nbr; ++i)
             if (!dec[i].dw1_out || !dec[i].fold_w3 || dec[i].g_pooled != enc[i].g_pooled) return hipErrorInvalidValue;
-        PIML_TRY(dec_stage_bwd_fused(dec, nbr, g_pred, self_features, tau, g_self, m, true));
+        const bool dcp = (flags & PIML_DEC_COMPACT) != 0;
+        if (dcp && !dec_compact_ok(enc, nbr, flags, false)) return hipErrorInvalidValue;
+        PIML_TRY(dec_stage_bwd_fused(dec, nbr, g_pred, self_features, tau, g_self, m, true, dcp ? enc[1].plan : nullptr));
         trace_mark("dec_bwd", m);
         DecSlotSums D = {};
         if (g_dec_slots_enc) {
@@ -453,6 +472,7 @@
             for (int i = 0; i < nbr; ++i) {
                 D.parts[i] = dec[i].partials;
                 D.grads[i] = dec[i].grads;
+                D.dev_slots[i] = (dcp && i == 1) ? enc[1].plan + 5 : nullptr;
                 if (pending_slot_sums_write(dec[i].grads)) D.nsets = 0;
             }
         }
@@ -460,8 +480,9 @@
         PIML_TRY(enc_stage_bwd_sum(enc, nbr, m, D.nsets > 0 ? &D : nullptr, &dec_summed));
         trace_mark("enc_bwd_dx", m);
         return reduce_all(enc, dec, nbr, m, (flags & PIML_ACCUMULATE) != 0, (flags & PIML_DEFER_SLOT_SUMS) != 0, true,
-                          (flags & PIML_DEFER_UNFOLD) != 0, dec_summed);
-    }
+                          (flags & PIML_DEFER_UNFOLD) != 0, dec_summed, dcp);
+    }
+    if (flags & PIML_DEC_COMPACT) return hipErrorInvalidValue;
     if (!(flags & PIML_FORK)) {
         PIML_TRY(dec_stage_bwd_fused(dec, nbr, g_pred, self_features, tau, g_self, m));
         trace_mark("dec_bwd", m);
diff --git a/piml_amd/csrc/pack.hpp b/piml_amd/csrc/pack.hpp
--- a/piml_amd/csrc/pack.hpp
+++ b/piml_amd/csrc/pack.hpp
@@ -198,23 +198,24 @@
 }
 
 template <int N>
-__device__ __forceinline__ void slot_chains(const float4* const (&parts)[N], int B, int lanes, const int (&j)[N], int c, float4 (&s)[N]) {
-#pragma unroll
-    for (int n = 0; n < N; ++n) s[n] = make_float4(0.f, 0.f, 0.f, 0.f);
-    for (int q0 = c; q0 < B; q0 += 16 * 8) {
+__device__ __forceinline__ void slot_chains(const float4* const (&parts)[N], const int (&B)[N], int lanes, const int (&j)[N], int c, float4 (&s)[N]) {
+    int Bmax = B[0];
+#pragma unroll
+    for (int n = 0; n < N; ++n) { s[n] = make_float4(0.f, 0.f, 0.f, 0.f); Bmax = B[n] > Bmax ? B[n] : Bmax; }
+    for (int q0 = c; q0 < Bmax; q0 += 16 * 8) {
         float4 v[N][8];
 #pragma unroll
         for (int n = 0; n < N; ++n)
 #pragma unroll
             for (int u = 0; u < 8; ++u) {
                 const int q = q0 + 16 * u;
-                v[n][u] = parts[n][(size_t)(q < B ? q : c) * lanes + j[n]];
+                v[n][u] = parts[n][(size_t)(q < B[n] ? q : 0) * lanes + j[n]];
             }
 #pragma unroll
         for (int n = 0; n < N; ++n)
 #pragma unroll
             for (int u = 0; u < 8; ++u) {
-                const bool ok = q0 + 16 * u < B;
+                const bool ok = q0 + 16 * u < B[n];
                 s[n].x += ok ? v[n][u].x : 0.f; s[n].y += ok ? v[n][u].y : 0.f; s[n].z += ok ? v[n][u].z : 0.f; s[n].w += ok ? v[n][u].w : 0.f;
             }
     }
@@ -233,9 +234,9 @@
     float4 s = make_float4(0.f, 0.f, 0.f, 0.f);
     if (j < lanes) {
         const float4* const p[1] = {reinterpret_cast<const float4*>(partials)};
-        const int jj[1] = {j};
+        const int jj[1] = {j}, BB[1] = {B};
         float4 r[1];
-        slot_chains<1>(p, B, lanes, jj, grp, r);
+        slot_chains<1>(p, BB, lanes, jj, grp, r);
         s = r[0];
     }
     sh[threadIdx.x] = s;
@@ -251,6 +252,7 @@
     const float* parts[2];
     float* grads[2];
     int nsets, slots, lanes, accumulate;
+    const int* dev_slots[2];
 };
 
 __device__ __forceinline__ void sum_slots_16x16(const float* __restrict__ partials, float* __restrict__ grads, int B, int lanes,
diff --git a/piml_amd/csrc/stages.hpp b/piml_amd/csrc/stages.hpp
--- a/piml_amd/csrc/stages.hpp
+++ b/piml_amd/csrc/stages.hpp
@@ -31,9 +31,9 @@
 int dec_stage_bwd_dx(const piml_decoder_branch* br, int nbr, const float* g_pred, const float* self_features, float tau,
                      float* g_self, hipStream_t s);
 int dec_stage_bwd_fused(const piml_decoder_branch* br, int nbr, const float* g_pred, const float* self_features, float tau,
-                        float* g_self, hipStream_t s, bool sums = false);
+                        float* g_self, hipStream_t s, bool sums = false, const int* cplan = nullptr);
 int dec_stage_fwd_sum(const piml_decoder_branch* br, int nbr, const piml_collision_head* h, const float* self_features, float tau,
-                      float* acc, hipStream_t s, bool fold = true);
+                      float* acc, hipStream_t s, bool fold = true, const int* cplan = nullptr);
 int dec_stage_bwd_dw(const piml_decoder_branch* br, int nbr, const float* g_pred, bool reduce, hipStream_t s);
 
 int dropout_stage(unsigned long long* state, const long long* rows, unsigned* const* bits, const unsigned* streams, int njobs,
diff --git a/piml_amd/csrc/store.hpp b/piml_amd/csrc/store.hpp
--- a/piml_amd/csrc/store.hpp
+++ b/piml_amd/csrc/store.hpp
@@ -6,6 +6,9 @@
 #endif
 #ifndef PIML_WT_DEC_BWD_SLOTS
 #define PIML_WT_DEC_BWD_SLOTS 3
+#endif
+#ifndef PIML_WT_DEC_BWD_GPOOLED
+#define PIML_WT_DEC_BWD_GPOOLED 0
 #endif
 
 namespace piml {
diff --git a/piml_amd/ops.py b/piml_amd/ops.py
--- a/piml_amd/ops.py
+++ b/piml_amd/ops.py
@@ -2333,6 +2333,8 @@
             if nidx is not None:
                 plan = torch.empty(16 + 2 * ((agents + 3) // 4 * 4), device=dev, dtype=torch.int32)
         ctx.plan = plan
+        dcomp = plan is not None and need_grad and bool(L.piml_decoder_compact_rows(-1))
+        ctx.dcomp = dcomp
         sum_a, sum_b, masks = [None] * nbr, [None] * nbr, [None] * nbr
         for b in range(nbr):
             R = x2s[b].shape[0]
@@ -2343,7 +2345,7 @@
                 h2s.append(_h2_buffer(R, opt))
             elif sums:
                 msgs.append(None)
-                sum_a[b], sum_b[b] = torch.empty(agents, H, **opt), torch.empty(agents, H, **opt)
+                sum_a[b], sum_b[b] = torch.empty(agents, H, **opt), torch.empty(agents + (2 if dcomp and b == 1 else 0), H, **opt)
                 tiles = (R + 31) // 32
                 if plan is not None and b == 1:
                     tiles = max(tiles, -(-agents // (32 // ks[b])))
@@ -2354,7 +2356,8 @@
                 h2s.append(_h2_buffer(R, opt) if need_grad else None)
         if not sums and need_grad and _h1_needed([x2.shape[0] for x2 in x2s], alone=False):
             h1s = [torch.empty(x2.shape[0], H, **opt) for x2 in x2s]
-        flags = (_lib.FORK if FORK_NETWORK else 0) | (_lib.POOL_TRAIN if sums else 0) | (_lib.POOL_MSGS if msum else 0)
+        flags = (_lib.FORK if FORK_NETWORK else 0) | (_lib.POOL_TRAIN if sums else 0) | (_lib.POOL_MSGS if msum else 0) | \
+            (_lib.DEC_COMPACT if dcomp else 0)
         if packs is not None:
             if packs.sig != _weights_sig(ewb, dwb, hwb):
                 raise ValueError('fused_pinnsf: `packs` were filled from other weight tensors, or the weights were modified in '
@@ -2432,7 +2435,7 @@
         H = ENCODER_HIDDEN
         flags = _lib.FORK if FORK_NETWORK else 0
         if ctx.sums:
-            return _FusedPinnsf._backward_sums(ctx, g_acc, g_coll, grads, x2s, h2s, pooled, dh1, dd2, ewb, dwb, epack, dpack, sf)
+            return _FusedPinnsf._backward_sums(ctx, g_acc, g_coll, grads, x2s, h2s, pooled, dh1, dd2, ewb, dwb, epack, dpack, sf, msgs)
         if g_coll is not None:
             with torch.enable_grad():
                 ins = [t.detach().requires_grad_(True) for t in (msgs[0], *hwb)]
@@ -2537,7 +2540,7 @@
         return tuple(grads)
 
 
-def _backward_sums(ctx, g_acc, g_coll, grads, x2s, masks, pooled, dh1, dd2, ewb, dwb, epack, dpack, sf):
+def _backward_sums(ctx, g_acc, g_coll, grads, x2s, masks, pooled, dh1, dd2, ewb, dwb, epack, dpack, sf, sum_b):
     nbr, scales, tau, fold, ks, xshapes, sf_shape, agents, need_grad, nhead = ctx.meta
     PER, FIRST = _FusedPinnsf.PER, _FusedPinnsf.FIRST
     if g_coll is not None:
@@ -2566,7 +2569,8 @@
             slots = [_lib.COMPACT_SLOTS] * nbr
         parts = [torch.empty(n, part1, **opt) for n in slots]
         sink = ParamGradSink.current(ctx.sink)
-        flags = _lib.POOL_TRAIN
+        dcomp = getattr(ctx, 'dcomp', False)
+        flags = _lib.POOL_TRAIN | (_lib.DEC_COMPACT if dcomp else 0)
         flats = dflats = dw1 = None
         if sink is not None:
             ids = lambda lo, hi: tuple(id(t) for t in ctx.params[lo:hi])
@@ -2587,7 +2591,7 @@
         want_self = fold and ctx.needs_input_grad[_FusedPinnsf.SELF]
         g_self = torch.empty(agents, 7, **opt) if want_self else None
         nwg = L.piml_decoder_workgroups(agents)
-        dparts = [torch.empty(nwg, L.piml_decoder_partial_floats(), **opt) for _ in range(nbr)]
+        dparts = [torch.empty(nwg + (1 if dcomp and b == 1 else 0), L.piml_decoder_partial_floats(), **opt) for b in range(nbr)]
         if sink is None:
             dflats = [torch.empty(L.piml_decoder_partial_floats(), **opt) for _ in range(nbr)]
             dw1 = [torch.empty(64 * H, **opt) for _ in range(nbr)]
@@ -2595,8 +2599,8 @@
         for b in range(nbr):
             gp2, gp1 = torch.empty(agents, 64, **opt), torch.empty(agents, 64, **opt)
             keep += [gp2, gp1]
-            dstructs.append(_dec_branch_struct(pooled[b], agents, ks[b], dwb[b], dpack[b], pooled[b], dh1[b], dd2[b], gp2, gp1,
-                                               g_pooled[b], dparts[b], dflats[b], fold=(ewb[b][4], ewb[b][5], scales[b]), dw1_out=dw1[b]))
+            dstructs.append(_dec_branch_struct(sum_b[b] if dcomp and b == 1 else pooled[b], agents, ks[b], dwb[b], dpack[b], pooled[b], dh1[b], dd2[b],
+                                               gp2, gp1, g_pooled[b], dparts[b], dflats[b], fold=(ewb[b][4], ewb[b][5], scales[b]), dw1_out=dw1[b]))
         darr = (_lib.DecoderBranch * nbr)(*dstructs)
         if _defer_slot_sums([ctx.params[PER * b + jx] for b in range(nbr) for jx in range(1, 13)], sink, dev):
             flags |= _lib.DEFER_SLOT_SUMS
```
